# niclasborlin/dbat

Hardware: AMD Instinct MI355X
Metric: LM iterations/sec (higher is better)
Workload: dtype f64

## Files before the change

dbat_amd/_hip.py:

```python
from __future__ import annotations

import ctypes as C
import os
import sys

import numpy as np

_HERE = os.path.dirname(os.path.abspath(__file__))
LIB_PATH = os.path.join(_HERE, 'libdbat_hip.so')
if os.environ.get('DBAT_AMD_LIB') == 'prof':
    LIB_PATH = os.path.join(_HERE, 'libdbat_hip_prof.so')
elif os.environ.get('DBAT_AMD_LIB', '').endswith('.so'):
    LIB_PATH = os.environ['DBAT_AMD_LIB']
if LIB_PATH != os.path.join(_HERE, 'libdbat_hip.so'):
    sys.stderr.write('[dbat_amd] DBAT_AMD_LIB: loading %s instead of the product library\n' % LIB_PATH)

ABI_VERSION = 5
DAMP = {'none': 0, 'gm': 0, 'gna': 1, 'lm': 2, 'lmp': 3}

OK, EINVAL, EUNSUPPORTED, EDEVICE, ENOMEM = 0, -101, -102, -103, -104


class DbatHipUnavailable(RuntimeError):
    pass


class DbatHipError(RuntimeError):
    def __init__(self, code, msg):
        super().__init__('dbat_hip error %d: %s' % (code, msg))
        self.code = code


_dp = C.POINTER(C.c_double)
_ip = C.POINTER(C.c_int32)
_lp = C.POINTER(C.c_int64)
_bp = C.POINTER(C.c_uint8)


class Problem(C.Structure):
    _fields_ = [
        ('abi_version', C.c_int32), ('n_images', C.c_int32), ('n_points', C.c_int32),
        ('n_obs', C.c_int64), ('dist_model', C.c_int32), ('nK', C.c_int32), ('nP', C.c_int32),
        ('ip_cam', _ip), ('ip_pt', _ip), ('ip_val', _dp), ('ip_std', _dp),
        ('IO_val', _dp), ('px_size', _dp), ('EO_val', _dp), ('OP_val', _dp),
        ('est_IO', _bp), ('est_EO', _bp), ('est_OP', _bp),
        ('IO_block', _ip), ('EO_block', _ip),
        ('prior_IO_use', _bp), ('prior_IO_val', _dp), ('prior_IO_std', _dp),
        ('prior_EO_use', _bp), ('prior_EO_val', _dp), ('prior_EO_std', _dp),
        ('prior_OP_use', _bp), ('prior_OP_val', _dp), ('prior_OP_std', _dp),
        ('device', C.c_int32), ('shard_rank', C.c_int32), ('shard_count', C.c_int32),
    ]


class Options(C.Structure):
    _fields_ = [
        ('damping', C.c_int32), ('max_iter', C.c_int32), ('conv_tol', C.c_double),
        ('abs_term', C.c_int32), ('singular_test', C.c_int32), ('store_trace', C.c_int32),
        ('mu', C.c_double), ('alpha_min', C.c_double), ('lambda0', C.c_double),
        ('lambda_min', C.c_double), ('rho_bad', C.c_double), ('rho_good', C.c_double),
        ('delta0', C.c_double),
        ('term_fun', C.c_void_p), ('term_user', C.c_void_p), ('veto_fun', C.c_void_p), ('veto_user', C.c_void_p),
        ('trace_fun', C.c_void_p), ('trace_user', C.c_void_p),
    ]


TERM_FN = C.CFUNCTYPE(C.c_int32, C.c_void_p, _dp, _dp, C.c_int64)
VETO_FN = C.CFUNCTYPE(C.c_int32, C.c_void_p, _dp, C.c_int64)
TRACE_FN = C.CFUNCTYPE(None, C.c_void_p, C.c_int32, C.c_int32, C.c_double, C.c_double, C.c_int32, C.c_double)


def trace_text(damping, n, res, damp, step, rho):
    from fractions import Fraction
    if damping == DAMP['gna']:
        if damp != damp:
            return 'Gauss-Newton-Armijo: iteration %d, residual norm=%.2g' % (n, res)
        return 'Gauss-Newton-Armijo: iteration %d, residual norm=%.2g, last alpha=%s' % (n, res, Fraction(damp).limit_denominator(1 << 40))
    if damping == DAMP['lm']:
        if damp != damp:
            return 'Levenberg-Marquardt: iteration %d, residual norm=%.2g' % (n, res)
        return 'Levenberg-Marquardt: iteration %d, residual norm=%.2g, lambda=%.2g' % (n, res, damp)
    if damping == DAMP['lmp']:
        return 'Levenberg-Marquardt-Powell: iteration %d, residual norm=%.2g, delta=%.2g, step=%s, rho=%.1f' % (
            n, res, damp, ('GN', 'IP', 'CP')[step] if 0 <= step < 3 else '?', rho)
    return 'Gauss-Markov: iteration %d, residual norm=%.2g' % (n, res)


class Result(C.Structure):
    _fields_ = [
        ('code', C.c_int32), ('iters', C.c_int32), ('n_res', C.c_int32), ('n_damp', C.c_int32),
        ('n_trace', C.c_int32), ('sigma0', C.c_double), ('time_s', C.c_double),
        ('n_residual_evals', C.c_int32), ('n_linearizations', C.c_int32), ('n_solves', C.c_int32),
        ('n_trace_only', C.c_int32), ('stage_s', C.c_double * 5),
    ]


LOSS = {'huber': 0, 'cauchy': 1}
SCALE = {'apriori': 0, 'mad': 1}
ROBUST_MAX_OUTER = 64


class RobustOptions(C.Structure):
    _fields_ = [
        ('loss', C.c_int32), ('k', C.c_double), ('scale', C.c_int32), ('max_outer', C.c_int32),
        ('weight_tol', C.c_double),
    ]


class PairOptions(C.Structure):
    _fields_ = [('max_iter', C.c_int32), ('conv_tol', C.c_double), ('min_angle', C.c_double)]


class RobustResult(C.Structure):
    _fields_ = [
        ('outer', C.c_int32), ('converged', C.c_int32), ('inner_iters', C.c_int32 * ROBUST_MAX_OUTER),
        ('scale', C.c_double * ROBUST_MAX_OUTER), ('max_change', C.c_double), ('reweight_s', C.c_double),
    ]


ALLREDUCE_FN = C.CFUNCTYPE(C.c_int, C.c_void_p, C.c_void_p, C.c_int64, C.c_void_p)

class DepthStats(C.Structure):
    _fields_ = [('n_behind', C.c_int64), ('min_depth', C.c_double), ('argmin_column', C.c_int64)]


class VetoStats(C.Structure):
    _fields_ = [('tested', C.c_int64), ('rejected', C.c_int64), ('n_behind', C.c_int64), ('min_depth', C.c_double)]


_H = C.c_void_p
SYMBOLS = {
    'dbat_hip_last_error': (C.c_char_p, []),
    'dbat_hip_abi_version': (C.c_int, []),
    'dbat_hip_default_options': (C.c_int, [C.c_int32, C.POINTER(Options)]),
    'dbat_hip_plan': (C.c_int, [C.POINTER(Problem)] + [C.POINTER(C.c_int64)] * 7),
    'dbat_hip_plan_structural_rank_ok': (C.c_int, [C.POINTER(Problem), C.POINTER(C.c_int32)]),
    'dbat_hip_plan_point_owner': (C.c_int, [C.POINTER(Problem), _ip]),
    'dbat_hip_plan_serialize': (C.c_int, [C.POINTER(Problem), _dp]),
    'dbat_hip_plan_layout_stats': (C.c_int, [C.POINTER(Problem), C.POINTER(C.c_int64)]),
    'dbat_hip_plan_domain_map': (C.c_int, [C.POINTER(Problem), _ip, C.POINTER(C.c_int32)]),
    'dbat_hip_create': (C.c_int, [C.POINTER(Problem), C.POINTER(_H)]),
    'dbat_hip_destroy': (None, [_H]),
    'dbat_hip_num_params': (C.c_int64, [_H]),
    'dbat_hip_num_residuals': (C.c_int64, [_H]),
    'dbat_hip_serialize': (C.c_int, [_H, _dp]),
    'dbat_hip_deserialize': (C.c_int, [_H, _dp, _dp, _dp, _dp]),
    'dbat_hip_structural_rank_ok': (C.c_int, [_H, C.POINTER(C.c_int32)]),
    'dbat_hip_residual': (C.c_int, [_H, _dp, _dp, _dp]),
    'dbat_hip_jacobian_blocks': (C.c_int, [_H, _dp, _dp, _dp, _dp]),
    'dbat_hip_jacobian_sample': (C.c_int, [_H, _dp, C.c_int64, C.POINTER(C.c_int64), _dp, _dp, _dp, _dp]),
    'dbat_hip_linearize_solve': (C.c_int, [_H, _dp, C.c_double, C.c_int32, _dp, _dp]),
    'dbat_hip_jacobian_csc': (C.c_int, [_H, _dp, C.c_int32, C.POINTER(C.c_int64), C.POINTER(C.c_int64), C.POINTER(C.c_int64), _dp]),
    'dbat_hip_gradient': (C.c_int, [_H, _dp]),
    'dbat_hip_colnorms': (C.c_int, [_H, _dp]),
    'dbat_hip_jtimes_sqnorm': (C.c_int, [_H, _dp, _dp]),
    'dbat_hip_jtimes': (C.c_int, [_H, _dp, _dp]),
    'dbat_hip_solve': (C.c_int, [_H, C.POINTER(Options), _dp, C.POINTER(Result), _dp, _dp, _dp, _dp]),
    'dbat_hip_final_residuals': (C.c_int, [_H, _dp, _dp]),
    'dbat_hip_comm_unique_id': (C.c_int, [_bp]),
    'dbat_hip_comm_init': (C.c_int, [_H, _bp]),
    'dbat_hip_comm_allreduce_host': (C.c_int, [_H, _dp, C.c_int64, C.c_int32]),
    'dbat_hip_set_deterministic': (C.c_int, [_H, C.c_int32]),
    'dbat_hip_set_allreduce': (C.c_int, [_H, ALLREDUCE_FN, C.c_void_p]),
    'dbat_hip_owned_mask': (C.c_int, [_H, _bp]),
    'dbat_hip_forwintersect': (C.c_int, [_H, _dp, _bp, _dp]),
    'dbat_hip_resect': (C.c_int, [C.c_int32, C.c_int32, C.POINTER(C.c_int64), _dp, _dp, C.POINTER(C.c_int64), _ip, _dp, _dp]),
    'dbat_hip_rigidalign': (C.c_int, [C.c_int32, C.c_int64, _dp, _dp, _bp, C.c_int32, _dp, _dp, _dp]),
    'dbat_hip_multixform': (C.c_int, [C.c_int32, _dp, C.c_int64, C.c_int32, _dp, C.c_int64, _dp, _bp]),
    'dbat_hip_essmat5': (C.c_int, [C.c_int32, C.c_int32, C.POINTER(C.c_int64), _dp, _dp, _dp, _ip]),
    'dbat_hip_relorient': (C.c_int, [C.c_int32, C.c_int32, C.POINTER(C.c_int64), _dp, _dp, C.POINTER(C.c_int64), _ip, _dp,
                                     C.c_int32, _dp, _dp, _ip, _bp, _bp, _dp]),
    'dbat_hip_default_pair_options': (C.c_int, [C.POINTER(PairOptions)]),
    'dbat_hip_pairadjust': (C.c_int, [C.c_int32, C.c_int32, C.POINTER(C.c_int64), _dp, _dp, _bp, _dp, _dp, C.c_int32,
                                      C.POINTER(PairOptions), _dp, _dp, _bp, _dp, _ip, _dp, _dp]),
    'dbat_hip_bench_step': (C.c_int, [_H, C.c_double, C.c_int32, _dp]),
    'dbat_hip_structure_key': (C.c_int, [C.POINTER(Problem), C.POINTER(C.c_uint64)]),
    'dbat_hip_handle_key': (C.c_int, [_H, C.POINTER(C.c_uint64)]),
    'dbat_hip_set_values': (C.c_int, [_H, C.POINTER(Problem)]),
    'dbat_hip_set_x': (C.c_int, [_H, _dp]),
    'dbat_hip_info': (C.c_int, [_H, C.POINTER(C.c_int64)]),
    'dbat_hip_build_kernel_name': (C.c_int, [_H, C.c_char_p, C.c_int32]),
    'dbat_hip_chol_stats': (C.c_int, [_H, C.POINTER(C.c_int64)]),
    'dbat_hip_posterior_cov': (C.c_int, [_H, _dp, C.c_double, _dp, _dp, _dp, _dp]),
    'dbat_hip_redundancy': (C.c_int, [_H, _dp, _dp, _dp]),
    'dbat_hip_ray_angles': (C.c_int, [_H, _dp, _dp, _dp, _ip, _ip]),
    'dbat_hip_debug_ray_angles_host': (C.c_int, [C.POINTER(Problem), _dp, _dp]),
    'dbat_hip_point_depths': (C.c_int, [_H, _dp, C.c_double, _dp, _dp, C.POINTER(DepthStats)]),
    'dbat_hip_set_chirality': (C.c_int, [_H, C.c_int32, C.c_double]),
    'dbat_hip_chirality_stats': (C.c_int, [_H, C.POINTER(VetoStats)]),
    'dbat_hip_coverage': (C.c_int, [_H, _dp, _dp, _dp, _lp, _dp, _lp, _lp]),
    'dbat_hip_residual_stats': (C.c_int, [_H, _dp, _lp, _dp, _lp, _dp, _dp, _dp, _lp]),
    'dbat_hip_quality_hull_cap': (C.c_int32, []),
    'dbat_hip_debug_coverage_host': (C.c_int, [C.POINTER(Problem), _dp, _dp, _dp, _lp, _dp, _lp, _lp]),
    'dbat_hip_default_robust_options': (C.c_int, [C.c_int32, C.POINTER(RobustOptions)]),
    'dbat_hip_robust_weights': (C.c_int, [_H, _dp, C.POINTER(RobustOptions), _dp, _dp, _dp]),
    'dbat_hip_set_obs_weights': (C.c_int, [_H, _dp]),
    'dbat_hip_solve_robust': (C.c_int, [_H, C.POINTER(Options), C.POINTER(RobustOptions), _dp, C.POINTER(Result),
                                        _dp, _dp, _dp, _dp, C.POINTER(RobustResult), _dp]),
}
DEBUG_SYMBOLS = {
    'dbat_hip_debug_plan_digest': (C.c_int, [C.POINTER(Problem), C.POINTER(C.c_uint64), C.c_int32, C.c_char_p, C.c_int32]),
    'dbat_hip_debug_heavy_plan_selftest': (C.c_int, [C.POINTER(Problem), _dp]),
    'dbat_hip_debug_batch_stats': (C.c_int, [C.POINTER(Problem), C.POINTER(C.c_int64)]),
    'dbat_hip_debug_nd_stats': (C.c_int, [C.POINTER(Problem), C.c_int32, _dp]),
    'dbat_hip_debug_model_eval_host': (C.c_int, [C.c_int32, C.c_int32, C.c_int32, _dp, _dp, C.c_double,
                                                 _dp, _dp, _dp, _dp, _dp, _dp]),
    'dbat_hip_debug_ray_angles_ms': (C.c_int, [_H, _dp, C.POINTER(C.c_int64)]),
    'dbat_hip_debug_quality_ms': (C.c_int, [_H, _dp]),
    'dbat_hip_debug_point_depths_ms': (C.c_int, [_H, _dp]),
    'dbat_hip_debug_chirality_pass_ms': (C.c_int, [_H, _dp, C.c_int32, _dp]),
    'dbat_hip_debug_align_ms': (C.c_int, [_dp]),
    'dbat_hip_debug_align_timing': (C.c_int, [C.c_int32]),
    'dbat_hip_debug_relorient_ms': (C.c_int, [_dp]),
    'dbat_hip_debug_relorient_timing': (C.c_int, [C.c_int32]),
    'dbat_hip_debug_pairadjust_ms': (C.c_int, [_dp]),
    'dbat_hip_debug_pairadjust_timing': (C.c_int, [C.c_int32]),
}

_lib = None


def load():
    global _lib
    if _lib is not None:
        return _lib
    if not os.path.exists(LIB_PATH):
        raise DbatHipUnavailable(
            '%s not built: run `python -c "import __graft_entry__ as g; g.build()"` or '
            '`make -C dbat_amd/csrc` (needs hipcc).  There is no CPU fallback.' % LIB_PATH)
    try:
        try:
            import torch
        except Exception:
            pass
        lib = C.CDLL(LIB_PATH)
    except OSError as e:
        raise DbatHipUnavailable('cannot load %s: %s' % (LIB_PATH, e)) from e
    for name, (res, args) in {**SYMBOLS, **DEBUG_SYMBOLS}.items():
        try:
            fn = getattr(lib, name)
        except AttributeError as e:
            raise DbatHipUnavailable('%s does not export %s' % (LIB_PATH, name)) from e
        fn.restype = res
        fn.argtypes = args
    if lib.dbat_hip_abi_version() != ABI_VERSION:
        raise DbatHipUnavailable('ABI version mismatch')
    _lib = lib
    return lib


UNIQUE_ID_BYTES = 128


def comm_unique_id():
    buf = (C.c_uint8 * UNIQUE_ID_BYTES)()
    check(load().dbat_hip_comm_unique_id(buf))
    return bytes(buf)


def last_error():
    return load().dbat_hip_last_error().decode('utf-8', 'replace')


def check(rc):
    if rc != 0:
        raise DbatHipError(rc, last_error())


def dptr(a):
    return a.ctypes.data_as(_dp) if a is not None else None


def _flat(a, dtype):
    a = np.asarray(a)
    if a.dtype != dtype:
        a = a.astype(dtype)
    if a.ndim <= 1:
        return np.ascontiguousarray(a)
    if a.flags.f_contiguous:
        return a.reshape(-1, order='F')
    return a.flatten('F')


def _f64(a):
    return _flat(a, np.float64)


def _u8(a):
    a = np.asarray(a)
    if a.dtype != np.bool_:
        a = a.astype(bool)
    return _flat(a, np.bool_).view(np.uint8)


def _i32(a):
    return _flat(a, np.int32)


def problem_from_struct(s, device=0, shard_rank=0, shard_count=1):
    nc, npnt, no = s.EO.val.shape[1], s.OP.val.shape[1], s.IP.val.shape[1]
    dm = np.unique(s.IO.model.distModel)
    if dm.size != 1:
        raise ValueError('Mixed lens distortion models not implemented.')
    model = int(dm[0])
    if model == 1:
        if np.any(np.asarray(s.IO.val)[3:5] != 0) or np.any(np.asarray(s.bundle.est.IO)[3:5]):
            raise ValueError('lens distortion model 1 has no aspect/skew')
        model = 2
    if npnt >= 2 ** 31 or nc >= 2 ** 31:
        raise ValueError('too many points/images for int32 indices')
    keep = dict(
        ip_cam=_i32(s.IP.cam), ip_pt=_i32(s.IP.pt), ip_val=_f64(s.IP.val), ip_std=_f64(s.IP.std),
        IO_val=_f64(s.IO.val), px_size=_f64(s.IO.sensor.pxSize), EO_val=_f64(s.EO.val[:6]),
        OP_val=_f64(s.OP.val),
        est_IO=_u8(s.bundle.est.IO), est_EO=_u8(s.bundle.est.EO[:6]), est_OP=_u8(s.bundle.est.OP),
        IO_block=_i32(s.IO.struct.block), EO_block=_i32(s.EO.struct.block[:6]),
    )
    for nm in ('IO', 'EO', 'OP'):
        pr = getattr(s.prior, nm)
        rows = slice(0, 6) if nm == 'EO' else slice(None)
        use = np.asarray(pr.use)[rows]
        keep['prior_%s_use' % nm] = _u8(use)
        if use.any():
            keep['prior_%s_val' % nm] = _f64(np.nan_to_num(np.asarray(pr.val, float)[rows]))
            keep['prior_%s_std' % nm] = _f64(np.nan_to_num(np.asarray(pr.std, float)[rows], nan=1.0))
        else:
            keep['prior_%s_val' % nm] = _f64(np.asarray(pr.val, float)[rows])
            keep['prior_%s_std' % nm] = _f64(np.asarray(pr.std, float)[rows])
    p = Problem()
    p.abi_version = ABI_VERSION
    p.n_images, p.n_points, p.n_obs = nc, npnt, no
    p.dist_model, p.nK, p.nP = model, int(s.IO.model.nK), int(s.IO.model.nP)
    for k, v in keep.items():
        ptr_t = dict(Problem._fields_)[k]
        setattr(p, k, v.ctypes.data_as(ptr_t))
    p.device, p.shard_rank, p.shard_count = int(device), int(shard_rank), int(shard_count)
    return p, keep


class Handle:

    def __init__(self, s, device=0, shard_rank=0, shard_count=1, _problem=None):
        self.lib = load()
        self.prob, self._keep = _problem if _problem is not None else problem_from_struct(s, device, shard_rank, shard_count)
        h = _H()
        check(self.lib.dbat_hip_create(C.byref(self.prob), C.byref(h)))
        self.h = h
        self.n = int(self.lib.dbat_hip_num_params(h))
        self.m = int(self.lib.dbat_hip_num_residuals(h))
        self._cb = None

    def close(self):
        if getattr(self, 'h', None):
            self.lib.dbat_hip_destroy(self.h)
            self.h = None

    __del__ = close

    def key(self):
        k = (C.c_uint64 * 2)()
        check(self.lib.dbat_hip_handle_key(self.h, k))
        return (int(k[0]), int(k[1]))

    def set_values(self, s=None, _problem=None):
        prob, keep = _problem if _problem is not None else problem_from_struct(
            s, self.prob.device, self.prob.shard_rank, self.prob.shard_count)
        check(self.lib.dbat_hip_set_values(self.h, C.byref(prob)))
        self.prob, self._keep = prob, keep

    def serialize(self):
        x = np.empty(self.n)
        check(self.lib.dbat_hip_serialize(self.h, dptr(x)))
        return x

    def deserialize(self, x):
        nc, npnt = self.prob.n_images, self.prob.n_points
        R = 5 + self.prob.nK + self.prob.nP
        IO, EO, OP = np.empty(R * nc), np.empty(6 * nc), np.empty(3 * npnt)
        x = np.ascontiguousarray(x, float)
        check(self.lib.dbat_hip_deserialize(self.h, dptr(x), dptr(IO), dptr(EO), dptr(OP)))
        return (IO.reshape(R, nc, order='F'), EO.reshape(6, nc, order='F'),
                OP.reshape(3, npnt, order='F'))

    def structural_rank_ok(self):
        ok = C.c_int32(0)
        check(self.lib.dbat_hip_structural_rank_ok(self.h, C.byref(ok)))
        return bool(ok.value)

    def residual(self, x, want_r=True):
        x = np.ascontiguousarray(x, float)
        r = np.zeros(self.m) if want_r else None
        f = C.c_double(0)
        check(self.lib.dbat_hip_residual(self.h, dptr(x), dptr(r), C.byref(f)))
        return (r, f.value) if want_r else f.value

    def jacobian_blocks(self, x):
        no, R = self.prob.n_obs, 5 + self.prob.nK + self.prob.nP
        x = np.ascontiguousarray(x, float)
        JEO, JOP, JIO = np.zeros(12 * no), np.zeros(6 * no), np.zeros(2 * R * no)
        check(self.lib.dbat_hip_jacobian_blocks(self.h, dptr(x), dptr(JEO), dptr(JOP), dptr(JIO)))
        return (JEO.reshape(no, 6, 2).transpose(0, 2, 1), JOP.reshape(no, 3, 2).transpose(0, 2, 1),
                JIO.reshape(no, R, 2).transpose(0, 2, 1))

    def jacobian_sample(self, x, ip_cols):
        idx = np.ascontiguousarray(ip_cols, np.int64)
        n, R = idx.size, 5 + self.prob.nK + self.prob.nP
        x = np.ascontiguousarray(x, float)
        r, JEO, JOP, JIO = np.zeros(2 * n), np.zeros(12 * n), np.zeros(6 * n), np.zeros(2 * R * n)
        check(self.lib.dbat_hip_jacobian_sample(self.h, dptr(x), n, idx.ctypes.data_as(C.POINTER(C.c_int64)), dptr(r), dptr(JEO),
                                                dptr(JOP), dptr(JIO)))
        return (r.reshape(n, 2), JEO.reshape(n, 6, 2).transpose(0, 2, 1), JOP.reshape(n, 3, 2).transpose(0, 2, 1),
                JIO.reshape(n, R, 2).transpose(0, 2, 1))

    def jacobian_csc(self, x, weighted=True):
        import scipy.sparse as sp
        x = np.ascontiguousarray(x, float)
        nnz = C.c_int64(0)
        check(self.lib.dbat_hip_jacobian_csc(self.h, dptr(x), int(bool(weighted)), C.byref(nnz), None, None, None))
        colptr = np.zeros(self.n + 1, np.int64)
        rowidx = np.zeros(max(nnz.value, 1), np.int64)
        val = np.zeros(max(nnz.value, 1))
        i64 = C.POINTER(C.c_int64)
        check(self.lib.dbat_hip_jacobian_csc(self.h, dptr(x), int(bool(weighted)), C.byref(nnz), colptr.ctypes.data_as(i64),
                                             rowidx.ctypes.data_as(i64), dptr(val)))
        return sp.csc_matrix((val[:nnz.value], rowidx[:nnz.value], colptr), shape=(self.m, self.n))

    def linearize_solve(self, x, lam=0.0, scale=True):
        x = np.ascontiguousarray(x, float)
        p, st = np.empty(self.n), np.empty(8)
        check(self.lib.dbat_hip_linearize_solve(self.h, dptr(x), float(lam), int(bool(scale)),
                                                dptr(p), dptr(st)))
        return p, dict(f=st[0], JpJp=st[1], rJp=st[2], pp=st[3], trace=st[4], singular=bool(st[5]), rcond=st[6], chol_info=int(st[7]))

    def gradient(self):
        g = np.empty(self.n)
        check(self.lib.dbat_hip_gradient(self.h, dptr(g)))
        return g

    def colnorms(self):
        g = np.empty(self.n)
        check(self.lib.dbat_hip_colnorms(self.h, dptr(g)))
        return g

    def jtimes_sqnorm(self, v):
        v = np.ascontiguousarray(v, float)
        out = C.c_double(0)
        check(self.lib.dbat_hip_jtimes_sqnorm(self.h, dptr(v), C.byref(out)))
        return out.value

    def jtimes(self, v):
        v = np.ascontiguousarray(v, float)
        out = np.zeros(self.m)
        check(self.lib.dbat_hip_jtimes(self.h, dptr(v), dptr(out)))
        return out

    def solve(self, x0, opt, term_fun=None, veto_fun=None, trace_fun=None):
        x = np.ascontiguousarray(x0, float).copy()
        raised = []

        def guarded(fn, *views):
            if raised:
                return 1
            try:
                return int(bool(fn(*views)))
            except BaseException as e:
                raised.append(e)
                return 1
        keep = []
        if term_fun is not None:
            keep.append(TERM_FN(lambda _u, Jp, r, m: guarded(term_fun, np.ctypeslib.as_array(Jp, (m,)).copy(),
                                                             np.ctypeslib.as_array(r, (m,)).copy())))
            opt.term_fun = C.cast(keep[-1], C.c_void_p)
        if veto_fun is not None:
            keep.append(VETO_FN(lambda _u, xx, n: guarded(veto_fun, np.ctypeslib.as_array(xx, (n,)).copy())))
            opt.veto_fun = C.cast(keep[-1], C.c_void_p)
        if trace_fun is not None:
            def traced(_u, damping, n, res, damp, step, rho):
                if not raised:
                    try:
                        trace_fun(damping, n, res, damp, step, rho)
                    except BaseException as e:
                        raised.append(e)
            keep.append(TRACE_FN(traced))
            opt.trace_fun = C.cast(keep[-1], C.c_void_p)
        try:
            return self._solve(x, opt, raised)
        finally:
            if trace_fun is not None:
                opt.trace_fun = None
            if term_fun is not None:
                opt.term_fun = None
            if veto_fun is not None:
                opt.veto_fun = None

    def _solve(self, x, opt, raised):
        res = Result()
        mi = opt.max_iter
        rr = np.full(mi + 3, np.nan)
        damp = np.full(2 * mi + 4, np.nan)
        aux = np.full(2 * mi + 4, np.nan)
        trace = np.empty(self.n * (mi + 2)) if opt.store_trace else None
        check(self.lib.dbat_hip_solve(self.h, C.byref(opt), dptr(x), C.byref(res), dptr(rr),
                                      dptr(damp), dptr(aux), dptr(trace)))
        if raised:
            raise raised[0]
        T = (trace[:self.n * res.n_trace].reshape(self.n, res.n_trace, order='F')
             if trace is not None else None)
        return x, res, rr[:res.n_res], damp[:res.n_damp], aux, T

    def final_residuals(self):
        ru, rw = np.empty(self.m), np.empty(self.m)
        check(self.lib.dbat_hip_final_residuals(self.h, dptr(ru), dptr(rw)))
        return ru, rw

    def forwintersect(self, x, OP, skip=None):
        x = np.ascontiguousarray(x, float)
        out = np.ascontiguousarray(np.asarray(OP, float).flatten('F'))
        sk = None if skip is None else np.ascontiguousarray(np.asarray(skip, bool).astype(np.uint8))
        check(self.lib.dbat_hip_forwintersect(self.h, dptr(x), None if sk is None else sk.ctypes.data_as(_bp), dptr(out)))
        return out.reshape(3, -1, order='F')

    def set_deterministic(self, on=True):
        check(self.lib.dbat_hip_set_deterministic(self.h, int(bool(on))))

    def build_kernel_name(self):
        buf = C.create_string_buffer(64)
        check(self.lib.dbat_hip_build_kernel_name(self.h, buf, 64))
        return buf.value.decode()

    def comm_init(self, unique_id):
        buf = (C.c_uint8 * UNIQUE_ID_BYTES).from_buffer_copy(bytes(unique_id))
        check(self.lib.dbat_hip_comm_init(self.h, buf))

    def comm_allreduce_host(self, a, op='sum'):
        a = np.ascontiguousarray(a, np.float64).copy()
        check(self.lib.dbat_hip_comm_allreduce_host(self.h, dptr(a), a.size, {'sum': 0, 'max': 1, 'min': 2}[op]))
        return a

    def set_allreduce(self, pyfunc):
        def tramp(user, buf, count, stream):
            try:
                return int(pyfunc(int(buf or 0), int(count), int(stream or 0)) or 0)
            except Exception:
                import traceback
                traceback.print_exc()
                return 1
        self._cb = ALLREDUCE_FN(tramp)
        check(self.lib.dbat_hip_set_allreduce(self.h, self._cb, None))

    def owned_mask(self):
        m = np.zeros(self.n, np.uint8)
        check(self.lib.dbat_hip_owned_mask(self.h, m.ctypes.data_as(_bp)))
        return m.astype(bool)

    def index_maps(self):
        if getattr(self, '_index_maps', None) is None:
            big = 1e15
            IO, EO, OP = self.deserialize(big + np.arange(self.n, dtype=float))
            f = lambda a: np.where(a >= big / 2, np.rint(a - big), -1).astype(np.int64)
            maps = f(IO), f(EO), f(OP)
            for a in maps:
                a.setflags(write=False)
            self._index_maps = maps
        return self._index_maps

    def posterior_cov(self, x, sigma0, want_sinv=False):
        x = np.ascontiguousarray(x, float)
        NS = self.info()['NS']
        nc, npnt = int(self.prob.n_images), int(self.prob.n_points)
        nIOu = NS - 6 * nc
        CEO = np.zeros(36 * nc)
        CIO = np.zeros(max(nIOu * nIOu, 1))
        COP = np.zeros(9 * npnt)
        Sinv = np.zeros(NS * NS) if want_sinv else None
        check(self.lib.dbat_hip_posterior_cov(self.h, dptr(x), float(sigma0), dptr(CEO), dptr(CIO), dptr(COP),
                                              dptr(Sinv) if want_sinv else None))
        out = [CEO.reshape(nc, 6, 6).transpose(0, 2, 1), CIO[:nIOu * nIOu].reshape(nIOu, nIOu).T,
               COP.reshape(npnt, 3, 3).transpose(0, 2, 1)]
        if want_sinv:
            L = np.tril(Sinv.reshape(NS, NS).T)
            out.append(L + np.tril(L, -1).T)
        return tuple(out)

    def redundancy(self, x):
        x = np.ascontiguousarray(x, float)
        no = int(self.prob.n_obs)
        qvv = np.zeros(3 * max(no, 1))
        rp = np.zeros(max(self.m - 2 * no, 1))
        check(self.lib.dbat_hip_redundancy(self.h, dptr(x), dptr(qvv), dptr(rp)))
        return qvv[:3 * no].reshape(3, no, order='F'), rp[:self.m - 2 * no]

    def ray_angles(self, x):
        x = np.ascontiguousarray(x, float)
        nc, npnt = int(self.prob.n_images), int(self.prob.n_points)
        op, cam = np.zeros(max(npnt, 1)), np.zeros(max(nc, 1))
        opr, camr = np.zeros(max(npnt, 1), np.int32), np.zeros(max(nc, 1), np.int32)
        check(self.lib.dbat_hip_ray_angles(self.h, dptr(x), dptr(op), dptr(cam), opr.ctypes.data_as(_ip),
                                           camr.ctypes.data_as(_ip)))
        return op[:npnt], cam[:nc], opr[:npnt], camr[:nc]

    def ray_angles_ms(self):
        ms, info = np.zeros(3), (C.c_int64 * 2)()
        check(self.lib.dbat_hip_debug_ray_angles_ms(self.h, dptr(ms), info))
        return dict(points=float(ms[0]), cam_dirs=float(ms[1]), cam_pairs=float(ms[2]), mfma=int(info[0]),
                    workgroups=int(info[1]))

    def point_depths(self, x, thr=0.0, want_depth=True):
        x = np.ascontiguousarray(x, float)
        nc, no = int(self.prob.n_images), int(self.prob.n_obs)
        d = np.zeros(max(no, 1)) if want_depth else None
        im = np.zeros(max(nc, 1))
        st = DepthStats()
        check(self.lib.dbat_hip_point_depths(self.h, dptr(x), float(thr), dptr(d), dptr(im), C.byref(st)))
        return (d[:no] if want_depth else None), im[:nc], int(st.n_behind), float(st.min_depth), int(st.argmin_column)

    def point_depths_ms(self):
        ms = np.zeros(1)
        check(self.lib.dbat_hip_debug_point_depths_ms(self.h, dptr(ms)))
        return float(ms[0])

    def chirality_pass_ms(self, x, reps=20):
        x = np.ascontiguousarray(x, float)
        ms = np.zeros(2)
        check(self.lib.dbat_hip_debug_chirality_pass_ms(self.h, dptr(x), int(reps), dptr(ms)))
        return float(ms[0]), int(ms[1])

    def set_chirality(self, on=True, min_depth=0.0):
        check(self.lib.dbat_hip_set_chirality(self.h, int(bool(on)), float(min_depth)))

    def chirality_stats(self):
        st = VetoStats()
        check(self.lib.dbat_hip_chirality_stats(self.h, C.byref(st)))
        return int(st.tested), int(st.rejected), int(st.n_behind), float(st.min_depth)

    def coverage(self):
        return _coverage_call(lambda *a: self.lib.dbat_hip_coverage(self.h, *a), int(self.prob.n_images), int(self.prob.n_obs))

    def residual_stats(self, x):
        x = np.ascontiguousarray(x, float)
        nc, npnt = int(self.prob.n_images), int(self.prob.n_points)
        cam_n, op_n = np.zeros(max(nc, 1), np.int64), np.zeros(max(npnt, 1), np.int64)
        cam_ss, op_ss = np.zeros(max(nc, 1)), np.zeros(max(npnt, 1))
        tot, mx, mip = C.c_double(), C.c_double(), C.c_int64()
        check(self.lib.dbat_hip_residual_stats(self.h, dptr(x), cam_n.ctypes.data_as(_lp), dptr(cam_ss),
                                               op_n.ctypes.data_as(_lp), dptr(op_ss), C.cast(C.byref(tot), _dp),
                                               C.cast(C.byref(mx), _dp), C.cast(C.byref(mip), _lp)))
        return dict(cam_n=cam_n[:nc], cam_ss=cam_ss[:nc], op_n=op_n[:npnt], op_ss=op_ss[:npnt], total_ss=tot.value,
                    max_e=mx.value, max_ip=int(mip.value))

    def quality_ms(self):
        ms = np.zeros(2)
        check(self.lib.dbat_hip_debug_quality_ms(self.h, dptr(ms)))
        return dict(coverage=float(ms[0]), residual_stats=float(ms[1]))

    def robust_weights(self, x, ropt):
        x = np.ascontiguousarray(x, float)
        no = int(self.prob.n_obs)
        om, sn, sc = np.zeros(max(no, 1)), np.zeros(max(no, 1)), C.c_double()
        check(self.lib.dbat_hip_robust_weights(self.h, dptr(x), C.byref(ropt), dptr(om), dptr(sn), C.byref(sc)))
        return om[:no], sn[:no], sc.value

    def set_obs_weights(self, omega):
        if omega is None:
            check(self.lib.dbat_hip_set_obs_weights(self.h, None))
            return
        om = np.ascontiguousarray(omega, float).ravel()
        if om.size != int(self.prob.n_obs):
            raise ValueError('set_obs_weights: %d values for %d image points' % (om.size, int(self.prob.n_obs)))
        check(self.lib.dbat_hip_set_obs_weights(self.h, dptr(om)))

    def solve_robust(self, x0, opt, ropt):
        x = np.ascontiguousarray(x0, float).copy()
        res, rr = Result(), RobustResult()
        mi = opt.max_iter
        r = np.full(mi + 3, np.nan)
        damp = np.full(2 * mi + 4, np.nan)
        aux = np.full(2 * mi + 4, np.nan)
        trace = np.empty(self.n * (mi + 2)) if opt.store_trace else None
        no = int(self.prob.n_obs)
        om = np.ones(max(no, 1))
        check(self.lib.dbat_hip_solve_robust(self.h, C.byref(opt), C.byref(ropt), dptr(x), C.byref(res), dptr(r),
                                             dptr(damp), dptr(aux), dptr(trace), C.byref(rr), dptr(om)))
        T = (trace[:self.n * res.n_trace].reshape(self.n, res.n_trace, order='F')
             if trace is not None else None)
        return x, res, r[:res.n_res], damp[:res.n_damp], aux, T, rr, om[:no]

    def set_x(self, x):
        x = np.ascontiguousarray(x, float)
        check(self.lib.dbat_hip_set_x(self.h, dptr(x)))

    def bench_step(self, lam=0.0, scale=False):
        ms = np.zeros(16)
        check(self.lib.dbat_hip_bench_step(self.h, float(lam), int(bool(scale)), dptr(ms)))
        return ms

    def chol_stats(self):
        a = (C.c_int64 * 6)()
        check(self.lib.dbat_hip_chol_stats(self.h, a))
        keys = ('order_padded', 'tile_tasks', 'tile_products', 'tile_rows', 'nested_dissection', 'dataflow')
        return dict(zip(keys, [int(v) for v in a]))

    def info(self):
        a = (C.c_int64 * 24)()
        check(self.lib.dbat_hip_info(self.h, a))
        keys = ('NS', 'n_batches', 'max_k', 'n_obs_shard', 'n_pts_shard', 'BT', 'ncolmax', 'n_tiles',
                'domain_sharding', 'reduced_doubles_per_factorisation', 'vector_doubles_per_linearisation',
                'n_top_cams', 'factor_tile_rows', 'tasks_domain', 'tasks_top', 'tile_kernel_mfma',
                'heavy_tasks', 'heavy_mfma', 'heavy_row_groups', 'heavy_scratch_bytes', 'heavy_points', 'heavy_obs',
                'heavy_ksteps_per_task', 'heavy_algorithmic_flops')
        return dict(zip(keys, [int(v) for v in a]))


def structure_key(s, device=0, shard_rank=0, shard_count=1, _problem=None):
    prob, keep = _problem if _problem is not None else problem_from_struct(s, device, shard_rank, shard_count)
    k = (C.c_uint64 * 2)()
    check(load().dbat_hip_structure_key(C.byref(prob), k))
    return (int(k[0]), int(k[1]))


_cached = None
cache_stats = {'hits': 0, 'misses': 0}


def acquire(s, device=0):
    global _cached
    problem = problem_from_struct(s, device)
    h, _cached = _cached, None
    if h is not None and h.h:
        if h.key() == structure_key(None, _problem=problem):
            try:
                h.set_values(_problem=problem)
                cache_stats['hits'] += 1
                cache_stats['last'] = 'hit'
                return h
            except DbatHipError:
                pass
        h.close()
    cache_stats['misses'] += 1
    cache_stats['last'] = 'miss'
    return Handle(None, _problem=problem)


def release(h, keep=True):
    global _cached
    if not keep or h is None or not h.h:
        if h is not None:
            h.close()
        return
    if _cached is not None and _cached is not h:
        _cached.close()
    h.set_deterministic(False)
    h.set_chirality(False)
    _cached = h


def clear_cache():
    global _cached
    if _cached is not None:
        _cached.close()
    _cached = None


def default_options(damping='gna'):
    o = Options()
    check(load().dbat_hip_default_options(DAMP[damping.lower()], C.byref(o)))
    return o


def robust_options(loss, k=None, scale='apriori', max_outer=10, weight_tol=1e-3):
    o = RobustOptions()
    check(load().dbat_hip_default_robust_options(LOSS[loss], C.byref(o)))
    if k is not None:
        o.k = float(k)
    o.scale = SCALE[scale]
    o.max_outer = int(max_outer)
    o.weight_tol = float(weight_tol)
    return o


def plan(s, shard_rank=0, shard_count=1):
    lib = load()
    p, keep = problem_from_struct(s, 0, shard_rank, shard_count)
    v = [C.c_int64(0) for _ in range(7)]
    check(lib.dbat_hip_plan(C.byref(p), *[C.byref(a) for a in v]))
    keys = ('n', 'm', 'nIO', 'nEO', 'nOP', 'pt_lo', 'pt_hi')
    return dict(zip(keys, [a.value for a in v]))


def plan_structural_rank_ok(s):
    lib = load()
    p, keep = problem_from_struct(s)
    ok = C.c_int32(0)
    check(lib.dbat_hip_plan_structural_rank_ok(C.byref(p), C.byref(ok)))
    return bool(ok.value)


def plan_point_owner(s, shard_count):
    lib = load()
    p, keep = problem_from_struct(s, 0, 0, shard_count)
    owner = np.full(s.OP.val.shape[1], -1, np.int32)
    check(lib.dbat_hip_plan_point_owner(C.byref(p), owner.ctypes.data_as(_ip)))
    return owner


def resect_poses(pt_start, X, xn, tri_start, tri, device=0):
    lib = load()
    n = len(pt_start) - 1
    ps = np.ascontiguousarray(pt_start, np.int64)
    ts = np.ascontiguousarray(tri_start, np.int64)
    Xf = np.ascontiguousarray(np.asarray(X, float).flatten('F'))
    xf = np.ascontiguousarray(np.asarray(xn, float).flatten('F'))
    tf = np.ascontiguousarray(np.asarray(tri, np.int32).reshape(-1))
    P, rms = np.empty(12 * n), np.empty(n)
    i64p = C.POINTER(C.c_int64)
    check(lib.dbat_hip_resect(int(device), n, ps.ctypes.data_as(i64p), dptr(Xf), dptr(xf), ts.ctypes.data_as(i64p),
                              tf.ctypes.data_as(_ip), dptr(P), dptr(rms)))
    return P.reshape(n, 4, 3).transpose(0, 2, 1), rms


def essmat5_sets(set_start, Q1, Q2, device=0):
    lib = load()
    ss = np.ascontiguousarray(set_start, np.int64)
    n = len(ss) - 1
    Q1, Q2 = np.asarray(Q1, float), np.asarray(Q2, float)
    if Q1.ndim != 2 or Q1.shape[0] != 3 or Q1.shape != Q2.shape or n < 0 or (n >= 0 and Q1.shape[1] != ss[-1]):
        raise ValueError('essmat5: Q1 and Q2 must both be 3-by-n, n the end of the last set')
    q1, q2 = _f64(Q1), _f64(Q2)
    E, ns = np.zeros(90 * max(n, 1)), np.zeros(max(n, 1), np.int32)
    check(lib.dbat_hip_essmat5(int(device), n, ss.ctypes.data_as(C.POINTER(C.c_int64)), dptr(q1), dptr(q2), dptr(E),
                               ns.ctypes.data_as(_ip)))
    return E[:90 * n].reshape(n, 10, 9), ns[:n]


def relorient_pairs(pt_start, x1, x2, hyp_start, samples, thr2, front_dir, device=0):
    lib = load()
    ps, hs = np.ascontiguousarray(pt_start, np.int64), np.ascontiguousarray(hyp_start, np.int64)
    n = len(ps) - 1
    x1, x2 = np.asarray(x1, float), np.asarray(x2, float)
    smp = np.ascontiguousarray(np.asarray(samples, np.int32).reshape(-1, 5))
    t2 = np.ascontiguousarray(np.broadcast_to(np.asarray(thr2, float), (max(n, 0),)))
    if len(hs) != n + 1 or x1.ndim != 2 or x1.shape[0] != 2 or x1.shape != x2.shape or x1.shape[1] != ps[-1] or smp.shape[0] != hs[-1]:
        raise ValueError('relorient: x1 and x2 must both be 2-by-n and samples k-by-5, n and k the ends of the last ranges')
    total = x1.shape[1]
    a, b = _f64(x1), _f64(x2)
    E, P2, st = np.zeros(9 * max(n, 1)), np.zeros(12 * max(n, 1)), np.zeros(8 * max(n, 1), np.int32)
    inl, fr, X = np.zeros(max(total, 1), np.uint8), np.zeros(max(total, 1), np.uint8), np.zeros(3 * max(total, 1))
    i64p = C.POINTER(C.c_int64)
    check(lib.dbat_hip_relorient(int(device), n, ps.ctypes.data_as(i64p), dptr(a), dptr(b), hs.ctypes.data_as(i64p),
                                 smp.ctypes.data_as(_ip), dptr(t2), int(front_dir), dptr(E), dptr(P2), st.ctypes.data_as(_ip),
                                 inl.ctypes.data_as(_bp), fr.ctypes.data_as(_bp), dptr(X)))
    return dict(E=E[:9 * n].reshape(n, 9), P2=P2[:12 * n].reshape(n, 4, 3).transpose(0, 2, 1), stats=st[:8 * n].reshape(n, 8),
                inlier=inl[:total].astype(bool), in_front=fr[:total].astype(bool), X=X[:3 * total].reshape(3, total, order='F'))


def cams_from_e(e, x1, x2, front_dir, device=0):
    lib = load()
    x1, x2 = np.asarray(x1, float), np.asarray(x2, float)
    if x1.ndim != 2 or x1.shape[0] != 2 or x1.shape != x2.shape:
        raise ValueError('camsfrome: the points must be 2-by-n')
    n = x1.shape[1]
    ps = np.array([0, n], np.int64)
    a, b, E, t2 = _f64(x1), _f64(x2), np.ascontiguousarray(np.asarray(e, float).reshape(9)).copy(), np.ones(1)
    P2, st = np.zeros(12), np.zeros(8, np.int32)
    inl, fr, X = np.zeros(max(n, 1), np.uint8), np.zeros(max(n, 1), np.uint8), np.zeros(3 * max(n, 1))
    check(lib.dbat_hip_relorient(int(device), 1, ps.ctypes.data_as(C.POINTER(C.c_int64)), dptr(a), dptr(b), None, None, dptr(t2),
                                 int(front_dir), dptr(E), dptr(P2), st.ctypes.data_as(_ip), inl.ctypes.data_as(_bp),
                                 fr.ctypes.data_as(_bp), dptr(X)))
    return dict(P2=P2.reshape(4, 3).T.copy(), X=X[:3 * n].reshape(3, n, order='F'), in_front=fr[:n].astype(bool), sp=st[4:8].copy())


def relorient_timing(on=True):
    check(load().dbat_hip_debug_relorient_timing(int(bool(on))))


def relorient_ms():
    ms = np.zeros(3)
    check(load().dbat_hip_debug_relorient_ms(dptr(ms)))
    return dict(solve=float(ms[0]), score=float(ms[1]), cams=float(ms[2]))


PAIR_CODES = ('converged', 'max_iter', 'no_step', 'singular', 'too_few')


def pairadjust(pt_start, x1, x2, P2, X, use=None, w1=None, w2=None, front_dir=-1, max_iter=20, conv_tol=1e-6, min_angle=0.0,
               residuals=False, device=0):
    lib = load()
    ps = np.ascontiguousarray(pt_start, np.int64)
    n = len(ps) - 1
    x1, x2, X = np.asarray(x1, float), np.asarray(x2, float), np.asarray(X, float)
    P2 = np.asarray(P2, float).reshape(-1, 3, 4)
    if n < 0 or x1.ndim != 2 or x1.shape[0] != 2 or x1.shape != x2.shape or x1.shape[1] != ps[-1] or X.shape != (3, x1.shape[1]) \
            or P2.shape[0] != n:
        raise ValueError('pairadjust: x1 and x2 must be 2-by-total, X 3-by-total, total the end of the last range, and P2 one 3-by-4 per pair')
    total = x1.shape[1]
    a, b = _f64(x1), _f64(x2)
    wt = [None if w is None else _f64(np.broadcast_to(np.asarray(w, float), (2, total))) for w in (w1, w2)]
    u = None if use is None else np.ascontiguousarray(np.broadcast_to(np.asarray(use, bool), (total,))).view(np.uint8)
    P = np.ascontiguousarray(P2.transpose(0, 2, 1)).reshape(-1).copy()
    P = np.concatenate([P, np.zeros(12)]) if n == 0 else P
    Xf = X.flatten('F')
    Xf = np.zeros(3) if total == 0 else Xf
    used, ds, ist, Q = np.zeros(max(total, 1), np.uint8), np.zeros(4 * max(n, 1)), np.zeros(4 * max(n, 1), np.int32), np.zeros(36 * max(n, 1))
    res = np.zeros(4 * max(total, 1)) if residuals else None
    opt = PairOptions(int(max_iter), float(conv_tol), float(min_angle))
    check(lib.dbat_hip_pairadjust(int(device), n, ps.ctypes.data_as(C.POINTER(C.c_int64)), dptr(a), dptr(b),
                                  None if u is None else u.ctypes.data_as(_bp), dptr(wt[0]), dptr(wt[1]), int(front_dir), C.byref(opt),
                                  dptr(P), dptr(Xf), used.ctypes.data_as(_bp), dptr(ds), ist.ctypes.data_as(_ip), dptr(Q), dptr(res)))
    ds, ist = ds[:4 * n].reshape(n, 4), ist[:4 * n].reshape(n, 4)
    return dict(P2=P[:12 * n].reshape(n, 4, 3).transpose(0, 2, 1), X=Xf[:3 * total].reshape(3, total, order='F'), used=used[:total].astype(bool),
                f0=ds[:, 0].copy(), f=ds[:, 1].copy(), sigma0=ds[:, 2].copy(), lam=ds[:, 3].copy(), code=ist[:, 0].copy(),
                iters=ist[:, 1].copy(), trials=ist[:, 2].copy(), n_used=ist[:, 3].copy(), Q=Q[:36 * n].reshape(n, 6, 6).transpose(0, 2, 1),
                res=None if res is None else res[:4 * total].reshape(total, 2, 2).transpose(1, 2, 0))


def pairadjust_timing(on=True):
    check(load().dbat_hip_debug_pairadjust_timing(int(bool(on))))


def pairadjust_ms():
    ms = np.zeros(1)
    check(load().dbat_hip_debug_pairadjust_ms(dptr(ms)))
    return float(ms[0])


def rigidalign(X, Y, scale=False, use=None, resid=False, device=0):
    lib = load()
    X, Y = np.asarray(X, float), np.asarray(Y, float)
    if X.ndim != 2 or X.shape[0] != 3 or X.shape != Y.shape:
        raise ValueError('rigidalign: X and Y must both be 3-by-n')
    n = X.shape[1]
    Xf, Yf = _f64(X), _f64(Y)
    u = None
    if use is not None:
        u = np.ascontiguousarray(np.asarray(use, bool).ravel()).view(np.uint8)
        if u.shape[0] != n:
            raise ValueError('rigidalign: use must have one entry per column')
    T, st = np.zeros(16), np.zeros(4)
    r = np.empty(3 * n) if resid else None
    check(lib.dbat_hip_rigidalign(int(device), n, dptr(Xf), dptr(Yf), None if u is None else u.ctypes.data_as(_bp),
                                  int(bool(scale)), dptr(T), dptr(st), dptr(r)))
    return (T.reshape(4, 4, order='F'), dict(alpha=float(st[0]), rms=float(st[1]), used=int(st[2]), sv_ratio=float(st[3])),
            None if r is None else r.reshape(3, n, order='F'))


def multixform(EO, OP, T, device=0):
    lib = load()
    EO, OP, T = np.asarray(EO, float), np.asarray(OP, float), np.asarray(T, float)
    if T.shape != (4, 4):
        raise ValueError('multixform: T must be 4-by-4')
    EO = np.zeros((6, 0)) if EO.size == 0 else EO
    OP = np.zeros((3, 0)) if OP.size == 0 else OP
    if EO.ndim != 2 or OP.ndim != 2 or (OP.size and OP.shape[0] != 3):
        raise ValueError('multixform: EO must be 6-by-M (or more rows), OP 3-by-N')
    nc, npnt = (EO.shape[1] if EO.size else 0), (OP.shape[1] if OP.size else 0)
    rows = EO.shape[0] if nc else 6
    eo, op = np.array(EO, float, order='F'), np.array(OP, float, order='F')
    fail = np.zeros(max(nc, 1), np.uint8)
    check(lib.dbat_hip_multixform(int(device), dptr(_f64(T)), nc, int(rows), dptr(eo.reshape(-1, order='F')) if nc else None,
                                  npnt, dptr(op.reshape(-1, order='F')) if npnt else None, fail.ctypes.data_as(_bp)))
    return eo, op, fail[:nc].astype(bool)


def align_timing(on=True):
    check(load().dbat_hip_debug_align_timing(int(bool(on))))


def align_ms():
    ms = np.zeros(5)
    check(load().dbat_hip_debug_align_ms(dptr(ms)))
    return dict(centroid=float(ms[0]), cross=float(ms[1]), resid=float(ms[2]), points=float(ms[3]), cams=float(ms[4]))


def plan_layout_stats(s, shard_rank=0, shard_count=1):
    lib = load()
    p, keep = problem_from_struct(s, 0, shard_rank, shard_count)
    a = (C.c_int64 * 16)()
    check(lib.dbat_hip_plan_layout_stats(C.byref(p), a))
    v = [int(x) for x in a]
    return dict(n_tiles=v[0], n_batches=v[1], n_batches_tiled=v[2], n_groups=v[3], n_group_points=v[4], n_chunks=v[5],
                chunks_by_length={'1-8': v[6], '9-16': v[7], '17-32': v[8], '33-64': v[9]}, chunks_multi_round=v[10],
                k_max=v[11], rows_max=v[12], build_sig=bool(v[13]), backsub_sig=bool(v[14]), heavy_tasks=v[15])


def plan_digest(s, shard_rank=0, shard_count=1):
    lib = load()
    p, keep = problem_from_struct(s, 0, shard_rank, shard_count)
    out = (C.c_uint64 * 96)()
    names = C.create_string_buffer(4096)
    n = lib.dbat_hip_debug_plan_digest(C.byref(p), out, 96, names, 4096)
    if n < 0:
        check(n)
    return dict(zip(names.value.decode().split(','), [int(v) for v in out[:n]]))


def heavy_plan_selftest(s, shard_rank=0, shard_count=1):
    lib = load()
    p, keep = problem_from_struct(s, 0, shard_rank, shard_count)
    out = np.zeros(8)
    check(lib.dbat_hip_debug_heavy_plan_selftest(C.byref(p), dptr(out)))
    return dict(on=bool(out[0]), points=int(out[1]), row_groups=int(out[2]), tasks=int(out[3]), ksteps=int(out[4]),
                max_diff=float(out[5]), max_abs=float(out[6]), entries=int(out[7]))


def nd_stats(s, mode, shard_rank=0, shard_count=1):
    lib = load()
    p, keep = problem_from_struct(s, 0, shard_rank, shard_count)
    out = np.zeros(24)
    check(lib.dbat_hip_debug_nd_stats(C.byref(p), int(mode), dptr(out)))
    part = lambda v: dict(cameras=int(v[0]), blocks=int(v[1]), tile_columns=int(v[2]), tiles=int(v[3]), chain=int(v[4]),
                          products=int(v[5]), model_us=float(v[6]), mode=int(v[7]), valid=int(v[8]) == 0, run=int(v[9]),
                          model='estimate' if v[10] else 'list schedule')
    return part(out[:12]), part(out[12:])


def batch_stats(s, shard_rank=0, shard_count=1):
    lib = load()
    p, keep = problem_from_struct(s, 0, shard_rank, shard_count)
    a = (C.c_int64 * 16)()
    check(lib.dbat_hip_debug_batch_stats(C.byref(p), a))
    v = [int(x) for x in a]
    part = lambda q: dict(max_points=v[q], max_obs=v[q + 1], closed_by_cap=v[q + 2], max_tile_batches=v[q + 3])
    return dict(tiled=part(0), untiled=part(4), BT=v[8], PMAX=v[9], tile_bmax=v[10], n_batches_tiled=v[11],
                n_batches_untiled=v[12])


def plan_domain_map(s, shard_count):
    lib = load()
    p, keep = problem_from_struct(s, 0, 0, shard_count)
    owner = np.full(s.EO.val.shape[1], -1, np.int32)
    sub = C.c_int32(0)
    check(lib.dbat_hip_plan_domain_map(C.byref(p), owner.ctypes.data_as(_ip), C.byref(sub)))
    return owner, bool(sub.value)


def plan_serialize(s):
    lib = load()
    p, keep = problem_from_struct(s)
    x0 = np.empty(plan(s)['n'])
    check(lib.dbat_hip_plan_serialize(C.byref(p), dptr(x0)))
    return x0


def debug_model_eval_host(model, nK, nP, EO6, IO, px, Q, uv):
    lib = load()
    R = 5 + nK + nP
    r, A, B, Cc = np.zeros(2), np.zeros(12), np.zeros(6), np.zeros(2 * R)
    a = [np.ascontiguousarray(v, float) for v in (EO6, IO, Q, uv)]
    check(lib.dbat_hip_debug_model_eval_host(model, nK, nP, dptr(a[0]), dptr(a[1]), float(px),
                                             dptr(a[2]), dptr(a[3]), dptr(r), dptr(A), dptr(B), dptr(Cc)))
    return r, A.reshape(6, 2).T, B.reshape(3, 2).T, Cc.reshape(R, 2).T


def _coverage_call(fn, nc, no):
    lo, hi = np.zeros(2 * max(nc, 1)), np.zeros(2 * max(nc, 1))
    rad, area = np.zeros(max(nc, 1)), np.zeros(max(nc, 1))
    rip, hs, hip = np.zeros(max(nc, 1), np.int64), np.zeros(nc + 1, np.int64), np.zeros(max(no, 1), np.int64)
    lp = lambda a: a.ctypes.data_as(_lp)
    check(fn(dptr(lo), dptr(hi), dptr(rad), lp(rip), dptr(area), lp(hs), lp(hip)))
    return dict(lo=lo[:2 * nc].reshape(2, nc, order='F'), hi=hi[:2 * nc].reshape(2, nc, order='F'), rad_max=rad[:nc],
                rad_ip=rip[:nc], hull_area=area[:nc], hull=[hip[hs[c]:hs[c + 1]].copy() for c in range(nc)])


def quality_hull_cap():
    return int(load().dbat_hip_quality_hull_cap())


def debug_coverage_host(s):
    lib = load()
    p, keep = problem_from_struct(s)
    return _coverage_call(lambda *a: lib.dbat_hip_debug_coverage_host(C.byref(p), *a), int(p.n_images), int(p.n_obs))


def debug_ray_angles_host(s):
    lib = load()
    p, keep = problem_from_struct(s)
    op, cam = np.zeros(max(int(p.n_points), 1)), np.zeros(max(int(p.n_images), 1))
    check(lib.dbat_hip_debug_ray_angles_host(C.byref(p), dptr(op), dptr(cam)))
    return op[:int(p.n_points)], cam[:int(p.n_images)]
```

dbat_amd/csrc/chol_df.hpp:

```cpp
#pragma once
#include "env.hpp"
#include <cstdio>
#include <functional>
#include <queue>

#include "chol.hpp"
#include "nd.hpp"

namespace dbat {

constexpr int DF_LD = 65;
constexpr int DF_SPIN_CAP = 1 << 22;

struct DfTask { int i, k; };
struct DfJob { int i, k, jlo, jhi, part, np, mode, p; };

__device__ __forceinline__ double ld_coh(const double *p) {
    return __hip_atomic_load(p, __ATOMIC_RELAXED, __HIP_MEMORY_SCOPE_AGENT);
}
__device__ __forceinline__ void st_coh(double *p, double v) {
    __hip_atomic_store(p, v, __ATOMIC_RELAXED, __HIP_MEMORY_SCOPE_AGENT);
}

typedef double df_d2 __attribute__((ext_vector_type(2)));
__device__ __forceinline__ df_d2 ld_coh16(const double *p) {
    df_d2 v;
    asm volatile("global_load_dwordx4 %0, %1, off sc1" : "=v"(v) : "v"(p) : "memory");
    return v;
}
__device__ __forceinline__ df_d2 ld_l2_16(const double *p) {
    df_d2 v;
    asm volatile("global_load_dwordx4 %0, %1, off" : "=v"(v) : "v"(p) : "memory");
    return v;
}
__device__ __forceinline__ double ld_tile(const double *p, bool l2) {
    return l2 ? __hip_atomic_load(p, __ATOMIC_RELAXED, __HIP_MEMORY_SCOPE_WORKGROUP)
              : __hip_atomic_load(p, __ATOMIC_RELAXED, __HIP_MEMORY_SCOPE_AGENT);
}
__device__ __forceinline__ void df_wait16(df_d2 &a, df_d2 &b) {
    asm volatile("s_waitcnt vmcnt(0)" : "+v"(a), "+v"(b) : : "memory");
}
template <int LD>
__device__ __forceinline__ void df_load_tile16(const double *T, int64_t ld, double *Pm, int tx, int ty, bool l2) {
    const double *src = T + 2 * (tx & 31);
    df_d2 v[8];
    if (l2) {
#pragma unroll
        for (int q = 0; q < 8; ++q) v[q] = ld_l2_16(src + (int64_t)(2 * (ty + 4 * q) + (tx >> 5)) * ld);
    } else {
#pragma unroll
        for (int q = 0; q < 8; ++q) v[q] = ld_coh16(src + (int64_t)(2 * (ty + 4 * q) + (tx >> 5)) * ld);
    }
#pragma unroll
    for (int q = 0; q < 8; q += 2) df_wait16(v[q], v[q + 1]);
#pragma unroll
    for (int q = 0; q < 8; ++q) {
        double *dst = Pm + (2 * (ty + 4 * q) + (tx >> 5)) * LD + 2 * (tx & 31);
        dst[0] = v[q].x; dst[1] = v[q].y;
    }
}
__device__ __forceinline__ void df_tile16_issue(const double *T, int64_t ld, df_d2 (&v)[8], int tx, int ty, bool l2) {
    const double *src = T + 2 * (tx & 31);
    if (l2) {
#pragma unroll
        for (int q = 0; q < 8; ++q) v[q] = ld_l2_16(src + (int64_t)(2 * (ty + 4 * q) + (tx >> 5)) * ld);
    } else {
#pragma unroll
        for (int q = 0; q < 8; ++q) v[q] = ld_coh16(src + (int64_t)(2 * (ty + 4 * q) + (tx >> 5)) * ld);
    }
}
template <int LD>
__device__ __forceinline__ void df_tile16_commit(df_d2 (&v)[8], double *Pm, int tx, int ty) {
#pragma unroll
    for (int q = 0; q < 8; q += 2) df_wait16(v[q], v[q + 1]);
#pragma unroll
    for (int q = 0; q < 8; ++q) {
        double *dst = Pm + (2 * (ty + 4 * q) + (tx >> 5)) * LD + 2 * (tx & 31);
        dst[0] = v[q].x; dst[1] = v[q].y;
    }
}

__device__ __forceinline__ bool df_spin(const int *flag, int epoch, int *abort_flag) {
    int spins = 0;
    while (__hip_atomic_load(flag, __ATOMIC_RELAXED, __HIP_MEMORY_SCOPE_AGENT) != epoch) {
        __builtin_amdgcn_s_sleep(1);
        ++spins;
        if ((spins & 255) == 0) {
            if (spins > DF_SPIN_CAP) __hip_atomic_store(abort_flag, 1, __ATOMIC_RELAXED, __HIP_MEMORY_SCOPE_AGENT);
            if (__hip_atomic_load(abort_flag, __ATOMIC_RELAXED, __HIP_MEMORY_SCOPE_AGENT)) return false;
        }
    }
    return true;
}

constexpr int DF_TLD = 130;

template <int K, bool FIRST>
__device__ __forceinline__ void df_fmac_bcast(double &a, double m, double b) {
    if constexpr (FIRST)
        asm volatile("s_nop 1\n\tv_fmac_f64_dpp %0, %1, %2 row_newbcast:%3 row_mask:0xf bank_mask:0xf" : "+v"(a) : "v"(m), "v"(b), "n"(K));
    else
        asm volatile("v_fmac_f64_dpp %0, %1, %2 row_newbcast:%3 row_mask:0xf bank_mask:0xf" : "+v"(a) : "v"(m), "v"(b), "n"(K));
}
template <int K, bool FIRST = true>
struct DfUpdFrom {
    static __device__ __forceinline__ void run(double (&a)[16], double m, double nly) {
        if constexpr (K < 16) { df_fmac_bcast<K, FIRST>(a[K], m, nly); DfUpdFrom<K + 1, false>::run(a, m, nly); }
    }
};
__device__ __forceinline__ double df_swap16(double v) {
    const long long b = __double_as_longlong(v);
    const int lo = __builtin_amdgcn_ds_swizzle((int)(b & 0xffffffffll), 0x401F);
    const int hi = __builtin_amdgcn_ds_swizzle((int)(b >> 32), 0x401F);
    return __longlong_as_double(((long long)hi << 32) | (unsigned int)lo);
}
__device__ __forceinline__ double df_mirror16(double v, int src4 ) {
    const long long b = __double_as_longlong(v);
    const int lo = __builtin_amdgcn_ds_bpermute(src4, (int)(b & 0xffffffffll));
    const int hi = __builtin_amdgcn_ds_bpermute(src4, (int)(b >> 32));
    return __longlong_as_double(((long long)hi << 32) | (unsigned int)lo);
}
template <int J>
struct DfElimCol {
    static __device__ __forceinline__ void run(double (&a)[16], double &piv, unsigned &badmask, double m, int src4) {
        badmask |= !(piv > 0.0) ? 1u << J : 0u;
        const double araw = a[J];
        constexpr int J1 = J + 1 < 16 ? J + 1 : 0;
        const double y0 = __builtin_amdgcn_rsq(piv);
        const double t = y0 * y0;
        const double e = __builtin_fma(-piv, t, 1.0);
        const double y = __builtin_fma(y0, __builtin_fma(e, 0.375, 0.5) * e, y0);
        const double y2 = __builtin_fma(t, __builtin_fma(e, e, e), t);
        const double nly = -(araw * y2);
        double mn = 0.0;
        if constexpr (J < 15) {
            df_fmac_bcast<J1, true>(a[J1], m, nly);
            mn = df_mirror16(a[J1], src4);
            piv = readlane_f64(a[J1], J1);
            __builtin_amdgcn_sched_barrier(0);
        }
        a[J] = araw * y;
        DfUpdFrom<J + 2, false>::run(a, m, nly);
        if constexpr (J < 15) DfElimCol<J + 1>::run(a, piv, badmask, mn, src4);
    }
};

template <int NS>
__device__ __forceinline__ void df_trail(double *Tm, int p, int w, int lane) {
    constexpr int LD = DF_TLD;
    const int ntile = p == 0 ? 9 : (p == 1 ? 7 : 4);
    chol_d4 c4[NS];
    double av[NS][4], bv[NS][4];
    int cbs[NS], rbs[NS];
    bool valid[NS];
#pragma unroll
    for (int s3 = 0; s3 < NS; ++s3) {
        int n = w + 4 * s3;
        valid[s3] = n < ntile;
        n = valid[s3] ? n : ntile - 1;
        const int step = n < 4 ? 0 : (n < 7 ? 1 : 2);
        const int cb = p + 1 + step;
        n -= step == 0 ? 0 : (step == 1 ? 4 : 7);
        const int nT_ = 4 - cb;
        const int rowbase = n < nT_ ? 16 * (cb + n) : 64 + 16 * (n - nT_);
        const bool fresh = n == nT_ + p;
        cbs[s3] = cb; rbs[s3] = rowbase;
#pragma unroll
        for (int e = 0; e < 4; ++e) {
            const double v = Tm[(16 * cb + (lane >> 4) + 4 * e) * LD + (fresh ? 16 * cb : rowbase) + (lane & 15)];
            c4[s3][e] = fresh ? 0.0 : v;
        }
#pragma unroll
        for (int q = 0; q < 4; ++q) {
            const int m = 16 * p + 4 * q + (lane >> 4);
            av[s3][q] = -Tm[m * LD + 16 * cb + (lane & 15)];
            bv[s3][q] = Tm[m * LD + rowbase + (lane & 15)];
        }
    }
#pragma unroll
    for (int q = 0; q < 4; ++q)
#pragma unroll
        for (int s3 = 0; s3 < NS; ++s3) c4[s3] = __builtin_amdgcn_mfma_f64_16x16x4f64(av[s3][q], bv[s3][q], c4[s3], 0, 0, 0);
#pragma unroll
    for (int s3 = 0; s3 < NS; ++s3)
        if (valid[s3]) {
#pragma unroll
            for (int e = 0; e < 4; ++e) Tm[(16 * cbs[s3] + (lane >> 4) + 4 * e) * LD + rbs[s3] + (lane & 15)] = c4[s3][e];
        }
}

struct DfHook {
    int *pub_flag = nullptr;
    int epoch = 0;
    const int *look1 = nullptr, *look2 = nullptr;
    int *look_out = nullptr;
    const double *tsrc = nullptr;
    int64_t tld = 0;
    bool tb_loaded = false;
    double tb[16];
};
struct DfNoHook {};

#ifdef DBAT_POTF2_STAGES
#define DF_STG(n) do { if (t == 0) { asm volatile("s_waitcnt lgkmcnt(0)" ::: "memory"); const long long now_ = (long long)__builtin_readcyclecounter(); \
    atomicAdd((unsigned long long *)(tr + 16 + (n)), (unsigned long long)(now_ - stg_last_)); stg_last_ = now_; } } while (0)
#else
#define DF_STG(n) do { } while (0)
#endif
template <bool PUB = false, class HOOK = DfNoHook>
__device__ __forceinline__ void df_potf2(double *Tm, int nb, int j0, int *info, long long *tr, HOOK *H = nullptr) {
    constexpr int LD = DF_TLD;
    const int t = threadIdx.x, lane = t & 63;
    const int w = __builtin_amdgcn_readfirstlane(t >> 6);
#ifdef DBAT_POTF2_STAGES
    long long stg_last_ = (long long)__builtin_readcyclecounter();
#endif
    __syncthreads();
#pragma unroll 1
    for (int p = 0; p < 4; ++p) {
        {
            const int nlowT = 48 - 16 * p;
            int row, ident = -1;
            if (lane < 16) row = 16 * p + lane;
            else {
                const int s = 16 * w + (lane - 16);
                row = s < nlowT ? 16 * (p + 1) + s : 64 + (s - nlowT);
                if (lane < 32 && s - nlowT >= 16 * p) ident = s - nlowT - 16 * p;
            }
            const bool act = lane < 32;
            int lk1 = 0, lk2 = 0;
            if constexpr (PUB) {
                if (p == 3 && H->tsrc && H->look_out[2] == H->epoch) {
#pragma unroll
                    for (int kk = 0; kk < 16; ++kk) H->tb[kk] = ld_coh(H->tsrc + (int64_t)(4 * kk) * H->tld);
                    H->tb_loaded = true;
                }
                if (p >= 2 && t == 0) {
                    if (H->look1 && !H->tb_loaded) lk1 = __hip_atomic_load(H->look1, __ATOMIC_RELAXED, __HIP_MEMORY_SCOPE_AGENT);
                    if (H->look2 && p == 3) lk2 = __hip_atomic_load(H->look2, __ATOMIC_RELAXED, __HIP_MEMORY_SCOPE_AGENT);
                }
            }
            DF_STG(0);
            double a[16];
#pragma unroll
            for (int q = 0; q < 16; ++q) a[q] = (act && ident < 0) ? Tm[(16 * p + q) * LD + row] : (ident == q ? 1.0 : 0.0);
            DF_STG(1);
#ifndef DBAT_POTF2_STAGES
            if (tr && t == 0 && p == 1) tr[5] = wall_clock64();
#endif
            unsigned badmask = 0;
            double piv = readlane_f64(a[0], 0);
            const int src4 = 4 * (lane & ~16);
            DfElimCol<0>::run(a, piv, badmask, df_mirror16(a[0], src4), src4);
            DF_STG(2);
#ifndef DBAT_POTF2_STAGES
            if (tr && t == 0 && p == 1) tr[13] = wall_clock64();
#endif
            if (lane >= 16 ? act : w == 0) {
#pragma unroll
                for (int q = 0; q < 16; ++q) Tm[(16 * p + q) * LD + row] = a[q];
            }
            DF_STG(3);
            if (badmask != 0 && t == 0 && *info == 0) *info = j0 + 16 * p + __builtin_ctz(badmask) + 1;
            if constexpr (PUB) {
                if (p == 2 && t == 0) H->look_out[2] = lk1;
                if (p == 3 && t == 0) { H->look_out[0] = H->tb_loaded ? H->epoch : lk1; H->look_out[1] = lk2; }
            }
        }
        if constexpr (PUB) { if (p == 0 && H->pub_flag) asm volatile("s_waitcnt vmcnt(0)" ::: "memory"); }
        __syncthreads();
        if constexpr (PUB) {
            if (p == 0 && H->pub_flag && t == 0) __hip_atomic_store(H->pub_flag, H->epoch, __ATOMIC_RELAXED, __HIP_MEMORY_SCOPE_AGENT);
        }
        DF_STG(4);
#ifndef DBAT_POTF2_STAGES
        if (tr && t == 0) tr[6 + 2 * p] = wall_clock64();
#endif
        if (p == 3) break;
        if (p == 0) df_trail<3>(Tm, 0, w, lane);
        else if (p == 1) df_trail<2>(Tm, 1, w, lane);
        else df_trail<1>(Tm, 2, w, lane);
        DF_STG(5);
        __syncthreads();
        DF_STG(6);
#ifndef DBAT_POTF2_STAGES
        if (tr && t == 0) tr[7 + 2 * p] = wall_clock64();
#endif
    }
}

__device__ __forceinline__ bool df_spin_wave(const int *flag, int epoch, int *abort_flag) {
    int spins = 0;
    while (__hip_atomic_load(flag, __ATOMIC_RELAXED, __HIP_MEMORY_SCOPE_AGENT) != epoch) {
        __builtin_amdgcn_s_sleep(1);
        ++spins;
        if ((spins & 255) == 0) {
            if (spins > DF_SPIN_CAP) __hip_atomic_store(abort_flag, 1, __ATOMIC_RELAXED, __HIP_MEMORY_SCOPE_AGENT);
            if (__hip_atomic_load(abort_flag, __ATOMIC_RELAXED, __HIP_MEMORY_SCOPE_AGENT)) return false;
        }
    }
    return true;
}

constexpr unsigned long long DF_SENTINEL = 0xFFFFFFFFFFFFFFFFull;

struct DfView {
    double *base;
    const int64_t *toff;
    int64_t ld;
    const uint64_t *rowbits;
    int W;
    const int *iperm;
    const double *S;
    int64_t ldS;
    int n_nat;
    int no_l2;
};

__device__ __forceinline__ bool df_backward(double *smem, const DfView &V, int n, int nT, int j,
                                            const int *__restrict__ bk_ptr, const int *__restrict__ bk_idx,
                                            const int *flags, int epoch, int *abort_flag, const double *linv_all,
                                            double *q_out, double *q_nat, const double *qscale, double *dz_out) {
    constexpr int NB = 64, LD = 65;
    const int t = threadIdx.x, tx = t & 63, ty = t >> 6;
    const int nc = min(NB, n - NB * j);
    const int64_t col0 = (int64_t)NB * j;
    double *red = smem;
    double *part = smem + NB * LD;
    double *sv = part + 4 * NB;
    if (!df_spin_wave(flags + (int64_t)j * nT + j, epoch, abort_flag)) return false;
    if (!df_spin_wave(flags + (int64_t)nT * nT + j, epoch, abort_flag)) return false;
    double lv[16];
    const bool l2 = V.iperm != nullptr && !(V.no_l2 & 1);
#pragma unroll
    for (int q = 0; q < 16; ++q) lv[q] = ld_tile(linv_all + (size_t)j * NB * NB + tx * NB + ty + 4 * q, l2);
    const double yv = tx < nc ? ld_coh(V.base + V.toff[(int64_t)nT * nT + j] + (int64_t)tx * V.ld) : 0.0;
    double acc[16];
#pragma unroll
    for (int q = 0; q < 16; ++q) acc[q] = 0.0;
    for (int e = bk_ptr[j]; e < bk_ptr[j + 1]; ++e) {
        const int i = bk_idx[e];
        const int nr = min(NB, n - NB * i);
        if (!df_spin_wave(flags + (int64_t)i * nT + j, epoch, abort_flag)) return false;
        double v[16];
        const double *Lt = V.base + V.toff[(int64_t)i * nT + j] + tx;
#pragma unroll
        for (int q = 0; q < 16; ++q) v[q] = (tx < nr && ty + 4 * q < nc) ? ld_tile(Lt + (int64_t)(ty + 4 * q) * V.ld, l2) : 0.0;
        double qv = 0.0;
        int spins = 0;
        for (;;) {
            qv = tx < nr ? ld_coh(q_out + (int64_t)NB * i + tx) : 0.0;
            if (__all((unsigned long long)__double_as_longlong(qv) != DF_SENTINEL)) break;
            __builtin_amdgcn_s_sleep(1);
            if ((++spins & 255) == 0) {
                if (spins > DF_SPIN_CAP) __hip_atomic_store(abort_flag, 1, __ATOMIC_RELAXED, __HIP_MEMORY_SCOPE_AGENT);
                if (__hip_atomic_load(abort_flag, __ATOMIC_RELAXED, __HIP_MEMORY_SCOPE_AGENT)) return false;
            }
        }
#pragma unroll
        for (int q = 0; q < 16; ++q) acc[q] += v[q] * qv;
    }
#pragma unroll
    for (int q = 0; q < 16; ++q) red[(ty + 4 * q) * LD + tx] = acc[q];
    __syncthreads();
    {
        double s = 0.0;
#pragma unroll
        for (int r = 0; r < 16; ++r) s += red[tx * LD + 16 * ty + r];
        part[ty * NB + tx] = s;
    }
    __syncthreads();
    if (ty == 0) sv[tx] = yv - ((part[tx] + part[NB + tx]) + (part[2 * NB + tx] + part[3 * NB + tx]));
    __syncthreads();
    {
        double s = 0.0;
#pragma unroll
        for (int q = 0; q < 16; ++q) s += lv[q] * sv[ty + 4 * q];
        red[ty * NB + tx] = s;
    }
    __syncthreads();
    if (ty == 0 && tx < nc) {
        double qj = (red[tx] + red[NB + tx]) + (red[2 * NB + tx] + red[3 * NB + tx]);
        if (qj != qj) qj = __longlong_as_double(0x7ff8000000000000ll);
        st_coh(q_out + col0 + tx, qj);
        if (q_nat != q_out || dz_out) {
            const int zn = V.iperm ? V.iperm[col0 + tx] : (int)(col0 + tx);
            if (zn >= 0 && q_nat != q_out) q_nat[zn] = qj;
            if (zn >= 0 && dz_out) dz_out[zn] = qscale[zn] * qj;
        }
    }
    __syncthreads();
    return true;
}

struct DfChain {
    const int *cols;
    const int *par;
    const int *bits;
    int *claim;
    int *dflags;
    int *giveup;
    const int *pos;
    int ncols, nwg, ctr_slot, role_slot;
    int trace_potf2;
};

__device__ __forceinline__ void df_issue_acc_tile(const double *T, int64_t ld, double (&tp)[16], int tx, int ty) {
#pragma unroll
    for (int rt = 0; rt < 4; ++rt)
#pragma unroll
        for (int e = 0; e < 4; ++e) tp[4 * rt + e] = ld_coh(T + (int64_t)(16 * ty + (tx >> 4) + 4 * e) * ld + 16 * rt + (tx & 15));
}

__device__ __forceinline__ bool df_chain_role(double *smem, const DfView &V, int nT, const DfChain &C, int *flags, int *tflags,
                                              int *ctl, int epoch, double *linv_all, int *info, double *ldiag,
                                              int *s_word, long long *trace) {
    constexpr int NB = 64, XLD = DF_LD;
    double *Tm = smem, *Xm = smem + NB * DF_TLD;
    const int t = threadIdx.x, tx = t & 63, ty = t >> 6;
    int *abort_flag = ctl + 1, *counter = ctl + C.ctr_slot;
    int *s_task = s_word, *s_ok = s_word + 1, *look = s_word + 2;
    int k = -1;
    int *pub = nullptr;
    double tp[16];
#define DF_CLK(slot) do { if (trace && t == 0) trace[(int64_t)k * 16 + (slot)] = wall_clock64(); } while (0)
#define DF_VAL(slot, v) do { if (trace && t == 0) trace[(int64_t)k * 16 + (slot)] = (v); } while (0)
    bool fresh = true;
    for (;;) {
        if (k < 0) {
            for (;;) {
                if (t == 0) {
                    const int tk = atomicAdd(counter, 1);
                    int kk = tk < C.ncols ? C.cols[tk] : -1;
                    if (kk >= 0 && (C.bits[kk] & 1) && atomicAdd(C.giveup + kk - 1, 0) != epoch) kk = -2;
                    if (kk >= 0 && atomicExch(C.claim + kk, epoch) == epoch) kk = -2;
                    *s_task = kk;
                }
                __syncthreads();
                k = *s_task;
                __syncthreads();
                if (k != -2) break;
            }
            if (k < 0) return true;
            fresh = true;
        }
        if (fresh) {
            fresh = false;
            DF_CLK(0); DF_VAL(8, 1);
            const bool cont = (C.bits[k] & 1) != 0;
            if (t == 0) {
                bool ok = df_spin(C.dflags + k, epoch, abort_flag);
                if (ok && cont) ok = df_spin(flags + (int64_t)k * nT + (k - 1), epoch, abort_flag);
                *s_ok = ok;
            }
            __syncthreads();
            if (!*s_ok) { if (t == 0) *info = -1; return false; }
            df_issue_acc_tile(V.base + V.toff[(int64_t)k * nT + k], V.ld, tp, tx, ty);
            if (cont) df_load_tile16<XLD>(V.base + V.toff[(int64_t)k * nT + (k - 1)], V.ld, Xm, tx, ty, false);
            __syncthreads();
        }
        DF_CLK(1);
        {
            chol_d4 acc[4] = {{0, 0, 0, 0}, {0, 0, 0, 0}, {0, 0, 0, 0}, {0, 0, 0, 0}};
            if (C.bits[k] & 1) mfma_tile64<XLD>(Xm, Xm, ty, tx, acc);
#pragma unroll
            for (int rt = 0; rt < 4; ++rt)
#pragma unroll
                for (int e = 0; e < 4; ++e) {
                    const int c = 16 * ty + (tx >> 4) + 4 * e, r = 16 * rt + (tx & 15);
                    Tm[c * DF_TLD + r] = r >= c ? tp[4 * rt + e] - acc[rt][e] : 0.0;
                }
        }
        DF_CLK(2);
        const int p = C.par[k];
        const bool nxt = (C.bits[k] & 2) != 0;
        double *Tpk = V.base + V.toff[(int64_t)p * nT + k];
        DfHook H;
        H.pub_flag = pub; H.epoch = epoch;
        H.look1 = tflags + k; H.look2 = nxt ? C.dflags + k + 1 : nullptr; H.look_out = look;
        H.tsrc = Tpk + (int64_t)(tx >> 4) * V.ld + 16 * ty + (tx & 15); H.tld = V.ld;
        df_potf2<true>(Tm, NB, NB * k, info, trace && C.trace_potf2 ? trace + (int64_t)(nT + k) * 16 : nullptr, &H);
        DF_CLK(3);
        pub = nullptr;
        const double piv = ty == 0 ? Tm[tx * DF_TLD + tx] : 0.0;
        bool have_t = H.tb_loaded || look[0] == epoch;
        bool pre = nxt && look[1] == epoch;
        if (!have_t || (nxt && !pre)) {
            if (t == 0) {
                const bool ok = have_t || df_spin(tflags + k, epoch, abort_flag);
                int pr = pre ? 1 : 0;
                if (ok && nxt && !pre && __hip_atomic_load(C.dflags + k + 1, __ATOMIC_RELAXED, __HIP_MEMORY_SCOPE_AGENT) == epoch) pr = 1;
                *s_ok = ok ? 1 + pr : 0;
            }
            __syncthreads();
            const int st = *s_ok;
            if (!st) { if (t == 0) *info = -1; return false; }
            pre = st == 2;
        }
        if (pre && t == 0) __hip_atomic_store(C.claim + k + 1, epoch, __ATOMIC_RELAXED, __HIP_MEMORY_SCOPE_AGENT);
        DF_CLK(4); DF_VAL(9, pre ? 1 : 0); DF_VAL(10, H.tb_loaded ? 1 : 0);
        if (!H.tb_loaded) {
#pragma unroll
            for (int kk = 0; kk < 16; ++kk) H.tb[kk] = ld_coh(H.tsrc + (int64_t)(4 * kk) * V.ld);
        }
        double *Linv = linv_all + (size_t)k * NB * NB;
#pragma unroll
        for (int q = 0; q < 16; ++q) {
            const int c = ty + 4 * q;
            st_coh(Linv + c * NB + tx, (c >> 4) <= (tx >> 4) ? Tm[tx * DF_TLD + 64 + c] : 0.0);
        }
        if (pre) df_issue_acc_tile(V.base + V.toff[(int64_t)(k + 1) * nT + k + 1], V.ld, tp, tx, ty);
        DF_CLK(5);
        const int nrp = p == nT ? 1 : NB;
        {
            chol_d4 x[4] = {{0, 0, 0, 0}, {0, 0, 0, 0}, {0, 0, 0, 0}, {0, 0, 0, 0}};
            const double *pl = Tm + (tx & 15) * DF_TLD + 64 + (tx >> 4);
#pragma unroll
            for (int kk = 0; kk < 16; ++kk) {
                const double b = H.tb[kk];
#pragma unroll
                for (int cb = 0; cb < 4; ++cb)
                    if (kk < 4 * (cb + 1)) {
                        const double a = pl[16 * cb * DF_TLD + 4 * kk];
                        x[cb] = __builtin_amdgcn_mfma_f64_16x16x4f64(a, b, x[cb], 0, 0, 0);
                    }
            }
            asm volatile("s_waitcnt vmcnt(0)" ::: "memory");
            if (tx == 0) {
                if (atomicAdd(s_word + 5, 1) == 3) {
                    s_word[5] = 0;
                    __hip_atomic_store(flags + (int64_t)k * nT + k, epoch, __ATOMIC_RELAXED, __HIP_MEMORY_SCOPE_AGENT);
                }
            }
#pragma unroll
            for (int cb = 0; cb < 4; ++cb)
#pragma unroll
                for (int e = 0; e < 4; ++e) {
                    const int c = 16 * cb + (tx >> 4) + 4 * e, r = 16 * ty + (tx & 15);
                    if (r < nrp) st_coh(Tpk + (int64_t)c * V.ld + r, x[cb][e]);
                    Xm[c * XLD + r] = x[cb][e];
                }
        }
        if (ldiag && ty == 0) { const int zn = V.iperm[NB * k + tx]; if (zn >= 0) ldiag[zn] = piv; }
        if (t == 0 && nxt && !pre) {
            int got = 0;
            for (int s = 0; s < 6 && !got; ++s) {
                if (__hip_atomic_load(C.dflags + k + 1, __ATOMIC_RELAXED, __HIP_MEMORY_SCOPE_AGENT) == epoch)
                    got = atomicExch(C.claim + k + 1, epoch) != epoch ? 1 : -1;
                else __builtin_amdgcn_s_sleep(8);
            }
            *s_task = got > 0;
        }
        __syncthreads();
        DF_CLK(6);
        if (nxt && !pre && *s_task) {
            DF_VAL(9, 2);
            df_issue_acc_tile(V.base + V.toff[(int64_t)(k + 1) * nT + k + 1], V.ld, tp, tx, ty);
            asm volatile("s_waitcnt vmcnt(0)" ::: "memory");
            __syncthreads();
            if (t == 0) __hip_atomic_store(flags + (int64_t)p * nT + k, epoch, __ATOMIC_RELAXED, __HIP_MEMORY_SCOPE_AGENT);
            DF_CLK(7);
            k = k + 1;
            DF_CLK(0); DF_VAL(8, 0);
            continue;
        }
        if (pre) {
            pub = flags + (int64_t)p * nT + k;
            DF_CLK(7);
            k = k + 1;
            DF_CLK(0); DF_VAL(8, 0);
            continue;
        }
        asm volatile("s_waitcnt vmcnt(0)" ::: "memory");
        __syncthreads();
        if (t == 0) {
            __hip_atomic_store(flags + (int64_t)p * nT + k, epoch, __ATOMIC_RELAXED, __HIP_MEMORY_SCOPE_AGENT);
            int take = 0;
            if (nxt) {
                const int was = atomicExch(C.giveup + k, epoch);
                asm volatile("" ::"v"(was) : "memory");
                if (atomicAdd(counter, 0) > C.pos[k + 1] && atomicExch(C.claim + k + 1, epoch) != epoch) take = 1;
            }
            *s_task = take;
        }
        DF_CLK(7);
        __syncthreads();
        const int take = *s_task;
        __syncthreads();
        if (take) { k = k + 1; fresh = true; }
        else k = -1;
    }
#undef DF_CLK
#undef DF_VAL
}

template <bool CHAIN>
__global__ __launch_bounds__(256) void k_chol_df(DfView V, int n, int nT, const DfJob *__restrict__ tasks,
                                                 int ntasks, int *__restrict__ flags, int *__restrict__ ctl, int epoch,
                                                 double *__restrict__ linv_all, int *__restrict__ info,
                                                 long long *__restrict__ trace, const int *__restrict__ bk_ptr,
                                                 const int *__restrict__ bk_idx, double *__restrict__ q_out,
                                                 double *__restrict__ q_nat, double *__restrict__ ldiag,
                                                 const double *__restrict__ qscale, double *__restrict__ dz_out,
                                                 double *__restrict__ parts, int nparts,
                                                 const int *__restrict__ bk_list, int nbk, int ctr_slot, DfChain C) {
    constexpr int NB = 64, LD = DF_LD;
    __shared__ double smem[(CHAIN ? 3 : 2) * NB * LD];
    double *Pm = smem, *Qm = smem + NB * LD;
    __shared__ int s_word[8];
    int &s_task = s_word[0], &s_ok = s_word[1];
    const int t = threadIdx.x, tx = t & 63, ty = t >> 6;
    int *counter = ctl + ctr_slot, *abort_flag = ctl + 1;
    const bool l2 = V.iperm != nullptr && !(V.no_l2 & 1);
    if constexpr (CHAIN) {
        if (t == 0) { s_task = atomicAdd(ctl + C.role_slot, 1); s_word[5] = 0; }
        __syncthreads();
        const int arrival = s_task;
        __syncthreads();
        if (arrival < C.nwg &&
            !df_chain_role(smem, V, nT, C, flags, flags + (int64_t)(nT + 1) * nT + nparts, ctl, epoch, linv_all, info, ldiag, s_word,
                           trace ? trace + (int64_t)(ntasks + nT) * 16 : nullptr))
            return;
    }
    for (;;) {
        if (t == 0) s_task = atomicAdd(counter, 1);
        __syncthreads();
        const int task = s_task;
        if (task >= ntasks) {
            if (q_out == nullptr || task >= ntasks + nbk) return;
            if (trace && t == 0) trace[task * 16 + 0] = wall_clock64();
            if (!df_backward(smem, V, n, nT, bk_list[task - ntasks], bk_ptr, bk_idx, flags, epoch, abort_flag,
                             linv_all, q_out, q_nat, qscale, dz_out)) {
                if (t == 0) *info = -1;
                return;
            }
            if (trace && t == 0) trace[task * 16 + 4] = wall_clock64();
            continue;
        }
        const DfJob jb = tasks[task];
        const int i = jb.i, k = jb.k;
        const bool helper = jb.np < 0;
        const int jend = jb.jhi;
        int *pflags = flags + (int64_t)(nT + 1) * nT;
        int *tflags = pflags + nparts;
        const int nr = i == nT ? 1 : min(NB, n - NB * i);
        const int64_t col0 = (int64_t)NB * k;
        const int nc = min(NB, n - NB * k);
        double *Tik = V.base + V.toff[(int64_t)i * nT + k];
        if (trace && t == 0) trace[task * 16 + 0] = wall_clock64();
        chol_d4 acc[4];
#pragma unroll
        for (int rt = 0; rt < 4; ++rt)
#pragma unroll
            for (int e = 0; e < 4; ++e) {
                const int c = 16 * ty + (tx >> 4) + 4 * e, r = 16 * rt + (tx & 15);
                double v = 0.0;
                if (!helper && r < nr && c < nc) {
                    if (V.S) {
                        const int cn = V.iperm[NB * k + c];
                        if (i == nT) v = (r == 0 && cn >= 0) ? V.S[(int64_t)cn * V.ldS + V.n_nat] : 0.0;
                        else {
                            const int rn = V.iperm[NB * i + r];
                            if (cn >= 0 && rn >= 0) v = rn >= cn ? V.S[(int64_t)cn * V.ldS + rn] : V.S[(int64_t)rn * V.ldS + cn];
                            else v = (i == k && r == c && !(jb.mode & 8)) ? 1.0 : 0.0;
                        }
                    } else v = Tik[(int64_t)c * V.ld + r];
                }
                acc[rt][e] = -v;
            }
        bool alive = true;
        const uint64_t *bi = V.rowbits + (size_t)i * V.W, *bk = V.rowbits + (size_t)k * V.W;
        const int wend = (jend - 1) >> 6;
        auto word = [&](int w) {
            uint64_t m = bi[w] & bk[w];
            if (w == (jb.jlo >> 6)) m &= ~0ull << (jb.jlo & 63);
            if (w == (jend >> 6)) m &= (1ull << (jend & 63)) - 1;
            return m;
        };
        int jw = jb.jlo >> 6;
        uint64_t jm = jend > jb.jlo ? word(jw) : 0ull;
        auto next_j = [&]() -> int {
            for (;;) {
                if (jm) { const int j = 64 * jw + __builtin_ctzll(jm); jm &= jm - 1; return j; }
                if (jend <= jb.jlo || ++jw > wend) return -1;
                jm = word(jw);
            }
        };
        auto spin_both = [&](int j) {
            bool ok = df_spin(flags + (int64_t)k * nT + j, epoch, abort_flag);
            if (ok && i != k) ok = df_spin(flags + (int64_t)i * nT + j, epoch, abort_flag);
            return ok;
        };
        if (nc == NB && (nr == NB || i == k || (V.iperm && i == nT)) && !(V.ld & 1)) {
            df_d2 rp[8], rq[8];
#ifdef DBAT_HIP_PROFILING
            const bool abl_f = (V.no_l2 & 6) == 6;
            const bool abl_q = (V.no_l2 & 6) != 0, abl_p = (V.no_l2 & 4) != 0;
            if (abl_q) for (int q = 0; q < 8; ++q) { rq[q].x = 1e-3 * tx; rq[q].y = 1e-3 * ty; }
            if (abl_p) for (int q = 0; q < 8; ++q) { rp[q].x = 1e-3 * tx; rp[q].y = 1e-3 * ty; }
#else
            constexpr bool abl_q = false, abl_p = false, abl_f = false;
#endif
            int jc = next_j(), jn = -1;
            int f1 = 0, f2 = 0;
            auto look = [&](int j) {
                f1 = f2 = epoch;
                if (t == 0 && j >= 0 && !abl_f) {
                    f1 = __hip_atomic_load(flags + (int64_t)k * nT + j, __ATOMIC_RELAXED, __HIP_MEMORY_SCOPE_AGENT);
                    if (i != k) f2 = __hip_atomic_load(flags + (int64_t)i * nT + j, __ATOMIC_RELAXED, __HIP_MEMORY_SCOPE_AGENT);
                }
            };
            int64_t ok_n = 0, oi_n = 0;
            auto offsets = [&](int j, int64_t &ok_, int64_t &oi_) {
                ok_ = j >= 0 ? V.toff[(int64_t)k * nT + j] : 0;
                oi_ = j >= 0 && i != k ? V.toff[(int64_t)i * nT + j] : 0;
            };
            auto issue = [&](int64_t ok_, int64_t oi_) {
                if (!abl_p) df_tile16_issue(V.base + ok_, V.ld, rp, tx, ty, l2);
                if (i != k && !abl_q) df_tile16_issue(V.base + oi_, V.ld, rq, tx, ty, l2);
            };
            if (jc >= 0) {
                int64_t ok_c, oi_c;
                offsets(jc, ok_c, oi_c);
                jn = next_j();
                offsets(jn, ok_n, oi_n);
                if (t == 0) s_ok = spin_both(jc);
                __syncthreads();
                if (!s_ok) alive = false;
                else {
                    issue(ok_c, oi_c);
                    look(jn);
                }
            }
            while (alive && jc >= 0) {
                const int jnn = jn >= 0 ? next_j() : -1;
                int64_t ok_nn, oi_nn;
                offsets(jnn, ok_nn, oi_nn);
                if (t == 0 && jn >= 0 && (f1 != epoch || f2 != epoch)) look(jn);
                __syncthreads();
                df_tile16_commit<LD>(rp, Pm, tx, ty);
                if (i != k) df_tile16_commit<LD>(rq, Qm, tx, ty);
                if (t == 0) s_ok = jn >= 0 && f1 == epoch && f2 == epoch;
                __syncthreads();
                const bool early = s_ok;
                if (early) { issue(ok_n, oi_n); look(jnn); }
                mfma_tile64<LD>(Pm, i == k ? Pm : Qm, ty, tx, acc);
                if (jn >= 0 && !early) {
                    __syncthreads();
                    if (t == 0) s_ok = spin_both(jn);
                    __syncthreads();
                    if (!s_ok) { alive = false; break; }
                    issue(ok_n, oi_n);
                    look(jnn);
                }
                jc = jn; jn = jnn; ok_n = ok_nn; oi_n = oi_nn;
            }
        } else {
            for (int j = next_j(); j >= 0; j = next_j()) {
                if (t == 0) s_ok = spin_both(j);
                __syncthreads();
                if (!s_ok) { alive = false; break; }
                const double *Lk = V.base + V.toff[(int64_t)k * nT + j] + tx;
                const double *Li = V.base + V.toff[(int64_t)i * nT + j] + tx;
                const bool okc = tx < nc, okr = tx < nr && i != k;
                double vk[16], vi[16];
#pragma unroll
                for (int q = 0; q < 16; ++q) vk[q] = okc ? ld_tile(Lk + (int64_t)(ty + 4 * q) * V.ld, l2) : 0.0;
#pragma unroll
                for (int q = 0; q < 16; ++q) vi[q] = okr ? ld_tile(Li + (int64_t)(ty + 4 * q) * V.ld, l2) : 0.0;
#pragma unroll
                for (int q = 0; q < 16; ++q) { Pm[(ty + 4 * q) * LD + tx] = vk[q]; Qm[(ty + 4 * q) * LD + tx] = vi[q]; }
                __syncthreads();
                mfma_tile64<LD>(Pm, i == k ? Pm : Qm, ty, tx, acc);
            }
        }
        if (!alive) { if (t == 0) *info = -1; return; }
        __syncthreads();
        if (helper) {
            double *slot = parts + (size_t)jb.part * 4096;
#pragma unroll
            for (int rt = 0; rt < 4; ++rt)
#pragma unroll
                for (int e = 0; e < 4; ++e) {
                    const int c = 16 * ty + (tx >> 4) + 4 * e, r = 16 * rt + (tx & 15);
                    st_coh(slot + c * 64 + r, acc[rt][e]);
                }
            if (trace && t == 0) trace[task * 16 + 1] = wall_clock64();
            __builtin_amdgcn_s_waitcnt(0);
            __syncthreads();
            if (t == 0) __hip_atomic_store(pflags + jb.part, epoch, __ATOMIC_RELAXED, __HIP_MEMORY_SCOPE_AGENT);
            if (trace && t == 0) trace[task * 16 + 4] = wall_clock64();
            continue;
        }
        for (int h = 0; h < jb.np; ++h) {
            if (t == 0) s_ok = df_spin(pflags + jb.part + h, epoch, abort_flag);
            __syncthreads();
            if (!s_ok) { if (t == 0) *info = -1; return; }
            const double *slot = parts + (size_t)(jb.part + h) * 4096;
#pragma unroll
            for (int rt = 0; rt < 4; ++rt)
#pragma unroll
                for (int e = 0; e < 4; ++e) {
                    const int c = 16 * ty + (tx >> 4) + 4 * e, r = 16 * rt + (tx & 15);
                    acc[rt][e] += ld_coh(slot + c * 64 + r);
                }
            __syncthreads();
        }
        if (trace && t == 0) trace[task * 16 + 1] = wall_clock64();
        if (jb.mode & 4) {
#pragma unroll
            for (int rt = 0; rt < 4; ++rt)
#pragma unroll
                for (int e = 0; e < 4; ++e) {
                    const int c = 16 * ty + (tx >> 4) + 4 * e, r = 16 * rt + (tx & 15);
                    if (r < nr && c < nc) Tik[(int64_t)c * V.ld + r] = -acc[rt][e];
                }
            __syncthreads();
            continue;
        }
        if (jb.mode == 1 || jb.mode == 16) {
#pragma unroll
            for (int rt = 0; rt < 4; ++rt)
#pragma unroll
                for (int e = 0; e < 4; ++e) {
                    const int c = 16 * ty + (tx >> 4) + 4 * e, r = 16 * rt + (tx & 15);
                    if (r < nr && c < nc) st_coh(Tik + (int64_t)c * V.ld + r, -acc[rt][e]);
                }
            if (trace && t == 0) trace[task * 16 + 3] = wall_clock64();
            __builtin_amdgcn_s_waitcnt(0);
            __syncthreads();
            if (t == 0) __hip_atomic_store(jb.mode == 1 ? tflags + k : C.dflags + k, epoch, __ATOMIC_RELAXED, __HIP_MEMORY_SCOPE_AGENT);
            if (trace && t == 0) trace[task * 16 + 4] = wall_clock64();
            continue;
        }
        double *Linv = linv_all + (size_t)k * NB * NB;
        if (!CHAIN && i == k) {
#pragma unroll
            for (int rt = 0; rt < 4; ++rt)
#pragma unroll
                for (int e = 0; e < 4; ++e) {
                    const int c = 16 * ty + (tx >> 4) + 4 * e, r = 16 * rt + (tx & 15);
                    const double v = -acc[rt][e];
                    smem[c * DF_TLD + r] = (r < nc && c < nc) ? (r >= c ? v : 0.0) : (r == c ? 1.0 : 0.0);
                }
            if (trace && t == 0) trace[task * 16 + 2] = wall_clock64();
            if (trace && t == 0) trace[task * 16 + 14] = (long long)__builtin_readcyclecounter();
            df_potf2(smem, nc, (int)col0, info, trace ? trace + task * 16 : nullptr);
            if (trace && t == 0) trace[task * 16 + 15] = (long long)__builtin_readcyclecounter();
            if (ldiag && ty == 0 && tx < nc) {
                const int zn = V.iperm ? V.iperm[col0 + tx] : (int)(col0 + tx);
                if (zn >= 0) ldiag[zn] = smem[tx * DF_TLD + tx];
            }
            if (jb.mode == 2) {
                __syncthreads();
                const int p = jb.p;
                const int nrp = p == nT ? 1 : min(NB, n - NB * p);
                double *Tpk = V.base + V.toff[(int64_t)p * nT + k];
                if (t == 0) s_ok = df_spin(tflags + k, epoch, abort_flag);
                __syncthreads();
                if (!s_ok) { if (t == 0) *info = -1; return; }
                df_load_tile16<DF_TLD>(Tpk, V.ld, smem, tx, ty, false);
                __syncthreads();
                chol_d4 x[4] = {{0, 0, 0, 0}, {0, 0, 0, 0}, {0, 0, 0, 0}, {0, 0, 0, 0}};
                const double *pq = smem + (tx >> 4) * DF_TLD + 16 * ty + (tx & 15);
                const double *pl = smem + (tx & 15) * DF_TLD + 64 + (tx >> 4);
#pragma unroll
                for (int kk = 0; kk < 16; ++kk) {
                    const double b = pq[4 * kk * DF_TLD];
#pragma unroll
                    for (int cb = 0; cb < 4; ++cb)
                        if (kk < 4 * (cb + 1)) {
                            const double a = pl[16 * cb * DF_TLD + 4 * kk];
                            x[cb] = __builtin_amdgcn_mfma_f64_16x16x4f64(a, b, x[cb], 0, 0, 0);
                        }
                }
#pragma unroll
                for (int cb = 0; cb < 4; ++cb)
#pragma unroll
                    for (int e = 0; e < 4; ++e) {
                        const int c = 16 * cb + (tx >> 4) + 4 * e, r = 16 * ty + (tx & 15);
                        if (r < nrp && c < nc) st_coh(Tpk + (int64_t)c * V.ld + r, x[cb][e]);
                    }
                __builtin_amdgcn_s_waitcnt(0);
                __syncthreads();
                if (t == 0) __hip_atomic_store(flags + (int64_t)p * nT + k, epoch, __ATOMIC_RELAXED, __HIP_MEMORY_SCOPE_AGENT);
            }
#pragma unroll 4
            for (int c = ty; c < NB; c += 4) {
                if (!V.iperm && tx < nc && c < nc && tx >= c) st_coh(Tik + (int64_t)c * V.ld + tx, smem[c * DF_TLD + tx]);
                st_coh(Linv + c * NB + tx, (tx < nc && c < nc && (c >> 4) <= (tx >> 4)) ? smem[tx * DF_TLD + 64 + c] : 0.0);
            }
        } else {
#pragma unroll
            for (int rt = 0; rt < 4; ++rt)
#pragma unroll
                for (int e = 0; e < 4; ++e) {
                    const int c = 16 * ty + (tx >> 4) + 4 * e, r = 16 * rt + (tx & 15);
                    Qm[c * LD + r] = -acc[rt][e];
                }
            if (t == 0) s_ok = df_spin(flags + (int64_t)k * nT + k, epoch, abort_flag);
            __syncthreads();
            if (!s_ok) { if (t == 0) *info = -1; return; }
            if (trace && t == 0) trace[task * 16 + 2] = wall_clock64();
            df_load_tile16<LD>(Linv, NB, Pm, tx, ty, l2);
            __syncthreads();
            {
                chol_d4 x[4] = {{0, 0, 0, 0}, {0, 0, 0, 0}, {0, 0, 0, 0}, {0, 0, 0, 0}};
                mfma_tile64<LD>(Pm, Qm, ty, tx, x);
#pragma unroll
                for (int rt = 0; rt < 4; ++rt)
#pragma unroll
                    for (int e = 0; e < 4; ++e) {
                        const int c = 16 * ty + (tx >> 4) + 4 * e, r = 16 * rt + (tx & 15);
                        if (r < nr && c < nc) st_coh(Tik + (int64_t)c * V.ld + r, x[rt][e]);
                    }
            }
        }
        if (trace && t == 0) trace[task * 16 + 3] = wall_clock64();
        __builtin_amdgcn_s_waitcnt(0);
        __syncthreads();
        if (t == 0) {
            __hip_atomic_store(flags + (int64_t)i * nT + k, epoch, __ATOMIC_RELAXED, __HIP_MEMORY_SCOPE_AGENT);
        }
        if (trace && t == 0) trace[task * 16 + 4] = wall_clock64();
    }
}

__global__ void k_df_reset(int *__restrict__ info, int *__restrict__ ctl, unsigned long long *__restrict__ qflag, int nq) {
    const int i = blockIdx.x * blockDim.x + threadIdx.x;
    if (i == 0) { *info = 0; for (int q = 0; q < 8; ++q) ctl[q] = 0; }
    if (i < nq) qflag[i] = DF_SENTINEL;
}

template <int LD>
__device__ __forceinline__ void si_load(const double *T, double *Pm, int tx, int ty, double sign = 1.0) {
#pragma unroll
    for (int q = 0; q < 16; ++q) { const int c = ty + 4 * q; Pm[c * LD + tx] = sign * T[c * 64 + tx]; }
}
template <int LD>
__device__ __forceinline__ void si_load_T(const double *T, double *Pm, int tx, int ty, double sign = 1.0) {
#pragma unroll
    for (int q = 0; q < 16; ++q) { const int c = ty + 4 * q; Pm[tx * LD + c] = sign * T[c * 64 + tx]; }
}
struct SiTask { int i, k; };
__global__ __launch_bounds__(256) void k_selinv_m(double *__restrict__ tiles, const int64_t *__restrict__ toff, int nT,
                                                  const double *__restrict__ linv_all, const SiTask *__restrict__ tasks) {
    constexpr int LD = DF_LD;
    __shared__ double smem[2 * 64 * LD];
    double *Pm = smem, *Qm = smem + 64 * LD;
    const int tx = threadIdx.x & 63, ty = threadIdx.x >> 6;
    const SiTask tk = tasks[blockIdx.x];
    double *T = tiles + toff[(int64_t)tk.i * nT + tk.k];
    si_load_T<LD>(linv_all + (size_t)tk.k * 4096, Pm, tx, ty);
    si_load<LD>(T, Qm, tx, ty);
    __syncthreads();
    chol_d4 acc[4] = {{0, 0, 0, 0}, {0, 0, 0, 0}, {0, 0, 0, 0}, {0, 0, 0, 0}};
    mfma_tile64<LD>(Pm, Qm, ty, tx, acc);
#pragma unroll
    for (int rt = 0; rt < 4; ++rt)
#pragma unroll
        for (int e = 0; e < 4; ++e) T[(16 * ty + (tx >> 4) + 4 * e) * 64 + 16 * rt + (tx & 15)] = acc[rt][e];
}
__global__ __launch_bounds__(256) void k_selinv_off(double *__restrict__ Z, const double *__restrict__ M, const int64_t *__restrict__ toff,
                                                    int nT, const int *__restrict__ bk_ptr, const int *__restrict__ bk_idx,
                                                    const SiTask *__restrict__ tasks) {
    constexpr int LD = DF_LD;
    __shared__ double smem[2 * 64 * LD];
    double *Pm = smem, *Qm = smem + 64 * LD;
    const int tx = threadIdx.x & 63, ty = threadIdx.x >> 6;
    const SiTask tk = tasks[blockIdx.x];
    const int i = tk.i, k = tk.k;
    chol_d4 acc[4] = {{0, 0, 0, 0}, {0, 0, 0, 0}, {0, 0, 0, 0}, {0, 0, 0, 0}};
    for (int e = bk_ptr[k]; e < bk_ptr[k + 1]; ++e) {
        const int j = bk_idx[e];
        __syncthreads();
        si_load_T<LD>(M + toff[(int64_t)j * nT + k], Pm, tx, ty);
        if (i >= j) si_load<LD>(Z + toff[(int64_t)i * nT + j], Qm, tx, ty);
        else si_load_T<LD>(Z + toff[(int64_t)j * nT + i], Qm, tx, ty);
        __syncthreads();
        mfma_tile64<LD>(Pm, Qm, ty, tx, acc);
    }
    double *T = Z + toff[(int64_t)i * nT + k];
#pragma unroll
    for (int rt = 0; rt < 4; ++rt)
#pragma unroll
        for (int e = 0; e < 4; ++e) T[(16 * ty + (tx >> 4) + 4 * e) * 64 + 16 * rt + (tx & 15)] = -acc[rt][e];
}
__global__ __launch_bounds__(256) void k_selinv_diag(double *__restrict__ Z, const double *__restrict__ M, const int64_t *__restrict__ toff,
                                                     int nT, const int *__restrict__ bk_ptr, const int *__restrict__ bk_idx,
                                                     const double *__restrict__ linv_all, const int *__restrict__ cols) {
    constexpr int LD = DF_LD;
    __shared__ double smem[2 * 64 * LD];
    double *Pm = smem, *Qm = smem + 64 * LD;
    const int tx = threadIdx.x & 63, ty = threadIdx.x >> 6;
    const int k = cols[blockIdx.x];
    chol_d4 acc[4] = {{0, 0, 0, 0}, {0, 0, 0, 0}, {0, 0, 0, 0}, {0, 0, 0, 0}};
    si_load_T<LD>(linv_all + (size_t)k * 4096, Pm, tx, ty);
    __syncthreads();
    mfma_tile64<LD>(Pm, Pm, ty, tx, acc);
    for (int e = bk_ptr[k]; e < bk_ptr[k + 1]; ++e) {
        const int j = bk_idx[e];
        __syncthreads();
        si_load_T<LD>(Z + toff[(int64_t)j * nT + k], Pm, tx, ty);
        si_load_T<LD>(M + toff[(int64_t)j * nT + k], Qm, tx, ty, -1.0);
        __syncthreads();
        mfma_tile64<LD>(Pm, Qm, ty, tx, acc);
    }
    double *T = Z + toff[(int64_t)k * nT + k];
#pragma unroll
    for (int rt = 0; rt < 4; ++rt)
#pragma unroll
        for (int e = 0; e < 4; ++e) T[(16 * ty + (tx >> 4) + 4 * e) * 64 + 16 * rt + (tx & 15)] = acc[rt][e];
}

struct DataflowChol {
    int n = 0, n_nat = 0, nT = 0, W = 0, ntasks = 0, ntiles = 0, epoch = 0, grid = 512;
    bool permuted = false;
    bool reset_done = false;
    bool reset_args(int *&ctl, unsigned long long *&q, int &nq) const {
        if (!permuted || !d_ctl || !d_qperm) return false;
        ctl = d_ctl; q = reinterpret_cast<unsigned long long *>(d_qperm); nq = nT * CHOL_NB;
        return true;
    }
    long long n_products = 0;
    int *d_flags = nullptr, *d_ctl = nullptr, *d_bk_ptr = nullptr, *d_bk_idx = nullptr, *d_iperm = nullptr;
    int64_t *d_toff = nullptr;
    uint64_t *d_rowbits = nullptr;
    DfJob *d_tasks = nullptr, *d_tasksB = nullptr;
    int ntasksB = 0, nbk = 0;
    int *d_bk_list = nullptr;
    uint64_t *d_rowbits_top = nullptr;
    bool two_phase = false;
    int64_t top_tile0 = 0, n_top_tiles = 0;
    std::vector<double> sim_critical_us, sim_schedule_us;
    std::vector<DfJob> h_tasksB;
    DfTask *d_tile_ij = nullptr;
    int nparts = 0;
    bool env_l2 = false;
    int env_df_ablate = 0;
    bool use_chain = false;
    int nchain = 0, nchainB = 0, chain_wg = 0, chain_wgB = 0;
    int *d_chain_cols = nullptr, *d_chain_colsB = nullptr, *d_chain_par = nullptr, *d_chain_bits = nullptr, *d_chain_bitsB = nullptr, *d_chain_pos = nullptr;
    double *d_parts = nullptr;
    double *d_tiles = nullptr, *d_qperm = nullptr;
    double *d_ztiles = nullptr;
    SiTask *d_si_m = nullptr, *d_si_off = nullptr;
    int *d_si_diag = nullptr, *d_perm = nullptr;
    int n_si_m = 0;
    std::vector<int> si_off_ptr, si_diag_ptr;
    std::vector<uint64_t> h_rowbits;
    long long *d_trace = nullptr;
    std::vector<DfJob> h_tasks;
    std::vector<int> perm;
    size_t linv_doubles() const { return (size_t)std::max(nT, 1) * CHOL_NB * CHOL_NB; }

    void release() {
        void *ps[] = {d_flags, d_ctl, d_bk_ptr, d_bk_idx, d_iperm, d_toff, d_rowbits, d_tasks, d_tile_ij, d_tiles, d_qperm, d_parts,
                      d_tasksB, d_bk_list, d_rowbits_top, d_chain_cols, d_chain_colsB, d_chain_par, d_chain_bits, d_chain_bitsB, d_chain_pos,
                      d_ztiles, d_si_m, d_si_off, d_si_diag, d_perm};
        for (void *p : ps) if (p) (void)hipFree(p);
        d_flags = d_ctl = d_bk_ptr = d_bk_idx = d_iperm = nullptr; d_toff = nullptr; d_rowbits = nullptr;
        d_tasks = nullptr; d_tile_ij = nullptr; d_tiles = d_qperm = d_parts = nullptr;
        d_tasksB = nullptr; d_bk_list = nullptr; d_rowbits_top = nullptr;
        d_chain_cols = d_chain_colsB = d_chain_par = d_chain_bits = d_chain_bitsB = d_chain_pos = nullptr;
        d_ztiles = nullptr; d_si_m = d_si_off = nullptr; d_si_diag = d_perm = nullptr; n_si_m = 0;
        si_off_ptr.clear(); si_diag_ptr.clear();
    }
    void dump_trace(hipStream_t stream, const char *path) const {
        if (!d_trace) return;
        std::vector<long long> h((size_t)(ntasks + 3 * nT) * 16);
        (void)hipStreamSynchronize(stream);
        (void)hipMemcpy(h.data(), d_trace, h.size() * sizeof(long long), hipMemcpyDeviceToHost);
        FILE *f = fopen(path, "w");
        if (!f) return;
        for (int t = 0; t < ntasks + nT; ++t) {
            const int i = t < ntasks ? (h_tasks[t].np < 0 ? -(h_tasks[t].i + 2) : h_tasks[t].i) : -1, k = t < ntasks ? h_tasks[t].k : nT - 1 - (t - ntasks);
            fprintf(f, "%d,%d,%d", t, i, k);
            for (int q = 0; q < 16; ++q) fprintf(f, ",%lld", h[(size_t)t * 16 + q]);
            fprintf(f, ",%d,%d,%d\n", t < ntasks ? h_tasks[t].jlo : 0, t < ntasks ? (h_tasks[t].np < 0 ? h_tasks[t].jhi : h_tasks[t].k) : 0,
                    t < ntasks ? h_tasks[t].mode : 0);
        }
        for (int k = 0; k < nT && use_chain; ++k) {
            fprintf(f, "%d,-3,%d", ntasks + nT + k, k);
            for (int q = 0; q < 16; ++q) fprintf(f, ",%lld", h[(size_t)(ntasks + nT + k) * 16 + q]);
            fprintf(f, ",0,0,0\n");
        }
        for (int k = 0; k < nT && use_chain; ++k) {
            fprintf(f, "%d,-4,%d", ntasks + 2 * nT + k, k);
            for (int q = 0; q < 16; ++q) fprintf(f, ",%lld", h[(size_t)(ntasks + 2 * nT + k) * 16 + q]);
            fprintf(f, ",0,0,0\n");
        }
        fclose(f);
    }
    template <class T>
    static bool up(T *&dst, const std::vector<T> &v) {
        if (hipMalloc((void **)&dst, std::max<size_t>(v.size(), 1) * sizeof(T)) != hipSuccess) return false;
        if (!v.empty()) (void)hipMemcpy(dst, v.data(), v.size() * sizeof(T), hipMemcpyHostToDevice);
        return true;
    }
    struct JobList { std::vector<DfJob> jobs; std::vector<int> dptr, dep, own, sumjob, presum, bits, par; };
    void build_jobs(int phase, const std::vector<uint64_t> &rowbits, const std::vector<int> &col_owner, int rank, JobList &L, int merge_depth = 0) {
        auto has = [&](int i, int k) { return (rowbits[(size_t)i * W + (k >> 6)] >> (k & 63)) & 1ull; };
        const int split_min = std::max(env_int("DBAT_HIP_DF_SPLIT", 96), 2);
        const int chunk = std::max(env_int("DBAT_HIP_DF_CHUNK", 32), 1);
        const bool merge = permuted;
        auto top = [&](int k) { return phase != 0 && col_owner[k] < 0; };
        auto mine = [&](int k) { return phase == 0 || col_owner[k] == rank; };
        int dom_lo = nT, dom_hi = 0;
        if (phase == 1) for (int k = 0; k < nT; ++k) if (col_owner[k] == rank) { dom_lo = std::min(dom_lo, k); dom_hi = k + 1; }
        if (dom_hi <= dom_lo) dom_lo = dom_hi = 0;
        L.jobs.clear(); L.dptr.assign(1, 0); L.dep.clear();
        L.own.assign((size_t)(nT + 1) * nT, -1); L.sumjob.assign(nT, -1);
        L.presum.assign(nT, -1); L.bits.assign(nT, 0); L.par.assign(nT, -1);
        const bool chain = use_chain && merge;
        auto inphase = [&](int c) { return c < nT && (phase == 0 || (phase == 1 ? col_owner[c] == rank : col_owner[c] < 0)); };
        std::vector<int> js;
        const int merge_min = 4;
        int merge_k = 0;
        int run0 = 0;
        std::vector<int> run_of(nT, 0), merge_cut;
        for (int k = 0; k < nT; ++k) {
            if (chain && merge_depth > 0) {
                if (!(k > 0 && (L.bits[k - 1] & 2))) { run0 = k; merge_cut.clear(); }
                run_of[k] = run0;
                int c = run0 - 1;
                while (c >= 0 && L.par[c] != k) --c;
                if (c >= 0) { merge_cut.assign({run_of[c], c + 1, run0}); merge_k = k; }
                else if (k - merge_k >= merge_depth) merge_cut.clear();
            }
            auto emit = [&](int i, int mode, int par, int jhi_owner) {
                auto push_products = [&](int q0, int q1) {
                    for (int q = q0; q < q1; ++q) { L.dep.push_back(L.own[(size_t)k * nT + js[q]]); L.dep.push_back(i != k ? L.own[(size_t)i * nT + js[q]] : -1); }
                    L.dptr.push_back((int)L.dep.size());
                };
                n_products += (long long)js.size();
                const int nj = (int)js.size();
                const int nch = nj > split_min ? (nj + chunk - 1) / chunk : 1;
                if (nch == 1 && !merge_cut.empty()) {
                    int qc[4], npc = 0, q0 = 0;
                    for (int c : merge_cut) {
                        const int q = (int)(std::lower_bound(js.begin(), js.end(), c) - js.begin());
                        if (q > q0) { qc[npc++] = q; q0 = q; }
                    }
                    if (npc > 0 && nj - q0 >= merge_min) {
                        q0 = 0;
                        for (int c = 0; c < npc; ++c) {
                            L.jobs.push_back(DfJob{i, k, js[q0], qc[c] < nj ? js[qc[c]] : jhi_owner, nparts + c, -1, 0, -1});
                            push_products(q0, qc[c]);
                            q0 = qc[c];
                        }
                        const int me = (int)L.jobs.size();
                        L.jobs.push_back(DfJob{i, k, q0 < nj ? js[q0] : jhi_owner, jhi_owner, nparts, npc, mode, i == k ? par : -1});
                        push_products(q0, nj);
                        nparts += npc;
                        return me;
                    }
                }
                for (int c = 0; c + 1 < nch; ++c) {
                    L.jobs.push_back(DfJob{i, k, js[chunk * c], js[chunk * (c + 1)], nparts + c, -1, 0, -1});
                    push_products(chunk * c, chunk * (c + 1));
                }
                const int me = (int)L.jobs.size();
                L.jobs.push_back(DfJob{i, k, nch > 1 ? js[chunk * (nch - 1)] : (nj ? js[0] : jhi_owner), jhi_owner, nparts, nch - 1, mode, i == k ? par : -1});
                push_products(chunk * (nch - 1), nj);
                nparts += nch - 1;
                return me;
            };
            if (phase == 1 && top(k)) {
                for (int i = k; i <= nT; ++i) {
                    if (!has(i, k)) continue;
                    js.clear();
                    for (int j = dom_lo; j < std::min(dom_hi, k); ++j) if (has(i, j) && has(k, j)) js.push_back(j);
                    emit(i, rank == 0 ? 4 : 12, -1, std::min(dom_hi, k));
                }
                continue;
            }
            if (phase == 1 ? !mine(k) : (phase == 2 && !top(k))) continue;
            auto products = [&](int i) {
                js.clear();
                for (int j = 0; j < k; ++j) if (has(i, j) && has(k, j) && (phase != 2 || top(j))) js.push_back(j);
            };
            int par = -1;
            if (merge) for (int i = k + 1; i <= nT && par < 0; ++i) if (has(i, k)) par = i;
            if (par >= 0) { products(par); L.sumjob[k] = emit(par, 1, -1, k); }
            products(k);
            L.par[k] = par;
            if (chain) {
                const bool cont = k > 0 && (L.bits[k - 1] & 2) != 0;
                if (cont) js.pop_back();
                L.presum[k] = emit(k, 16, -1, cont ? k - 1 : k);
                js.clear();
                L.bits[k] = (cont ? 1 : 0) | ((par == k + 1 && k + 1 < nT && inphase(k + 1)) ? 2 : 0);
            }
            L.own[(size_t)k * nT + k] = emit(k, par >= 0 ? 2 : 0, par, k);
            if (par >= 0) L.own[(size_t)par * nT + k] = L.own[(size_t)k * nT + k];
            for (int i = k + 1; i <= nT; ++i)
                if (has(i, k) && i != par) { products(i); L.own[(size_t)i * nT + k] = emit(i, 0, -1, k); }
        }
    }
    void order_jobs(JobList &L, const char *what) {
        std::vector<DfJob> &jobs = L.jobs;
        const std::vector<int> &dptr = L.dptr, &dep = L.dep, &own = L.own, &sumjob = L.sumjob;
        const int nt = (int)jobs.size();
        if (nt == 0) return;
        auto is_helper = [&](int t) { return jobs[t].np < 0; };
        auto is_share = [&](int t) { return (jobs[t].mode & 4) != 0; };
        auto is_diag = [&](int t) { return jobs[t].np >= 0 && jobs[t].i == jobs[t].k && !is_share(t) && jobs[t].mode != 16; };
        auto nprod_of = [&](int t) { return (dptr[t + 1] - dptr[t]) / 2; };
        auto for_deps = [&](int t, const std::function<void(int)> &f) {
            for (int q = dptr[t]; q < dptr[t + 1]; ++q) if (dep[q] >= 0) f(dep[q]);
            if (!is_helper(t)) {
                for (int h = 1; h <= jobs[t].np; ++h) f(t - h);
                if (jobs[t].mode == 0 && jobs[t].i != jobs[t].k) f(own[(size_t)jobs[t].k * nT + jobs[t].k]);
                if (jobs[t].mode == 2) f(sumjob[jobs[t].k]);
                if (is_diag(t) && L.presum[jobs[t].k] >= 0) {
                    f(L.presum[jobs[t].k]);
                    if (L.bits[jobs[t].k] & 1) f(own[(size_t)(jobs[t].k - 1) * nT + jobs[t].k - 1]);
                }
            }
        };
        const double c_prod = 2.5, c_diag = 13.5, c_off = 4.5, c_hop = 2.0, c_add = 1.5, c_help = 2.0;
        auto tail_of = [&](int t) { return is_helper(t) || is_share(t) || jobs[t].mode == 1 || jobs[t].mode == 16 ? c_help : (is_diag(t) ? c_diag + (jobs[t].mode == 2 ? 2.5 : 0.0) : c_off); };
        std::vector<double> est(nt, 0.0), fin(nt, 0.0);
        for (int t = 0; t < nt; ++t) {
            double e = 0.0;
            for_deps(t, [&](int d) { e = std::max(e, fin[d]); });
            est[t] = e;
            fin[t] = e + c_hop + (nprod_of(t) ? c_prod : 0.0) + tail_of(t);
        }
        std::vector<double> blev(nt, 0.0);
        for (int t = nt - 1; t >= 0; --t) {
            blev[t] += c_hop + c_prod + tail_of(t);
            for_deps(t, [&](int d) { blev[d] = std::max(blev[d], blev[t]); });
        }
        const int workers = std::max(1, std::min(grid, 256));
        auto simulate = [&](const std::vector<int> &ord) {
            std::vector<double> done(nt, 0.0);
            std::priority_queue<double, std::vector<double>, std::greater<double>> freeat;
            for (int w = 0; w < workers; ++w) freeat.push(0.0);
            double last = 0.0;
            for (int t : ord) {
                double tc = freeat.top(); freeat.pop();
                for (int q = dptr[t]; q + 1 < dptr[t + 1]; q += 2) {
                    double av = done[dep[q]];
                    if (dep[q + 1] >= 0) av = std::max(av, done[dep[q + 1]]);
                    tc = std::max(tc, av + c_hop) + c_prod;
                }
                if (!is_helper(t)) {
                    for (int h = jobs[t].np; h >= 1; --h) tc = std::max(tc, done[t - h] + c_hop) + c_add;
                    if (jobs[t].mode == 0 && jobs[t].i != jobs[t].k) tc = std::max(tc, done[own[(size_t)jobs[t].k * nT + jobs[t].k]] + c_hop);
                    if (jobs[t].mode == 2) tc = std::max(tc, done[sumjob[jobs[t].k]] + c_hop - c_diag);
                    if (is_diag(t) && L.presum[jobs[t].k] >= 0) {
                        tc = std::max(tc, done[L.presum[jobs[t].k]] + c_hop);
                        if (L.bits[jobs[t].k] & 1) tc = std::max(tc, done[own[(size_t)(jobs[t].k - 1) * nT + jobs[t].k - 1]]);
                    }
                }
                tc += tail_of(t);
                done[t] = tc; last = std::max(last, tc);
                freeat.push(tc);
            }
            return last;
        };
        std::vector<int> indeg0(nt, 0), sptr(nt + 1, 0), succ;
        for (int t = 0; t < nt; ++t) for_deps(t, [&](int d) { ++indeg0[t]; ++sptr[d + 1]; });
        for (int t = 0; t < nt; ++t) sptr[t + 1] += sptr[t];
        succ.resize(sptr[nt]);
        {
            std::vector<int> fill(sptr.begin(), sptr.end() - 1);
            for (int t = 0; t < nt; ++t) for_deps(t, [&](int d) { succ[fill[d]++] = t; });
        }
        auto kahn = [&](const std::vector<double> &key) {
            std::vector<int> ord(nt), indeg(indeg0);
            typedef std::pair<double, int> KI;
            std::priority_queue<KI, std::vector<KI>, std::greater<KI>> pq;
            for (int t = 0; t < nt; ++t) if (!indeg[t]) pq.push(KI(key[t], t));
            size_t n_out = 0;
            while (!pq.empty()) {
                const int t = pq.top().second; pq.pop();
                ord[n_out++] = t;
                for (int q = sptr[t]; q < sptr[t + 1]; ++q) if (--indeg[succ[q]] == 0) pq.push(KI(key[succ[q]], succ[q]));
            }
            return ord;
        };
        const double betas[] = {0.0, 0.25, 0.5, 1.0, 2.0, 4.0, 1e6};
        const int ncand = (int)(sizeof(betas) / sizeof(betas[0])) + 1;
        std::vector<int> best_ord;
        double tbest = 1e300;
        int best = -1;
        std::vector<double> key(nt), tcs(ncand);
        const int forced = env_int("DBAT_HIP_DF_ORDER", -1);
        for (int c = 0; c < ncand; ++c) {
            if (quiet && forced < 0 && c != 0 && c != 3) { tcs[c] = 1e300; continue; }
            if (c + 1 < ncand) for (int t = 0; t < nt; ++t) key[t] = est[t] - betas[c] * blev[t];
            else for (int t = 0; t < nt; ++t) key[t] = est[t] - c_prod * nprod_of(t);
            std::vector<int> ord = kahn(key);
            tcs[c] = simulate(ord);
            if (forced == c || (forced < 0 && tcs[c] < tbest)) { tbest = tcs[c]; best = c; best_ord.swap(ord); }
        }
        double cp = 0.0;
        for (int t = 0; t < nt; ++t) cp = std::max(cp, fin[t]);
        sim_critical_us.push_back(cp); sim_schedule_us.push_back(tbest);
        if (stats_on()) {
            fprintf(stderr, "[chol %s] %d tasks, critical path %.0f us; simulated with %d workgroups, key = earliest start - beta x bottom level:",
                    what, nt, cp, workers);
            for (int c = 0; c + 1 < ncand; ++c) fprintf(stderr, " beta %g: %.0f us,", betas[c], tcs[c]);
            fprintf(stderr, " earliest start - own work: %.0f us -> candidate %d\n", tcs[ncand - 1], best);
        }
        std::vector<DfJob> sorted(nt);
        for (int t = 0; t < nt; ++t) sorted[t] = jobs[best_ord[t]];
        jobs.swap(sorted);
    }
    struct Sched { std::vector<int> colsA, colsB, bitsA, bitsB, par, pos, bkl, bptr, bidx; std::vector<uint64_t> rowbits_top; };
    bool quiet = false;
    bool stats_on() const { return !quiet && env_on("DBAT_HIP_PLAN_STATS"); }
    void schedule_host(const std::vector<uint64_t> &rowbits, const std::vector<int> &col_owner, int rank, Sched &H) {
        auto has = [&](int i, int k) { return (rowbits[(size_t)i * W + (k >> 6)] >> (k & 63)) & 1ull; };
        if (const char *g = env_get("DBAT_HIP_DF_GRID")) grid = std::min(std::max(atoi(g), 1), 4096);
        nparts = 0; n_products = 0;
        two_phase = !col_owner.empty();
        h_rowbits = rowbits;
        use_chain = permuted && env_int("DBAT_HIP_DF_CHAIN", 1) != 0;
        if (use_chain && !two_phase && !env_get("DBAT_HIP_DF_CHAIN")) {
            long long nprod = 0;
            int longest = 0, cur = 0;
            for (int k = 0; k < nT; ++k) {
                int par = -1;
                for (int i = k; i <= nT; ++i) {
                    if (!has(i, k)) continue;
                    if (i > k && par < 0) par = i;
                    for (int w = 0; w < W; ++w) {
                        uint64_t m = rowbits[(size_t)i * W + w] & rowbits[(size_t)k * W + w];
                        if (w == (k >> 6)) m &= (1ull << (k & 63)) - 1;
                        else if (w > (k >> 6)) m = 0;
                        nprod += __builtin_popcountll(m);
                    }
                }
                cur = (k > 0 && cur > 0) ? cur : 1;
                longest = std::max(longest, cur);
                cur = par == k + 1 ? cur + 1 : 0;
            }
            const double t_products = (double)nprod * 2.6 / std::min(grid, 256), t_chain = longest * 17.0;
            use_chain = t_products < 0.6 * t_chain;
            if (stats_on())
                fprintf(stderr, "[chol] %lld tile products (%.0f us over the workgroups), longest chain %d links (%.0f us): chain role %s\n",
                        nprod, t_products, longest, t_chain, use_chain ? "on" : "off");
        }
        auto split_chain = [&](JobList &L, std::vector<DfJob> &tasks, std::vector<int> &cols) {
            tasks.clear(); cols.clear();
            for (const DfJob &j : L.jobs) {
                if (use_chain && j.np >= 0 && j.i == j.k && (j.mode == 0 || j.mode == 2)) cols.push_back(j.k);
                else tasks.push_back(j);
            }
        };
        auto chain_width = [&](const std::vector<int> &cols, const std::vector<int> &bits) {
            int runs = 0;
            for (int k : cols) runs += !(bits[k] & 1);
            return std::max(1, std::min(runs, env_int("DBAT_HIP_DF_CHAIN_WG", 32)));
        };
        std::vector<int> &colsA = H.colsA, &colsB = H.colsB;
        sim_critical_us.clear(); sim_schedule_us.clear();
        JobList L;
        std::vector<int> &bkl = H.bkl;
        bkl.clear(); h_tasksB.clear(); ntasksB = 0; nchain = nchainB = 0; chain_wg = chain_wgB = 0;
        if (!two_phase) {
            build_jobs(0, rowbits, col_owner, rank, L);
            order_jobs(L, "all");
            const int force_merge = env_int("DBAT_HIP_DF_MERGE", -1);
            if (use_chain && force_merge != 0) {
                const int np0 = nparts;
                const long long prod0 = n_products;
                JobList M;
                nparts = 0; n_products = 0;
                build_jobs(0, rowbits, col_owner, rank, M, 2);
                order_jobs(M, "all, sums cut at the merge columns");
                const bool better = nparts <= 4096 && (force_merge == 1 || sim_schedule_us[1] < 0.99 * sim_schedule_us[0]);
                if (better) std::swap(L, M); else { nparts = np0; n_products = prod0; }
                sim_critical_us.erase(sim_critical_us.begin() + (better ? 0 : 1)); sim_schedule_us.erase(sim_schedule_us.begin() + (better ? 0 : 1));
                if (stats_on()) fprintf(stderr, "[chol] sums cut at the merge columns: %s (%d partial sums)\n", better ? "yes" : "no", nparts);
            }
            split_chain(L, h_tasks, colsA); ntasks = (int)h_tasks.size();
            for (int j = nT - 1; j >= 0; --j) bkl.push_back(j);
        } else {
            build_jobs(1, rowbits, col_owner, rank, L);
            order_jobs(L, "domain");
            split_chain(L, h_tasks, colsA); ntasks = (int)h_tasks.size();
            JobList B;
            build_jobs(2, rowbits, col_owner, rank, B);
            order_jobs(B, "top");
            split_chain(B, h_tasksB, colsB); ntasksB = (int)h_tasksB.size();
            if (use_chain) {
                for (int k = 0; k < nT; ++k) if (B.par[k] >= 0) L.par[k] = B.par[k];
                nchainB = (int)colsB.size(); chain_wgB = chain_width(colsB, B.bits);
                H.bitsB = B.bits;
            }
            for (int j = nT - 1; j >= 0; --j) if (col_owner[j] < 0) bkl.push_back(j);
            for (int j = nT - 1; j >= 0; --j) if (col_owner[j] == rank) bkl.push_back(j);
            H.rowbits_top = rowbits;
            for (int i = 0; i <= nT; ++i)
                for (int k = 0; k < nT; ++k)
                    if (col_owner[k] >= 0) H.rowbits_top[(size_t)i * W + (k >> 6)] &= ~(1ull << (k & 63));
        }
        nbk = (int)bkl.size();
        if (use_chain) {
            nchain = (int)colsA.size(); chain_wg = chain_width(colsA, L.bits);
            H.pos.assign(nT, 0);
            for (size_t q = 0; q < colsA.size(); ++q) H.pos[colsA[q]] = (int)q;
            for (size_t q = 0; q < colsB.size(); ++q) H.pos[colsB[q]] = (int)q;
            H.bitsA = L.bits; H.par = L.par;
            if (stats_on()) {
                int runs = 0, longest = 0, cur = 0;
                for (int k = 0; k < nT; ++k) { if (L.bits[k] & 1) ++cur; else { cur = 1; } longest = std::max(longest, cur); }
                for (int k : colsA) runs += !(L.bits[k] & 1);
                fprintf(stderr, "[chol] chain role: %d diagonal tiles in %d chains (longest %d), %d workgroups%s\n", nchain, runs, longest, chain_wg,
                        two_phase ? " (domain)" : "");
            }
        }
        H.bptr.assign(nT + 1, 0); H.bidx.clear();
        for (int j = 0; j < nT; ++j) {
            for (int i = nT - 1; i > j; --i)
                if (has(i, j)) H.bidx.push_back(i);
            H.bptr[j + 1] = (int)H.bidx.size();
        }
    }
    bool finish_setup(const std::vector<uint64_t> &rowbits, const std::vector<int64_t> &toff,
                      const std::vector<int> &col_owner = std::vector<int>(), int rank = 0) {
        Sched H;
        schedule_host(rowbits, col_owner, rank, H);
        if (two_phase) {
            if (!up(d_tasksB, h_tasksB) || !up(d_rowbits_top, H.rowbits_top)) return false;
            if (use_chain && (!up(d_chain_colsB, H.colsB) || !up(d_chain_bitsB, H.bitsB))) return false;
        }
        if (use_chain && (!up(d_chain_cols, H.colsA) || !up(d_chain_bits, H.bitsA) || !up(d_chain_par, H.par) || !up(d_chain_pos, H.pos))) return false;
        if (env_on("DBAT_HIP_DF_TRACE") && !two_phase && hipMalloc(&d_trace, (size_t)(ntasks + 3 * nT) * 16 * sizeof(long long)) != hipSuccess) d_trace = nullptr;
        if (!up(d_tasks, h_tasks) || !up(d_bk_ptr, H.bptr) || !up(d_bk_idx, H.bidx) || !up(d_rowbits, rowbits) || !up(d_toff, toff) || !up(d_bk_list, H.bkl))
            return false;
        if (hipMalloc(&d_flags, ((size_t)(nT + 1) * nT + (size_t)nparts + 4 * (size_t)nT) * sizeof(int)) != hipSuccess) return false;
        if (nparts > 0 && hipMalloc(&d_parts, (size_t)nparts * 4096 * sizeof(double)) != hipSuccess) return false;
        if (hipMalloc(&d_ctl, 8 * sizeof(int)) != hipSuccess) return false;
        (void)hipMemset(d_flags, 0, ((size_t)(nT + 1) * nT + (size_t)nparts + 4 * (size_t)nT) * sizeof(int));
        (void)hipMemset(d_ctl, 0, 8 * sizeof(int));
        env_l2 = env_int("DBAT_HIP_DF_L2", 0) != 0;
        env_df_ablate = 2 * (env_int("DBAT_HIP_DF_ABLATE", 0) & 3);
        epoch = 0;
        return true;
    }
    bool setup_inplace(const CholEnvelope &env, int64_t lda) {
        release();
        permuted = false; perm.clear();
        n = n_nat = env.n; nT = (n + CHOL_NB - 1) / CHOL_NB; W = (nT + 64) / 64;
        std::vector<uint64_t> rb((size_t)(nT + 1) * W, 0);
        std::vector<int64_t> toff((size_t)(nT + 1) * nT, -1);
        for (int i = 0; i <= nT; ++i) {
            const int kf = i < nT ? env.panel_first[i] / CHOL_NB : 0;
            for (int k = kf; k <= std::min(i, nT - 1); ++k) {
                rb[(size_t)i * W + (k >> 6)] |= 1ull << (k & 63);
                toff[(size_t)i * nT + k] = (int64_t)CHOL_NB * k * lda + (i == nT ? (int64_t)n : (int64_t)CHOL_NB * i);
            }
        }
        return finish_setup(rb, toff);
    }
    struct Symbolic {
        std::vector<int> iperm, col_owner;
        std::vector<uint64_t> rb;
        std::vector<int64_t> toff;
        std::vector<DfTask> tile_ij;
    };
    struct PatternStats { int etree_depth = 0, longest_run = 0; long long products = 0; };
    PatternStats pattern_stats(const std::vector<uint64_t> &rb) const {
        PatternStats st;
        std::vector<int> depth(nT, 1);
        int cur = 0;
        for (int k = 0; k < nT; ++k) {
            int par = -1;
            for (int i = k + 1; i < nT; ++i) {
                if (!((rb[(size_t)i * W + (k >> 6)] >> (k & 63)) & 1ull)) continue;
                if (par < 0) par = i;
                for (int w = 0; w <= (k >> 6); ++w) {
                    uint64_t m = rb[(size_t)i * W + w] & rb[(size_t)k * W + w];
                    if (w == (k >> 6)) m &= (1ull << (k & 63)) - 1;
                    st.products += __builtin_popcountll(m);
                }
            }
            for (int w = 0; w <= (k >> 6); ++w) {
                uint64_t m = rb[(size_t)k * W + w];
                if (w == (k >> 6)) m &= (1ull << (k & 63)) - 1;
                st.products += __builtin_popcountll(m);
            }
            st.etree_depth = std::max(st.etree_depth, depth[k]);
            if (par >= 0) depth[par] = std::max(depth[par], depth[k] + 1);
            cur = cur > 0 ? cur : 1;
            st.longest_run = std::max(st.longest_run, cur);
            cur = par == k + 1 ? cur + 1 : 0;
        }
        return st;
    }
    bool setup_permuted(int nc, int nio, const uint64_t *adj, int adj_words, const NdTree &nd, int rank) {
        release();
        Symbolic Y;
        symbolic_permuted(nc, nio, adj, adj_words, nd, Y);
        const std::vector<int> &block_end = nd.block_end;
        if (!up(d_tile_ij, Y.tile_ij) || !up(d_iperm, Y.iperm)) return false;
        if (hipMalloc(&d_tiles, (size_t)ntiles * 4096 * sizeof(double)) != hipSuccess) return false;
        (void)hipMemset(d_tiles, 0, (size_t)ntiles * 4096 * sizeof(double));
        if (hipMalloc(&d_qperm, (size_t)nT * CHOL_NB * sizeof(double)) != hipSuccess) return false;
        if (env_on("DBAT_HIP_PLAN_STATS"))
            fprintf(stderr, "[chol] order %d (%d with block padding, %zu blocks), %d tile rows, %d tiles (%.1f MB), dense lower triangle would be %d tiles\n",
                    n_nat, n, block_end.size(), nT, ntiles, ntiles * 32768.0 / 1e6, nT * (nT + 1) / 2 + nT);
        if (env_on("DBAT_HIP_PLAN_STATS")) {
            fprintf(stderr, "[chol] cameras per block, last (root separator) first:");
            for (size_t b = block_end.size(); b-- > 0 && block_end.size() - b <= 24;)
                fprintf(stderr, " %d", block_end[b] - (b ? block_end[b - 1] : 0));
            fprintf(stderr, "\n");
        }
        if (env_on("DBAT_HIP_PLAN_STATS") && !Y.col_owner.empty()) {
            int ntop = 0, nmine = 0;
            for (int k = 0; k < nT; ++k) { ntop += Y.col_owner[k] < 0; nmine += Y.col_owner[k] == rank; }
            fprintf(stderr, "[chol] rank %d of %d: %d tile columns in its domain, %d top columns, %lld top tiles (%.1f MB summed over the ranks per factorisation)\n",
                    rank, nd.nparts, nmine, ntop, (long long)n_top_tiles, n_top_tiles * 32768.0 / 1e6);
        }
        return finish_setup(Y.rb, Y.toff, Y.col_owner, rank);
    }
    void symbolic_permuted(int nc, int nio, const uint64_t *adj, int adj_words, const NdTree &nd, Symbolic &Y) {
        permuted = true;
        n_nat = 6 * nc + nio;
        const std::vector<int> &order = nd.order, &block_end = nd.block_end;
        std::vector<int> rowpos(nc);
        int off = 0;
        {
            const bool pad_all = env_on("DBAT_HIP_ND_PAD_ALL");
            size_t b = 0; int q0 = 0;
            for (int q = 0; q < nc; ++q) {
                if (q == q0) {
                    const int sep_rows = 6 * (block_end[b] - q0), used = off % CHOL_NB;
                    const bool saves = used > 0 && (used + sep_rows + CHOL_NB - 1) / CHOL_NB < 1 + (sep_rows + CHOL_NB - 1) / CHOL_NB;
                    const int join_small = env_int("DBAT_HIP_ND_JOIN_SMALL", 2 * CHOL_NB);
                    const bool joins = !pad_all && (saves || (used > 0 && sep_rows <= join_small)) && b > 0 && b < nd.block_sep.size() && nd.block_sep[b] &&
                                       nd.block_owner[b] == nd.block_owner[b - 1];
                    if (!joins) off = (off + CHOL_NB - 1) / CHOL_NB * CHOL_NB;
                }
                rowpos[order[q]] = off; off += 6;
                while (b < block_end.size() && block_end[b] <= q + 1) { q0 = q + 1; ++b; }
            }
        }
        const int io0 = nio > 0 ? (off + CHOL_NB - 1) / CHOL_NB * CHOL_NB : off;
        n = (io0 + nio + CHOL_NB - 1) / CHOL_NB * CHOL_NB;
        nT = n / CHOL_NB; W = (nT + 64) / 64;
        perm.assign(n_nat, 0);
        std::vector<int> &iperm = Y.iperm;
        iperm.assign((size_t)n, -1);
        for (int c = 0; c < nc; ++c)
            for (int a = 0; a < 6; ++a) perm[6 * c + a] = rowpos[c] + a;
        for (int u = 0; u < nio; ++u) perm[6 * nc + u] = io0 + u;
        for (int z = 0; z < n_nat; ++z) iperm[perm[z]] = z;
        auto pos6 = [&](int c) { return rowpos[c]; };
        std::vector<uint64_t> &rb = Y.rb;
        rb.assign((size_t)(nT + 1) * W, 0);
        auto setbit = [&](int i, int k) { rb[(size_t)i * W + (k >> 6)] |= 1ull << (k & 63); };
        for (int a = 0; a < nc; ++a) {
            const int ta0 = pos6(a) / CHOL_NB, ta1 = (pos6(a) + 5) / CHOL_NB;
            for (int w = 0; w < adj_words; ++w) {
                uint64_t m = adj[(size_t)a * adj_words + w];
                while (m) {
                    const int b = 64 * w + __builtin_ctzll(m);
                    m &= m - 1;
                    if (b >= nc) break;
                    const int tb0 = pos6(b) / CHOL_NB, tb1 = (pos6(b) + 5) / CHOL_NB;
                    for (int ti = ta0; ti <= ta1; ++ti)
                        for (int tj = tb0; tj <= tb1; ++tj) setbit(std::max(ti, tj), std::min(ti, tj));
                }
            }
            for (int ti = ta0; ti <= ta1; ++ti) for (int tj = ta0; tj <= ti; ++tj) setbit(ti, tj);
        }
        for (int i = 0; i < nT; ++i) setbit(i, i);
        for (int i = io0 / CHOL_NB; i < nT && nio > 0; ++i) for (int k = 0; k <= i; ++k) setbit(i, k);
        for (int k = 0; k < nT; ++k) setbit(nT, k);
        {
            std::vector<int> rows;
            for (int k = 0; k < nT; ++k) {
                rows.clear();
                for (int i = k + 1; i <= nT; ++i) if ((rb[(size_t)i * W + (k >> 6)] >> (k & 63)) & 1ull) rows.push_back(i);
                for (size_t a = 0; a < rows.size(); ++a)
                    for (size_t b = 0; b <= a; ++b)
                        if (rows[b] < nT) setbit(rows[a], rows[b]);
            }
        }
        std::vector<int> &col_owner = Y.col_owner;
        col_owner.clear();
        if (nd.nparts > 1) {
            col_owner.assign(nT, -1);
            size_t b = 0;
            for (int q = 0; q < nc; ++q) {
                while (b < block_end.size() && block_end[b] <= q) ++b;
                const int ow = b < nd.block_owner.size() ? nd.block_owner[b] : -1;
                for (int t = rowpos[order[q]] / CHOL_NB; t <= (rowpos[order[q]] + 5) / CHOL_NB; ++t) col_owner[t] = ow;
            }
        }
        std::vector<int64_t> &toff = Y.toff;
        std::vector<DfTask> &tile_ij = Y.tile_ij;
        toff.assign((size_t)(nT + 1) * nT, -1); tile_ij.clear();
        for (int pass = 0; pass < 2; ++pass) {
            if (pass == 1) top_tile0 = (int64_t)tile_ij.size();
            for (int k = 0; k < nT; ++k) {
                if ((!col_owner.empty() && col_owner[k] < 0) != (pass == 1)) continue;
                for (int i = k; i <= nT; ++i)
                    if ((rb[(size_t)i * W + (k >> 6)] >> (k & 63)) & 1ull) {
                        toff[(size_t)i * nT + k] = (int64_t)tile_ij.size() * 4096;
                        tile_ij.push_back(DfTask{i, k});
                    }
            }
        }
        ntiles = (int)tile_ij.size();
        n_top_tiles = ntiles - top_tile0;
    }
    bool selinv_supported() const { return permuted && !two_phase; }
    bool selected_inverse(hipStream_t stream, const double *linv_work) {
        if (!d_ztiles) {
            auto has = [&](int i, int k) { return (h_rowbits[(size_t)i * W + (k >> 6)] >> (k & 63)) & 1ull; };
            std::vector<SiTask> mt, off;
            std::vector<int> level(nT, 0), diag;
            int nlev = 0;
            for (int k = nT - 1; k >= 0; --k) {
                int lv = 0;
                for (int i = k + 1; i < nT; ++i) if (has(i, k)) { lv = std::max(lv, level[i] + 1); mt.push_back(SiTask{i, k}); }
                level[k] = lv; nlev = std::max(nlev, lv + 1);
            }
            si_off_ptr.assign(nlev + 1, 0); si_diag_ptr.assign(nlev + 1, 0);
            for (int lv = 0; lv < nlev; ++lv) {
                for (int k = nT - 1; k >= 0; --k) {
                    if (level[k] != lv) continue;
                    diag.push_back(k);
                    for (int i = k + 1; i < nT; ++i) if (has(i, k)) off.push_back(SiTask{i, k});
                }
                si_off_ptr[lv + 1] = (int)off.size(); si_diag_ptr[lv + 1] = (int)diag.size();
            }
            n_si_m = (int)mt.size();
            if (!up(d_si_m, mt) || !up(d_si_off, off) || !up(d_si_diag, diag) || !up(d_perm, perm)) return false;
            if (hipMalloc(&d_ztiles, (size_t)ntiles * 4096 * sizeof(double)) != hipSuccess) { d_ztiles = nullptr; return false; }
        }
        if (n_si_m > 0)
            hipLaunchKernelGGL(k_selinv_m, dim3(n_si_m), dim3(256), 0, stream, d_tiles, d_toff, nT, linv_work, d_si_m);
        for (size_t lv = 0; lv + 1 < si_off_ptr.size(); ++lv) {
            const int no = si_off_ptr[lv + 1] - si_off_ptr[lv], nd = si_diag_ptr[lv + 1] - si_diag_ptr[lv];
            if (no > 0)
                hipLaunchKernelGGL(k_selinv_off, dim3(no), dim3(256), 0, stream, d_ztiles, (const double *)d_tiles, d_toff, nT, d_bk_ptr,
                                   d_bk_idx, d_si_off + si_off_ptr[lv]);
            if (nd > 0)
                hipLaunchKernelGGL(k_selinv_diag, dim3(nd), dim3(256), 0, stream, d_ztiles, (const double *)d_tiles, d_toff, nT, d_bk_ptr,
                                   d_bk_idx, linv_work, d_si_diag + si_diag_ptr[lv]);
        }
        return true;
    }
    int selinv_levels() const { return (int)si_off_ptr.size() - 1; }
    void solve(hipStream_t stream, double *A, int64_t lda, double *q_out, double *linv_work, int *info_dev,
               double *ldiag = nullptr, const double *qscale = nullptr, double *dz_out = nullptr) {
        if (d_trace) (void)hipMemsetAsync(d_trace, 0, (size_t)(ntasks + 3 * nT) * 16 * sizeof(long long), stream);
        ++epoch;
        DfView V;
        V.toff = d_toff; V.rowbits = d_rowbits; V.W = W; V.no_l2 = (env_l2 ? 0 : 1) | env_df_ablate;
        double *qflag;
        V.S = nullptr; V.ldS = lda; V.n_nat = n_nat;
        if (permuted) {
            if (!reset_done)
                hipLaunchKernelGGL(k_df_reset, dim3((nT * CHOL_NB + 255) / 256), dim3(256), 0, stream, info_dev, d_ctl,
                                   reinterpret_cast<unsigned long long *>(d_qperm), nT * CHOL_NB);
            reset_done = false;
            V.base = d_tiles; V.ld = 64; V.iperm = d_iperm; qflag = d_qperm; V.S = A;
        } else {
            (void)hipMemsetAsync(info_dev, 0, sizeof(int), stream);
            (void)hipMemsetAsync(d_ctl, 0, 8 * sizeof(int), stream);
            V.base = A; V.ld = lda; V.iperm = nullptr; qflag = q_out;
            (void)hipMemsetAsync(q_out, 0xFF, (size_t)n * sizeof(double), stream);
        }
        if (permuted && use_chain)
            hipLaunchKernelGGL(k_chol_df<true>, dim3(chain_grid(ntasks + nT, chain_wg)), dim3(256), 0, stream, V, n, nT, d_tasks, ntasks,
                               d_flags, d_ctl, epoch, linv_work, info_dev, d_trace, d_bk_ptr, d_bk_idx, qflag, q_out, ldiag,
                               qscale, dz_out, d_parts, nparts, d_bk_list, nbk, 0, chain_arg(0));
        else
            hipLaunchKernelGGL(k_chol_df<false>, dim3(std::min(grid, ntasks + nT)), dim3(256), 0, stream, V, n, nT, d_tasks, ntasks,
                               d_flags, d_ctl, epoch, linv_work, info_dev, d_trace, d_bk_ptr, d_bk_idx, qflag, q_out, ldiag,
                               qscale, dz_out, d_parts, nparts, d_bk_list, nbk, 0, DfChain{});
    }
    DfChain chain_arg(int which) const {
        DfChain C;
        int *dfl = d_flags + (size_t)(nT + 1) * nT + nparts + nT;
        C.cols = which ? d_chain_colsB : d_chain_cols; C.ncols = which ? nchainB : nchain;
        C.par = d_chain_par; C.bits = which ? d_chain_bitsB : d_chain_bits;
        C.dflags = dfl; C.claim = dfl + nT; C.giveup = dfl + 2 * nT; C.pos = d_chain_pos;
        C.nwg = which ? chain_wgB : chain_wg;
        C.ctr_slot = which ? 5 : 3; C.role_slot = which ? 6 : 4;
        C.trace_potf2 = env_int("DBAT_HIP_DF_TRACE_POTF2", 0);
        return C;
    }
    int chain_grid(int work, int wg) const { return std::max(std::min(grid, work + wg), wg + 1); }
    double *top_tiles() const { return d_tiles + top_tile0 * 4096; }
    int64_t top_tiles_count() const { return n_top_tiles * 4096; }
    void solve_domain(hipStream_t stream, double *A, int64_t lda, double *linv_work, int *info_dev, double *ldiag) {
        ++epoch;
        DfView V;
        V.toff = d_toff; V.rowbits = d_rowbits; V.W = W; V.no_l2 = (env_l2 ? 0 : 1) | env_df_ablate;
        V.ldS = lda; V.n_nat = n_nat; V.base = d_tiles; V.ld = 64; V.iperm = d_iperm; V.S = A;
        hipLaunchKernelGGL(k_df_reset, dim3((nT * CHOL_NB + 255) / 256), dim3(256), 0, stream, info_dev, d_ctl,
                           reinterpret_cast<unsigned long long *>(d_qperm), nT * CHOL_NB);
        if (ntasks > 0 && use_chain)
            hipLaunchKernelGGL(k_chol_df<true>, dim3(chain_grid(ntasks, chain_wg)), dim3(256), 0, stream, V, n, nT, d_tasks, ntasks,
                               d_flags, d_ctl, epoch, linv_work, info_dev, (long long *)nullptr, d_bk_ptr, d_bk_idx, (double *)nullptr,
                               (double *)nullptr, ldiag, (const double *)nullptr, (double *)nullptr, d_parts, nparts, d_bk_list, 0, 0, chain_arg(0));
        else if (ntasks > 0)
            hipLaunchKernelGGL(k_chol_df<false>, dim3(std::min(grid, ntasks)), dim3(256), 0, stream, V, n, nT, d_tasks, ntasks,
                               d_flags, d_ctl, epoch, linv_work, info_dev, (long long *)nullptr, d_bk_ptr, d_bk_idx, (double *)nullptr,
                               (double *)nullptr, ldiag, (const double *)nullptr, (double *)nullptr, d_parts, nparts, d_bk_list, 0, 0, DfChain{});
    }
    void solve_top(hipStream_t stream, int64_t lda, double *q_out, double *linv_work, int *info_dev, double *ldiag,
                   const double *qscale, double *dz_out) {
        DfView V;
        V.toff = d_toff; V.rowbits = d_rowbits_top; V.W = W; V.no_l2 = 1;
        V.ldS = lda; V.n_nat = n_nat; V.base = d_tiles; V.ld = 64; V.iperm = d_iperm; V.S = nullptr;
        if (use_chain)
            hipLaunchKernelGGL(k_chol_df<true>, dim3(chain_grid(ntasksB + nbk, chain_wgB)), dim3(256), 0, stream, V, n, nT, d_tasksB, ntasksB,
                               d_flags, d_ctl, epoch, linv_work, info_dev, (long long *)nullptr, d_bk_ptr, d_bk_idx, d_qperm, q_out, ldiag,
                               qscale, dz_out, d_parts, nparts, d_bk_list, nbk, 2, chain_arg(1));
        else
            hipLaunchKernelGGL(k_chol_df<false>, dim3(std::min(grid, ntasksB + nbk)), dim3(256), 0, stream, V, n, nT, d_tasksB, ntasksB,
                               d_flags, d_ctl, epoch, linv_work, info_dev, (long long *)nullptr, d_bk_ptr, d_bk_idx, d_qperm, q_out, ldiag,
                               qscale, dz_out, d_parts, nparts, d_bk_list, nbk, 2, DfChain{});
    }
};

inline void df_score_order(int nc, int nio, const uint64_t *adj, int adj_words, const NdTree &T, NdScore &sc) {
    DataflowChol D;
    D.quiet = true;
    DataflowChol::Symbolic Y;
    D.symbolic_permuted(nc, nio, adj, adj_words, T, Y);
    const DataflowChol::PatternStats st = D.pattern_stats(Y.rb);
    sc.cams = nc; sc.blocks = (int)T.block_end.size(); sc.tile_cols = D.nT; sc.tiles = D.ntiles;
    sc.chain = st.etree_depth; sc.run = st.longest_run; sc.products = st.products;
    if (st.products > 1000000) {
        sc.model = 1;
        sc.model_us = std::max(st.etree_depth * 17.0, (double)st.products * 2.6 / std::min(D.grid, 256));
    } else {
        DataflowChol::Sched H;
        D.schedule_host(Y.rb, std::vector<int>(), 0, H);
        sc.model = 0;
        sc.model_us = D.sim_schedule_us.empty() ? 0.0 : D.sim_schedule_us[0];
    }
}

}
```

dbat_amd/csrc/debug_host.hpp:

```cpp
#pragma once

extern "C" {
#define DBAT_PLAN_FIELDS(X)                                                                                           \
    X(x2z) X(io_src) X(io_fixed) X(z_est) X(z_prw) X(z_prv) X(z_mine) X(z0) X(prior_z) X(porder) X(pt_rank) X(o_cam)    \
    X(o_pt) X(o_uv) X(o_w) X(o_seg) X(o_row) X(batch_start) X(o_lc) X(o_pidx) X(tile_batch) X(tile_cam_start)           \
    X(tile_order) X(tile_cams) X(cm_pt) X(cm_uv) X(cm_w) X(cm_chunk_cam) X(cm_chunk_start) X(giant_start)               \
    X(tile_io_start) X(tile_iocols) X(tile_cam_io) X(tile_io_simple) X(sg_chunk) X(sg_tile_chunk0) X(sg_lc) X(sg_gcam)  \
    X(sg_uv) X(sg_w) X(cam_w) X(cam_ncol) X(cam_col) X(cam_iorow) X(cam_eo_est) X(px) X(cam_first) X(cam_adj)
int dbat_hip_debug_plan_digest(const dbat_hip_problem *prob, uint64_t *out, int32_t n_out, char *names, int32_t names_len) {
    API_TRY
    if (!prob || !out) { g_err = "null argument"; return DBAT_HIP_EINVAL; }
    Plan P;
    if (!build_plan(*prob, P, true)) { g_err = P.err; return DBAT_HIP_EINVAL; }
    auto fnv = [](const void *p, size_t n) {
        uint64_t h = 1469598103934665603ull;
        const unsigned char *b = (const unsigned char *)p;
        for (size_t i = 0; i < n; ++i) h = (h ^ b[i]) * 1099511628211ull;
        return h ^ (uint64_t)n;
    };
    std::vector<uint64_t> hs;
    std::string nm;
#define X(F) hs.push_back(fnv(P.F.data(), P.F.size() * sizeof(P.F[0]))); nm += #F ",";
    DBAT_PLAN_FIELDS(X)
#undef X
    hs.push_back(fnv(P.nd.order.data(), P.nd.order.size() * sizeof(int))); nm += "nd.order,";
    hs.push_back(fnv(P.nd.block_end.data(), P.nd.block_end.size() * sizeof(int))); nm += "nd.block_end,";
    hs.push_back(fnv(P.nd.cam_owner.data(), P.nd.cam_owner.size() * sizeof(int))); nm += "nd.cam_owner,";
    const int64_t sc[] = {P.n, P.m, P.NS, P.NZ, P.nIOu, P.pt_lo, P.pt_hi, P.CMAX, P.nb_tiled, P.n_cm_chunks_tiled, P.sg_kmax, P.sg_rows_max,
                          P.sg_ngroups, P.sg_npoints, P.sg_ok, P.sg_backsub_ok, P.BT, P.ncolmax, P.with_io, P.uniform_w, P.all_std8, P.max_k,
                          P.shared_eo, P.rank_ok, P.order_dims, P.mg_subtree, P.n_tiles_io_simple, P.n_prior[0], P.n_prior[1], P.n_prior[2]};
    hs.push_back(fnv(sc, sizeof(sc))); nm += "scalars";
    if ((int)hs.size() > n_out) { g_err = "digest buffer too small"; return DBAT_HIP_EINVAL; }
    for (size_t i = 0; i < hs.size(); ++i) out[i] = hs[i];
    for (int i = (int)hs.size(); i < n_out; ++i) out[i] = 0;
    if (names && names_len > 0) snprintf(names, (size_t)names_len, "%s", nm.c_str());
    return (int)hs.size();
    API_CATCH
}

int dbat_hip_debug_heavy_plan_selftest(const dbat_hip_problem *prob, double *out) {
    API_TRY
    if (!prob || !out) { g_err = "null argument"; return DBAT_HIP_EINVAL; }
    Plan P;
    if (!build_plan(*prob, P, true)) { g_err = P.err; return DBAT_HIP_EINVAL; }
    for (int i = 0; i < 8; ++i) out[i] = 0.0;
    if (!P.hv_ok) return DBAT_HIP_OK;
    const int64_t NS = P.NS;
    if (NS > 4000) { g_err = "selftest: reduced system too large for the dense host check"; return DBAT_HIP_EINVAL; }
    auto val = [](int64_t pt, int64_t row, int c) {
        uint64_t h = (uint64_t)pt * 0x9E3779B97F4A7C15ull ^ (uint64_t)(row + 1) * 0xC2B2AE3D27D4EB4Full ^ (uint64_t)(c + 1) * 0x165667B19E3779F9ull;
        h ^= h >> 29; h *= 0xBF58476D1CE4E5B9ull; h ^= h >> 32;
        return (double)(int64_t)(h % 2001) / 1000.0 - 1.0;
    };
    std::vector<double> Zs((size_t)P.hv_z_doubles, 0.0);
    std::vector<double> ref((size_t)(NS + 1) * (NS + 1), 0.0), got((size_t)(NS + 1) * (NS + 1), 0.0);
    const int64_t ho0 = P.hv_obs0, ho1 = (int64_t)P.o_cam.size();
    std::vector<int64_t> prow; std::vector<double> pval;
    int64_t o = ho0;
    while (o < ho1) {
        const int32_t pt = P.o_pt[o];
        const int32_t hp = pt - P.hv_pt0;
        prow.clear(); pval.clear();
        std::vector<int32_t> slot_row((size_t)(P.hv_pt_io0[hp + 1] - P.hv_pt_io0[hp]), -1);
        int64_t oe = o;
        for (; oe < ho1 && P.o_pt[oe] == pt; ++oe) {
            const int32_t c = P.o_cam[oe];
            const int32_t dst = P.hv_obs_dst[oe - ho0];
            const int ld = P.hv_obs_ld[oe - ho0];
            for (int a = 0; a < 6; ++a) {
                const int64_t row = P.cam_col[(size_t)c * MAXCOL + a];
                prow.push_back(row);
                for (int k = 0; k < 3; ++k) { const double v = val(pt, row, k); pval.push_back(v); Zs[(size_t)dst + (size_t)k * ld + a] = v; }
            }
            for (int q = 6; q < P.cam_ncol[c]; ++q) {
                const int sl = P.hv_obs_ioloc[(size_t)(oe - ho0) * Plan::HV_NIOC + (q - 6)];
                if (sl >= (int)slot_row.size()) { g_err = "selftest: IO slot out of range"; return DBAT_HIP_EINVAL; }
                const int32_t row = P.cam_col[(size_t)c * MAXCOL + q];
                if (slot_row[sl] >= 0 && slot_row[sl] != row) { g_err = "selftest: two IO columns in one slot"; return DBAT_HIP_EINVAL; }
                slot_row[sl] = row;
            }
        }
        for (size_t sl = 0; sl < slot_row.size(); ++sl) {
            if (slot_row[sl] < 0) { g_err = "selftest: IO slot without a column"; return DBAT_HIP_EINVAL; }
            const int gs = P.hv_pt_io0[hp] + (int)sl;
            if (P.hv_io_pt[gs] != hp) { g_err = "selftest: IO slot of another point"; return DBAT_HIP_EINVAL; }
            prow.push_back(slot_row[sl]);
            for (int k = 0; k < 3; ++k) { const double v = val(pt, slot_row[sl], k); pval.push_back(v); Zs[(size_t)P.hv_io_dst[gs] + (size_t)k * P.hv_io_ld[gs]] = v; }
        }
        prow.push_back(NS);
        for (int k = 0; k < 3; ++k) { const double v = val(pt, NS, k); pval.push_back(v); Zs[(size_t)P.hv_pt_y[2 * hp] + (size_t)k * P.hv_pt_y[2 * hp + 1]] = v; }
        for (size_t a = 0; a < prow.size(); ++a)
            for (size_t b = 0; b < prow.size(); ++b) {
                const int64_t ri = prow[a], rj = prow[b];
                if (ri < rj || (ri == NS && rj == NS)) continue;
                ref[(size_t)rj * (NS + 1) + ri] -= pval[3 * a] * pval[3 * b] + pval[3 * a + 1] * pval[3 * b + 1] + pval[3 * a + 2] * pval[3 * b + 2];
            }
        o = oe;
    }
    int64_t nks_all = 0;
    for (int t = 0; t < P.hv_ntasks; ++t) {
        const int gi = P.hv_task[4 * t], gj = P.hv_task[4 * t + 1], ks0 = P.hv_task[4 * t + 2], nks = P.hv_task[4 * t + 3];
        const int nbi = P.hv_grp_nb[gi], nbj = P.hv_grp_nb[gj];
        nks_all += nks;
        std::vector<double> acc((size_t)48 * 48, 0.0);
        for (int ks = 0; ks < nks; ++ks)
            for (int kk = 0; kk < 4; ++kk) {
                const int32_t *op = P.hv_ops.data() + ((size_t)(ks0 + ks) * 4 + kk) * 2;
                if ((op[0] < 0) != (op[1] < 0)) { g_err = "selftest: half an operand"; return DBAT_HIP_EINVAL; }
                if (op[0] < 0) continue;
                for (int i = 0; i < 16 * nbi; ++i)
                    for (int j = 0; j < 16 * nbj; ++j) acc[(size_t)i * 48 + j] += Zs[(size_t)op[0] + i] * Zs[(size_t)op[1] + j];
            }
        for (int i = 0; i < 16 * nbi; ++i)
            for (int j = 0; j < 16 * nbj; ++j) {
                if (gi == gj && i < j) continue;
                const int32_t ri = P.hv_grp_row[(size_t)gi * 48 + i], cj = P.hv_grp_row[(size_t)gj * 48 + j];
                if (ri < 0 || cj < 0 || cj == NS) continue;
                if (ri < cj) { g_err = "selftest: rows of the groups are not ascending"; return DBAT_HIP_EINVAL; }
                got[(size_t)cj * (NS + 1) + ri] -= acc[(size_t)i * 48 + j];
            }
    }
    double dmax = 0, vmax = 0; int64_t ncmp = 0;
    for (size_t i = 0; i < ref.size(); ++i) {
        dmax = std::max(dmax, std::fabs(ref[i] - got[i])); vmax = std::max(vmax, std::fabs(ref[i]));
        ncmp += ref[i] != 0.0;
    }
    out[0] = 1; out[1] = P.hv_npts; out[2] = P.hv_ngroups; out[3] = P.hv_ntasks; out[4] = (double)nks_all;
    out[5] = dmax; out[6] = vmax; out[7] = (double)ncmp;
    return DBAT_HIP_OK;
    API_CATCH
}

int dbat_hip_debug_batch_stats(const dbat_hip_problem *prob, int64_t *out) {
    API_TRY
    if (!prob || !out) { g_err = "null argument"; return DBAT_HIP_EINVAL; }
    Plan P;
    if (!build_plan(*prob, P, true)) { g_err = P.err; return DBAT_HIP_EINVAL; }
    for (int i = 0; i < 16; ++i) out[i] = 0;
    const int64_t nb = (int64_t)P.batch_start.size() - 1;
    for (int64_t b = 0; b < nb; ++b) {
        const int64_t o0 = P.batch_start[b], o1 = P.batch_start[b + 1];
        if (o1 <= o0) continue;
        int64_t *st = out + (b < P.nb_tiled ? 0 : 4);
        st[0] = std::max<int64_t>(st[0], (int64_t)P.o_pidx[o1 - 1] + 1);
        st[1] = std::max<int64_t>(st[1], o1 - o0);
    }
    out[2] = P.nb_pcap[0]; out[6] = P.nb_pcap[1];
    for (size_t t = 0; P.nb_tiled > 0 && t + 1 < P.tile_batch.size(); ++t)
        out[3] = std::max<int64_t>(out[3], P.tile_batch[t + 1] - P.tile_batch[t]);
    out[8] = P.BT; out[9] = Plan::PMAX; out[10] = P.tile_bmax; out[11] = P.nb_tiled; out[12] = nb - P.nb_tiled;
    return DBAT_HIP_OK;
    API_CATCH
}

int dbat_hip_debug_nd_stats(const dbat_hip_problem *prob, int32_t mode, double *out) {
    API_TRY
    if (!prob || !out || mode < 0 || mode > 2) { g_err = "null argument or mode not 0, 1, 2"; return DBAT_HIP_EINVAL; }
    Plan P;
    if (!build_plan(*prob, P, false)) { g_err = P.err; return DBAT_HIP_EINVAL; }
    const bool nd_off = env_on("DBAT_HIP_ND_OFF");
    const int nparts = P.mg_subtree ? P.nranks : 1;
    auto put = [&](const NdTree &T, NdScore sc, int m, double *o) {
        if (sc.mode != m) df_score_order(P.nc, P.nIOu, P.cam_adj.data(), P.cam_adj_words, T, sc);
        const double v[12] = {(double)sc.cams, (double)sc.blocks, (double)sc.tile_cols, (double)sc.tiles, (double)sc.chain, (double)sc.products,
                              sc.model_us, (double)m, (double)nd_check(P.nc, P.cam_adj.data(), P.cam_adj_words, T), (double)sc.run, (double)sc.model, 0.0};
        std::copy(v, v + 12, o);
    };
    NdTree T;
    nd_build(P.nc, P.cam_adj.data(), P.cam_adj_words, P.nd_xyz.data(), P.nd_weight.data(), nparts, P.nd_leaf, nd_off, mode, T);
    put(T, NdScore(), mode, out);
    NdScore sc[3];
    const int chosen = nd_select(P.nc, P.nIOu, P.cam_adj.data(), P.cam_adj_words, P.nd_xyz.data(), P.nd_weight.data(), nparts, P.nd_leaf, nd_off,
                                 -1, true, T, sc);
    put(T, sc[chosen], chosen, out + 12);
    return DBAT_HIP_OK;
    API_CATCH
}

int dbat_hip_debug_model_eval_host(int32_t model, int32_t nK, int32_t nP, const double *EO6, const double *IO,
                                   double px_size, const double *Q3, const double *uv, double *r2,
                                   double *A12, double *B6, double *C ) {
    if (model < 2 || model > 5 || nK < 0 || nK > MAXK || nP < 0 || nP > MAXP) { g_err = "bad model"; return DBAT_HIP_EINVAL; }
    CamRec c{};
    c.c[0] = EO6[0]; c.c[1] = EO6[1]; c.c[2] = EO6[2];
    cam_rotation(EO6 + 3, c.Mt, c.sk, c.ck);
    c.f = IO[0]; c.pp[0] = IO[1]; c.pp[1] = IO[2]; c.b[0] = IO[3]; c.b[1] = IO[4];
    for (int k = 0; k < nK; ++k) c.K[k] = IO[5 + k];
    for (int k = 0; k < nP; ++k) c.P[k] = IO[5 + nK + k];
    c.sz = px_size;
    double r[2], A[2][6], B[2][3], Cf[2][MAXIO];
    switch (model) {
        case 2: obs_eval<2, true, true>(c, nK, nP, Q3, uv[0], uv[1], r, A, B, Cf); break;
        case 3: obs_eval<3, true, true>(c, nK, nP, Q3, uv[0], uv[1], r, A, B, Cf); break;
        case 4: obs_eval<4, true, true>(c, nK, nP, Q3, uv[0], uv[1], r, A, B, Cf); break;
        default: obs_eval<5, true, true>(c, nK, nP, Q3, uv[0], uv[1], r, A, B, Cf); break;
    }
    r2[0] = r[0]; r2[1] = r[1];
    for (int k = 0; k < 6; ++k) { A12[2 * k] = A[0][k]; A12[2 * k + 1] = A[1][k]; }
    for (int k = 0; k < 3; ++k) { B6[2 * k] = B[0][k]; B6[2 * k + 1] = B[1][k]; }
    for (int k = 0; k < 5 + nK + nP; ++k) { C[2 * k] = Cf[0][k]; C[2 * k + 1] = Cf[1][k]; }
    return DBAT_HIP_OK;
}
}
```

dbat_amd/csrc/env.hpp:

```cpp
#pragma once
#include <cstdlib>
#include <cstring>
#include <string>

extern char **environ;

namespace dbat {

#ifdef DBAT_HIP_PROFILING
constexpr bool kProfilingBuild = true;
#else
constexpr bool kProfilingBuild = false;
#endif

struct EnvSwitch { const char *name; bool measurement; const char *what; const char *values = nullptr; };
static const EnvSwitch kEnvSwitches[] = {
    {"DBAT_HIP_SIG", false, "0: signature kernels off, 2: on wherever a chunk's rows fit (default: by group length)", "0|1|2"},
    {"DBAT_HIP_SIG_IOS_OFF", false, "self-calibration: IO rows by LDS atomics in every tile"},
    {"DBAT_HIP_CMAX", false, "cameras per tile (0: column-list kernel only)"},
    {"DBAT_HIP_BT", false, "observations per batch (128 | 256)", "128|256"},
    {"DBAT_HIP_TILE_BMIN", false, "fewest batches a tile may be capped at (default 2)"},
    {"DBAT_HIP_HEAVY", false, "0: heavy / giant points by the column-list kernels (pair terms by global atomics) instead of the matrix-core path", "0|1"},
    {"DBAT_HIP_HEAVY_KS", false, "heavy / giant points: k-steps per task of k_heavy_syrk at most (default: by the amount of work, 12 ... 96)"},
    {"DBAT_HIP_GIANT_THREADS", false, "threads of the giant-point kernels (64 | 128 | 256)", "64|128|256"},
    {"DBAT_HIP_MG_REPLICATED", false, "several ranks: envelope summed, replicated factorisation"},
    {"DBAT_HIP_ND_OFF", false, "no nested dissection"},
    {"DBAT_HIP_ND_LEAF", false, "leaf size of the dissection"},
    {"DBAT_HIP_ND_SEP", false, "separators inside a domain: 0 = lower boundary at the median, 1 = minimum vertex cover at the median, 2 = minimum cover with slid cuts (default: the one the model of the factorisation prefers)", "0|1|2"},
    {"DBAT_HIP_ND_PAD_ALL", false, "every block of the dissection on a tile boundary"},
    {"DBAT_HIP_ND_JOIN_SMALL", false, "separators up to that many rows join their child's last tile"},
    {"DBAT_HIP_DF_SPLIT", false, "factorisation: helper tasks for sums longer than this many products (default 96)"},
    {"DBAT_HIP_DF_CHUNK", false, "factorisation: products per helper task (default 32)"},
    {"DBAT_HIP_DF_CHAIN", false, "factorisation: 0 = diagonal tiles as ordinary tasks (no chain role), 1 = chain role whatever the pattern", "0|1"},
    {"DBAT_HIP_DF_MERGE", false, "factorisation: sums of the columns where two parts of the dissection meet cut into early and late pieces: 0 = never, 1 = wherever the chain role is on (default: where the simulated schedule is shorter)", "0|1"},
    {"DBAT_HIP_DF_CHAIN_WG", false, "factorisation: workgroups of the chain role at most (default 32)"},
    {"DBAT_HIP_DF_L2", false, "factorisation: 1 = finished tiles of the compact layout are read through the L2", "0|1"},
    {"DBAT_HIP_COV_DENSE", false, "posterior covariance: the dense inverse of the reduced system (rocsolver_dpotri) instead of the selected inversion"},
    {"DBAT_HIP_SPRANK_OFF", false, "structural rank from the counting conditions only"},
    {"DBAT_HIP_PLAN_THREADS", false, "threads of the host plan (default: hardware concurrency, at most 32)"},
    {"DBAT_HIP_PLAN_GRAIN", false, "elements per thread below which a pass of the host plan is not split (tests: 1)"},
    {"DBAT_HIP_PLAN_STATS", false, "1: print layout statistics, 2: also the wall time of every section of the plan"},
    {"DBAT_HIP_PIVOT_STATS", false, "print the pivot extremes and the rcond estimate of every solve"},
    {"DBAT_HIP_ABLATE", true, "k_build_sig / tile kernels: switch phases off (results are wrong), phase clocks"},
    {"DBAT_HIP_DF_TRACE", true, "per-task clocks of the factorisation, written to this file"},
    {"DBAT_HIP_DF_TRACE_POTF2", true, "with DF_TRACE: clocks inside the chain role's factorisations as well"},
    {"DBAT_HIP_DF_ABLATE", true, "factorisation: operand tiles of the products not fetched (1: L(i,j), 2: both, 3: and no flag looks) -- timing only, wrong results", "0|1|2|3"},
    {"DBAT_HIP_DF_ORDER", true, "one of the candidate task orders instead of the simulated best"},
    {"DBAT_HIP_DF_GRID", true, "workgroups of the factorisation"},
    {"DBAT_HIP_GRID_OBS", true, "launch size of the observation-parallel kernels"},
};

inline const char *env_get(const char *name) {
    for (const EnvSwitch &e : kEnvSwitches)
        if (!strcmp(e.name, name)) return (e.measurement && !kProfilingBuild) ? nullptr : getenv(name);
    return nullptr;
}
inline int env_int(const char *name, int dflt) { const char *e = env_get(name); return e ? atoi(e) : dflt; }
inline bool env_on(const char *name) { return env_get(name) != nullptr; }

inline bool env_validate(std::string &err) {
    for (char **p = environ; p && *p; ++p) {
        if (strncmp(*p, "DBAT_HIP_", 9) != 0) continue;
        const char *eq = strchr(*p, '=');
        const std::string name(*p, eq ? (size_t)(eq - *p) : strlen(*p));
        const EnvSwitch *hit = nullptr;
        for (const EnvSwitch &e : kEnvSwitches) if (name == e.name) hit = &e;
        if (!hit) { err = "unknown environment variable " + name + " (the switches of libdbat_hip.so: csrc/env.hpp, DESIGN.md 9)"; return false; }
        if (hit->measurement && !kProfilingBuild) {
            err = name + " is a measurement switch (" + hit->what + "): this library was built without -DDBAT_HIP_PROFILING (make -C dbat_amd/csrc prof)";
            return false;
        }
        if (hit->values && eq) {
            const std::string val(eq + 1), list = std::string("|") + hit->values + "|";
            if (val.empty() || val.find('|') != std::string::npos || list.find("|" + val + "|") == std::string::npos) {
                err = name + "=" + val + ": not one of " + hit->values + " (" + hit->what + ")";
                return false;
            }
        }
    }
    return true;
}

}
```

include/dbat_hip.h:

```cpp
#ifndef DBAT_HIP_H
#define DBAT_HIP_H

#include <stdint.h>

#ifdef __cplusplus
extern "C" {
#endif

#define DBAT_HIP_ABI_VERSION 5

#define DBAT_HIP_OK            0
#define DBAT_HIP_EINVAL       -101
#define DBAT_HIP_EUNSUPPORTED -102
#define DBAT_HIP_EDEVICE      -103
#define DBAT_HIP_ENOMEM       -104

#define DBAT_HIP_DAMP_GM   0
#define DBAT_HIP_DAMP_GNA  1
#define DBAT_HIP_DAMP_LM   2
#define DBAT_HIP_DAMP_LMP  3

typedef struct dbat_hip_handle dbat_hip_handle;

typedef struct dbat_hip_problem {
    int32_t abi_version;
    int32_t n_images;
    int32_t n_points;
    int64_t n_obs;
    int32_t dist_model;
    int32_t nK, nP;

    const int32_t *ip_cam;
    const int32_t *ip_pt;
    const double  *ip_val;
    const double  *ip_std;

    const double  *IO_val;
    const double  *px_size;
    const double  *EO_val;
    const double  *OP_val;

    const uint8_t *est_IO;
    const uint8_t *est_EO;
    const uint8_t *est_OP;
    const int32_t *IO_block;
    const int32_t *EO_block;

    const uint8_t *prior_IO_use; const double *prior_IO_val; const double *prior_IO_std;
    const uint8_t *prior_EO_use; const double *prior_EO_val; const double *prior_EO_std;
    const uint8_t *prior_OP_use; const double *prior_OP_val; const double *prior_OP_std;

    int32_t device;
    int32_t shard_rank;
    int32_t shard_count;
} dbat_hip_problem;

typedef int32_t (*dbat_hip_term_fn)(void *user, const double *Jp, const double *r, int64_t n_residuals);
typedef int32_t (*dbat_hip_veto_fn)(void *user, const double *x, int64_t n_params);
typedef void (*dbat_hip_trace_fn)(void *user, int32_t damping, int32_t iter, double res_norm, double damp, int32_t step_type, double rho);

typedef struct dbat_hip_options {
    int32_t damping;
    int32_t max_iter;
    double  conv_tol;
    int32_t abs_term;
    int32_t singular_test;
    int32_t store_trace;
    double  mu;
    double  alpha_min;
    double  lambda0;
    double  lambda_min;
    double  rho_bad;
    double  rho_good;
    double  delta0;
    dbat_hip_term_fn term_fun;
    void   *term_user;
    dbat_hip_veto_fn veto_fun;
    void   *veto_user;
    dbat_hip_trace_fn trace_fun;
    void   *trace_user;
} dbat_hip_options;

typedef struct dbat_hip_result {
    int32_t code;
    int32_t iters;
    int32_t n_res;
    int32_t n_damp;
    int32_t n_trace;
    double  sigma0;
    double  time_s;
    int32_t n_residual_evals;
    int32_t n_linearizations;
    int32_t n_solves;
    int32_t n_trace_only;
    double  stage_s[5];
} dbat_hip_result;

const char *dbat_hip_last_error(void);
int  dbat_hip_abi_version(void);

int  dbat_hip_default_options(int32_t damping, dbat_hip_options *opt);


int  dbat_hip_plan(const dbat_hip_problem *prob, int64_t *n_params, int64_t *n_residuals,
                   int64_t *n_io, int64_t *n_eo, int64_t *n_op,
                   int64_t *shard_pt_lo, int64_t *shard_pt_hi);

int  dbat_hip_plan_structural_rank_ok(const dbat_hip_problem *prob, int32_t *ok);

int  dbat_hip_plan_point_owner(const dbat_hip_problem *prob, int32_t *owner );

int  dbat_hip_plan_serialize(const dbat_hip_problem *prob, double *x0);

int  dbat_hip_create(const dbat_hip_problem *prob, dbat_hip_handle **out);
void dbat_hip_destroy(dbat_hip_handle *h);

int  dbat_hip_structure_key(const dbat_hip_problem *prob, uint64_t *key );
int  dbat_hip_handle_key(const dbat_hip_handle *h, uint64_t *key );
int  dbat_hip_set_values(dbat_hip_handle *h, const dbat_hip_problem *prob);

int64_t dbat_hip_num_params(const dbat_hip_handle *h);
int64_t dbat_hip_num_residuals(const dbat_hip_handle *h);

int  dbat_hip_serialize(const dbat_hip_handle *h, double *x );
int  dbat_hip_deserialize(const dbat_hip_handle *h, const double *x,
                          double *IO , double *EO , double *OP );
int  dbat_hip_structural_rank_ok(const dbat_hip_handle *h, int32_t *ok);


int  dbat_hip_residual(dbat_hip_handle *h, const double *x, double *r_unweighted, double *f);

int  dbat_hip_jacobian_blocks(dbat_hip_handle *h, const double *x,
                              double *JEO, double *JOP, double *JIO);


int  dbat_hip_linearize_solve(dbat_hip_handle *h, const double *x, double lambda,
                              int32_t scale_columns, double *p, double *stats);

int  dbat_hip_gradient(dbat_hip_handle *h, double *g);
int  dbat_hip_colnorms(dbat_hip_handle *h, double *Jn);
int  dbat_hip_jtimes_sqnorm(dbat_hip_handle *h, const double *v, double *sqnorm);
int  dbat_hip_jtimes(dbat_hip_handle *h, const double *v, double *Jv);

int  dbat_hip_jacobian_sample(dbat_hip_handle *h, const double *x, int64_t n, const int64_t *ip_col, double *res,
                              double *JEO, double *JOP, double *JIO);

int  dbat_hip_jacobian_csc(dbat_hip_handle *h, const double *x, int32_t weighted, int64_t *nnz,
                           int64_t *colptr, int64_t *rowidx, double *val);


int  dbat_hip_solve(dbat_hip_handle *h, const dbat_hip_options *opt, double *x,
                    dbat_hip_result *result, double *res, double *damp, double *aux,
                    double *trace);

int  dbat_hip_final_residuals(dbat_hip_handle *h, double *r_unweighted, double *r_weighted);


#define DBAT_HIP_UNIQUE_ID_BYTES 128
int  dbat_hip_comm_unique_id(uint8_t *id );
int  dbat_hip_comm_init(dbat_hip_handle *h, const uint8_t *id );
int  dbat_hip_comm_allreduce_host(dbat_hip_handle *h, double *buf, int64_t count, int32_t op);

int  dbat_hip_set_deterministic(dbat_hip_handle *h, int32_t on);

typedef int (*dbat_hip_allreduce_fn)(void *user, void *buf_dev, int64_t count, void *stream);
int  dbat_hip_set_allreduce(dbat_hip_handle *h, dbat_hip_allreduce_fn fn, void *user);

int  dbat_hip_plan_domain_map(const dbat_hip_problem *prob, int32_t *cam_owner, int32_t *subtree);

int  dbat_hip_owned_mask(const dbat_hip_handle *h, uint8_t *mask);


int  dbat_hip_forwintersect(dbat_hip_handle *h, const double *x, const uint8_t *skip, double *OP);

int  dbat_hip_resect(int32_t device, int32_t n_images, const int64_t *pt_start, const double *X, const double *xn,
                     const int64_t *tri_start, const int32_t *tri, double *P, double *rms);


int  dbat_hip_rigidalign(int32_t device, int64_t n, const double *X, const double *Y, const uint8_t *use, int32_t scale,
                         double *T, double *stats, double *resid);

int  dbat_hip_multixform(int32_t device, const double *T, int64_t n_images, int32_t eo_rows, double *EO, int64_t n_points,
                         double *OP, uint8_t *fail);


int  dbat_hip_essmat5(int32_t device, int32_t n_sets, const int64_t *set_start, const double *Q1, const double *Q2,
                      double *E, int32_t *n_sol);

int  dbat_hip_relorient(int32_t device, int32_t n_pairs, const int64_t *pt_start, const double *x1, const double *x2,
                        const int64_t *hyp_start, const int32_t *samples, const double *thr2, int32_t front_dir,
                        double *E, double *P2, int32_t *stats, uint8_t *inlier, uint8_t *in_front, double *X);


typedef struct dbat_hip_pair_options {
    int32_t max_iter;
    double  conv_tol;
    double  min_angle;
} dbat_hip_pair_options;

int  dbat_hip_default_pair_options(dbat_hip_pair_options *opt);

int  dbat_hip_pairadjust(int32_t device, int32_t n_pairs, const int64_t *pt_start, const double *x1, const double *x2,
                         const uint8_t *use, const double *w1, const double *w2, int32_t front_dir,
                         const dbat_hip_pair_options *opt, double *P2, double *X, uint8_t *used, double *dstat,
                         int32_t *istat, double *Q, double *res);


int  dbat_hip_bench_step(dbat_hip_handle *h, double lambda, int32_t scale_columns, double *ms);
int  dbat_hip_set_x(dbat_hip_handle *h, const double *x);
int  dbat_hip_info(const dbat_hip_handle *h, int64_t *info );

int  dbat_hip_plan_layout_stats(const dbat_hip_problem *prob, int64_t *st );

int  dbat_hip_build_kernel_name(const dbat_hip_handle *h, char *buf, int32_t buf_len);

int  dbat_hip_chol_stats(const dbat_hip_handle *h, int64_t *st );

int  dbat_hip_posterior_cov(dbat_hip_handle *h, const double *x, double sigma0, double *CEO, double *CIO,
                            double *COP, double *Sinv);

int  dbat_hip_redundancy(dbat_hip_handle *h, const double *x, double *qvv_ip, double *r_prior);

int  dbat_hip_ray_angles(dbat_hip_handle *h, const double *x, double *op_angle, double *cam_angle,
                         int32_t *op_rays, int32_t *cam_rays);
int  dbat_hip_debug_ray_angles_host(const dbat_hip_problem *prob, double *op_angle, double *cam_angle);

typedef struct dbat_hip_depth_stats {
    int64_t n_behind;
    double  min_depth;
    int64_t argmin_column;
} dbat_hip_depth_stats;
int  dbat_hip_point_depths(dbat_hip_handle *h, const double *x, double thr, double *depth_out, double *img_min_out,
                           dbat_hip_depth_stats *stats_out);

int  dbat_hip_set_chirality(dbat_hip_handle *h, int32_t on, double min_depth);
typedef struct dbat_hip_veto_stats {
    int64_t tested, rejected, n_behind;
    double  min_depth;
} dbat_hip_veto_stats;
int  dbat_hip_chirality_stats(const dbat_hip_handle *h, dbat_hip_veto_stats *out);

int  dbat_hip_coverage(dbat_hip_handle *h, double *lo, double *hi, double *rad_max, int64_t *rad_ip, double *hull_area,
                       int64_t *hull_start, int64_t *hull_ip);
int  dbat_hip_residual_stats(dbat_hip_handle *h, const double *x, int64_t *cam_n, double *cam_ss, int64_t *op_n,
                             double *op_ss, double *total_ss, double *max_e, int64_t *max_ip);
int32_t dbat_hip_quality_hull_cap(void);
int  dbat_hip_debug_coverage_host(const dbat_hip_problem *prob, double *lo, double *hi, double *rad_max, int64_t *rad_ip,
                                  double *hull_area, int64_t *hull_start, int64_t *hull_ip);

#define DBAT_HIP_LOSS_HUBER    0
#define DBAT_HIP_LOSS_CAUCHY   1
#define DBAT_HIP_SCALE_APRIORI 0
#define DBAT_HIP_SCALE_MAD     1
#define DBAT_HIP_ROBUST_MAX_OUTER 64

typedef struct dbat_hip_robust_options {
    int32_t loss;
    double  k;
    int32_t scale;
    int32_t max_outer;
    double  weight_tol;
} dbat_hip_robust_options;

typedef struct dbat_hip_robust_result {
    int32_t outer;
    int32_t converged;
    int32_t inner_iters[DBAT_HIP_ROBUST_MAX_OUTER];
    double  scale[DBAT_HIP_ROBUST_MAX_OUTER];
    double  max_change;
    double  reweight_s;
} dbat_hip_robust_result;

int  dbat_hip_default_robust_options(int32_t loss, dbat_hip_robust_options *ropt);

int  dbat_hip_robust_weights(dbat_hip_handle *h, const double *x, const dbat_hip_robust_options *ropt,
                             double *omega, double *s_norm, double *scale);

int  dbat_hip_set_obs_weights(dbat_hip_handle *h, const double *omega);

int  dbat_hip_solve_robust(dbat_hip_handle *h, const dbat_hip_options *opt, const dbat_hip_robust_options *ropt,
                           double *x, dbat_hip_result *result, double *res, double *damp, double *aux, double *trace,
                           dbat_hip_robust_result *rr, double *omega_out);

#ifdef __cplusplus
}
#endif
#endif
```

Baseline: 647.0.

## Order each dataflow Cholesky sum's products by modeled tile availability

Adds plan-time product lists so each update task in the dataflow Cholesky walks its products in the order the schedule simulator expects their source tiles to be ready, instead of ascending column order. The host simulator iteratively re-sorts products by modeled availability, compares column-order, cut-sum and listed candidates, and picks the shortest simulated schedule. Listed tasks carry a flag bit and index into a new device list array. The aim is less time that workgroups spend spinning on tiles not yet finished, at the cost of more host planning time and an extra indirect load per product.

```diff
diff --git a/dbat_amd/_hip.py b/dbat_amd/_hip.py
--- a/dbat_amd/_hip.py
+++ b/dbat_amd/_hip.py
@@ -191,6 +191,8 @@
     'dbat_hip_residual_stats': (C.c_int, [_H, _dp, _lp, _dp, _lp, _dp, _dp, _dp, _lp]),
     'dbat_hip_quality_hull_cap': (C.c_int32, []),
     'dbat_hip_debug_coverage_host': (C.c_int, [C.POINTER(Problem), _dp, _dp, _dp, _lp, _dp, _lp, _lp]),
+    'dbat_hip_debug_df_schedule': (C.c_int, [C.POINTER(Problem), _lp, _dp, _ip, C.c_int64, _ip, C.c_int64,
+                                             C.POINTER(C.c_uint64), C.c_int64]),
     'dbat_hip_default_robust_options': (C.c_int, [C.c_int32, C.POINTER(RobustOptions)]),
     'dbat_hip_robust_weights': (C.c_int, [_H, _dp, C.POINTER(RobustOptions), _dp, _dp, _dp]),
     'dbat_hip_set_obs_weights': (C.c_int, [_H, _dp]),
@@ -1012,6 +1014,24 @@
     return part(out[:12]), part(out[12:])
 
 
+def df_schedule(s):
+    lib = load()
+    p, keep = problem_from_struct(s)
+    hdr = np.zeros(16, np.int64)
+    cand = np.zeros(4)
+    null_i, null_u = C.cast(None, _ip), C.cast(None, C.POINTER(C.c_uint64))
+    check(lib.dbat_hip_debug_df_schedule(C.byref(p), hdr.ctypes.data_as(_lp), dptr(cand), null_i, 0, null_i, 0, null_u, 0))
+    nT, W, nt, nl = (int(v) for v in hdr[:4])
+    jobs = np.zeros((max(nt, 1), 8), np.int32)
+    plist = np.zeros(max(nl, 1), np.int32)
+    rb = np.zeros(((nT + 1), W), np.uint64)
+    check(lib.dbat_hip_debug_df_schedule(C.byref(p), hdr.ctypes.data_as(_lp), dptr(cand), jobs.ctypes.data_as(_ip), jobs.size,
+                                         plist.ctypes.data_as(_ip), plist.size, rb.ctypes.data_as(C.POINTER(C.c_uint64)), rb.size))
+    return dict(nT=nT, W=W, jobs=jobs[:nt], plist=plist[:nl], listed_bit=int(hdr[10]), rowbits=rb, cand_us=[float(v) for v in cand],
+                taken=int(hdr[4]), nparts=int(hdr[5]), products=int(hdr[6]), chain_role=bool(hdr[7]), chain_tiles=int(hdr[8]),
+                n_listed=int(hdr[9]))
+
+
 def batch_stats(s, shard_rank=0, shard_count=1):
     lib = load()
     p, keep = problem_from_struct(s, 0, shard_rank, shard_count)
diff --git a/dbat_amd/csrc/chol_df.hpp b/dbat_amd/csrc/chol_df.hpp
--- a/dbat_amd/csrc/chol_df.hpp
+++ b/dbat_amd/csrc/chol_df.hpp
@@ -13,6 +13,7 @@
 constexpr int DF_SPIN_CAP = 1 << 22;
 
 struct DfTask { int i, k; };
+constexpr int DF_LISTED = 32;
 struct DfJob { int i, k, jlo, jhi, part, np, mode, p; };
 
 __device__ __forceinline__ double ld_coh(const double *p) {
@@ -403,6 +404,7 @@
     const int *pos;
     int ncols, nwg, ctr_slot, role_slot;
     int trace_potf2;
+    const int *plist;
 };
 
 __device__ __forceinline__ void df_issue_acc_tile(const double *T, int64_t ld, double (&tp)[16], int tx, int ty) {
@@ -640,6 +642,8 @@
         const DfJob jb = tasks[task];
         const int i = jb.i, k = jb.k;
         const bool helper = jb.np < 0;
+        const bool listed = CHAIN && (jb.mode & DF_LISTED) != 0;
+        const int mode = CHAIN ? jb.mode & ~DF_LISTED : jb.mode;
         const int jend = jb.jhi;
         int *pflags = flags + (int64_t)(nT + 1) * nT;
         int *tflags = pflags + nparts;
@@ -677,9 +681,11 @@
             if (w == (jend >> 6)) m &= (1ull << (jend & 63)) - 1;
             return m;
         };
-        int jw = jb.jlo >> 6;
-        uint64_t jm = jend > jb.jlo ? word(jw) : 0ull;
+        int jw = listed ? 0 : jb.jlo >> 6;
+        uint64_t jm = !listed && jend > jb.jlo ? word(jw) : 0ull;
+        int lp = jb.jlo;
         auto next_j = [&]() -> int {
+            if (listed) return lp < jend ? C.plist[lp++] : -1;
             for (;;) {
                 if (jm) { const int j = 64 * jw + __builtin_ctzll(jm); jm &= jm - 1; return j; }
                 if (jend <= jb.jlo || ++jw > wend) return -1;
@@ -818,7 +824,7 @@
             __syncthreads();
             continue;
         }
-        if (jb.mode == 1 || jb.mode == 16) {
+        if (mode == 1 || mode == 16) {
 #pragma unroll
             for (int rt = 0; rt < 4; ++rt)
 #pragma unroll
@@ -829,7 +835,7 @@
             if (trace && t == 0) trace[task * 16 + 3] = wall_clock64();
             __builtin_amdgcn_s_waitcnt(0);
             __syncthreads();
-            if (t == 0) __hip_atomic_store(jb.mode == 1 ? tflags + k : C.dflags + k, epoch, __ATOMIC_RELAXED, __HIP_MEMORY_SCOPE_AGENT);
+            if (t == 0) __hip_atomic_store(mode == 1 ? tflags + k : C.dflags + k, epoch, __ATOMIC_RELAXED, __HIP_MEMORY_SCOPE_AGENT);
             if (trace && t == 0) trace[task * 16 + 4] = wall_clock64();
             continue;
         }
@@ -851,7 +857,7 @@
                 const int zn = V.iperm ? V.iperm[col0 + tx] : (int)(col0 + tx);
                 if (zn >= 0) ldiag[zn] = smem[tx * DF_TLD + tx];
             }
-            if (jb.mode == 2) {
+            if (mode == 2) {
                 __syncthreads();
                 const int p = jb.p;
                 const int nrp = p == nT ? 1 : min(NB, n - NB * p);
@@ -1034,6 +1040,10 @@
     int64_t top_tile0 = 0, n_top_tiles = 0;
     std::vector<double> sim_critical_us, sim_schedule_us;
     std::vector<DfJob> h_tasksB;
+    std::vector<int> h_plist;
+    int *d_plist = nullptr;
+    double cand_us[4] = {-1.0, -1.0, -1.0, -1.0};
+    int cand_taken = 0;
     DfTask *d_tile_ij = nullptr;
     int nparts = 0;
     bool env_l2 = false;
@@ -1057,11 +1067,11 @@
     void release() {
         void *ps[] = {d_flags, d_ctl, d_bk_ptr, d_bk_idx, d_iperm, d_toff, d_rowbits, d_tasks, d_tile_ij, d_tiles, d_qperm, d_parts,
                       d_tasksB, d_bk_list, d_rowbits_top, d_chain_cols, d_chain_colsB, d_chain_par, d_chain_bits, d_chain_bitsB, d_chain_pos,
-                      d_ztiles, d_si_m, d_si_off, d_si_diag, d_perm};
+                      d_ztiles, d_si_m, d_si_off, d_si_diag, d_perm, d_plist};
         for (void *p : ps) if (p) (void)hipFree(p);
         d_flags = d_ctl = d_bk_ptr = d_bk_idx = d_iperm = nullptr; d_toff = nullptr; d_rowbits = nullptr;
         d_tasks = nullptr; d_tile_ij = nullptr; d_tiles = d_qperm = d_parts = nullptr;
-        d_tasksB = nullptr; d_bk_list = nullptr; d_rowbits_top = nullptr;
+        d_tasksB = nullptr; d_bk_list = nullptr; d_rowbits_top = nullptr; d_plist = nullptr;
         d_chain_cols = d_chain_colsB = d_chain_par = d_chain_bits = d_chain_bitsB = d_chain_pos = nullptr;
         d_ztiles = nullptr; d_si_m = d_si_off = nullptr; d_si_diag = d_perm = nullptr; n_si_m = 0;
         si_off_ptr.clear(); si_diag_ptr.clear();
@@ -1098,7 +1108,12 @@
         if (!v.empty()) (void)hipMemcpy(dst, v.data(), v.size() * sizeof(T), hipMemcpyHostToDevice);
         return true;
     }
-    struct JobList { std::vector<DfJob> jobs; std::vector<int> dptr, dep, own, sumjob, presum, bits, par; };
+    struct JobList {
+        std::vector<DfJob> jobs; std::vector<int> dptr, dep, own, sumjob, presum, bits, par;
+        std::vector<int> pj, ord, ord_list, walk; std::vector<char> listed;
+        double t_col = 0.0, t_list = -1.0, cp = 0.0;
+        int np = 0; long long nprod = 0;
+    };
     void build_jobs(int phase, const std::vector<uint64_t> &rowbits, const std::vector<int> &col_owner, int rank, JobList &L, int merge_depth = 0) {
         auto has = [&](int i, int k) { return (rowbits[(size_t)i * W + (k >> 6)] >> (k & 63)) & 1ull; };
         const int split_min = std::max(env_int("DBAT_HIP_DF_SPLIT", 96), 2);
@@ -1109,7 +1124,7 @@
         int dom_lo = nT, dom_hi = 0;
         if (phase == 1) for (int k = 0; k < nT; ++k) if (col_owner[k] == rank) { dom_lo = std::min(dom_lo, k); dom_hi = k + 1; }
         if (dom_hi <= dom_lo) dom_lo = dom_hi = 0;
-        L.jobs.clear(); L.dptr.assign(1, 0); L.dep.clear();
+        L.jobs.clear(); L.dptr.assign(1, 0); L.dep.clear(); L.pj.clear();
         L.own.assign((size_t)(nT + 1) * nT, -1); L.sumjob.assign(nT, -1);
         L.presum.assign(nT, -1); L.bits.assign(nT, 0); L.par.assign(nT, -1);
         const bool chain = use_chain && merge;
@@ -1130,7 +1145,7 @@
             }
             auto emit = [&](int i, int mode, int par, int jhi_owner) {
                 auto push_products = [&](int q0, int q1) {
-                    for (int q = q0; q < q1; ++q) { L.dep.push_back(L.own[(size_t)k * nT + js[q]]); L.dep.push_back(i != k ? L.own[(size_t)i * nT + js[q]] : -1); }
+                    for (int q = q0; q < q1; ++q) { L.dep.push_back(L.own[(size_t)k * nT + js[q]]); L.dep.push_back(i != k ? L.own[(size_t)i * nT + js[q]] : -1); L.pj.push_back(js[q]); }
                     L.dptr.push_back((int)L.dep.size());
                 };
                 n_products += (long long)js.size();
@@ -1198,7 +1213,7 @@
                 if (has(i, k) && i != par) { products(i); L.own[(size_t)i * nT + k] = emit(i, 0, -1, k); }
         }
     }
-    void order_jobs(JobList &L, const char *what) {
+    void order_jobs(JobList &L, const char *what, int sums = 0) {
         std::vector<DfJob> &jobs = L.jobs;
         const std::vector<int> &dptr = L.dptr, &dep = L.dep, &own = L.own, &sumjob = L.sumjob;
         const int nt = (int)jobs.size();
@@ -1234,14 +1249,17 @@
             for_deps(t, [&](int d) { blev[d] = std::max(blev[d], blev[t]); });
         }
         const int workers = std::max(1, std::min(grid, 256));
+        std::vector<double> done;
+        const std::vector<int> *walk = nullptr;
         auto simulate = [&](const std::vector<int> &ord) {
-            std::vector<double> done(nt, 0.0);
+            done.assign(nt, 0.0);
             std::priority_queue<double, std::vector<double>, std::greater<double>> freeat;
             for (int w = 0; w < workers; ++w) freeat.push(0.0);
             double last = 0.0;
             for (int t : ord) {
                 double tc = freeat.top(); freeat.pop();
-                for (int q = dptr[t]; q + 1 < dptr[t + 1]; q += 2) {
+                for (int a = dptr[t] / 2; a < dptr[t + 1] / 2; ++a) {
+                    const int q = walk ? dptr[t] + 2 * (*walk)[a] : 2 * a;
                     double av = done[dep[q]];
                     if (dep[q + 1] >= 0) av = std::max(av, done[dep[q + 1]]);
                     tc = std::max(tc, av + c_hop) + c_prod;
@@ -1284,7 +1302,7 @@
         };
         const double betas[] = {0.0, 0.25, 0.5, 1.0, 2.0, 4.0, 1e6};
         const int ncand = (int)(sizeof(betas) / sizeof(betas[0])) + 1;
-        std::vector<int> best_ord;
+        std::vector<int> best_ord, list_ords[2];
         double tbest = 1e300;
         int best = -1;
         std::vector<double> key(nt), tcs(ncand);
@@ -1295,11 +1313,61 @@
             else for (int t = 0; t < nt; ++t) key[t] = est[t] - c_prod * nprod_of(t);
             std::vector<int> ord = kahn(key);
             tcs[c] = simulate(ord);
+            if (sums == 1 || sums < 0) { if (c == 0) list_ords[0] = ord; else if (c == 3) list_ords[1] = ord; }
             if (forced == c || (forced < 0 && tcs[c] < tbest)) { tbest = tcs[c]; best = c; best_ord.swap(ord); }
         }
         double cp = 0.0;
         for (int t = 0; t < nt; ++t) cp = std::max(cp, fin[t]);
         sim_critical_us.push_back(cp); sim_schedule_us.push_back(tbest);
+        L.t_col = tbest; L.t_list = -1.0; L.cp = cp;
+        L.ord_list = best_ord;
+        L.walk.clear(); L.listed.assign(nt, 0);
+        if (sums != 0) {
+            const int nslots = (int)dep.size() / 2;
+            std::vector<int> wk(nslots);
+            for (int t = 0; t < nt; ++t) for (int a = dptr[t] / 2; a < dptr[t + 1] / 2; ++a) wk[a] = a - dptr[t] / 2;
+            if (sums == 2 || sums == 3) {
+                if (sums == 3) for (int t = 0; t < nt; ++t) std::reverse(wk.begin() + dptr[t] / 2, wk.begin() + dptr[t + 1] / 2);
+                walk = &wk;
+                L.t_list = simulate(best_ord);
+                L.walk = wk;
+                for (int t = 0; t < nt; ++t) L.listed[t] = nprod_of(t) > 0;
+            } else {
+                std::vector<double> avail(nslots);
+                for (int lo = -1; lo < 2; ++lo) {
+                    const std::vector<int> &ord = lo < 0 ? best_ord : list_ords[lo];
+                    if (lo >= 0 && (ord.empty() || forced >= 0 || ord == best_ord)) continue;
+                    walk = nullptr;
+                    double tprev = simulate(ord);
+                    for (int round = 0; round < 3; ++round) {
+                        for (int t = 0; t < nt; ++t)
+                            for (int a = dptr[t] / 2; a < dptr[t + 1] / 2; ++a) {
+                                avail[a] = done[dep[2 * a]];
+                                if (dep[2 * a + 1] >= 0) avail[a] = std::max(avail[a], done[dep[2 * a + 1]]);
+                            }
+                        for (int t = 0; t < nt; ++t) {
+                            const int a0 = dptr[t] / 2;
+                            for (int a = a0; a < dptr[t + 1] / 2; ++a) wk[a] = a - a0;
+                            std::stable_sort(wk.begin() + a0, wk.begin() + dptr[t + 1] / 2, [&](int x, int y) { return avail[a0 + x] < avail[a0 + y]; });
+                        }
+                        walk = &wk;
+                        const double tl = simulate(ord);
+                        if (L.t_list < 0.0 || tl < L.t_list) { L.t_list = tl; L.walk = wk; L.ord_list = ord; }
+                        if (!(tl < tprev)) break;
+                        tprev = tl;
+                    }
+                }
+                for (int t = 0; t < nt; ++t)
+                    for (int a = dptr[t] / 2; a < dptr[t + 1] / 2; ++a) if (L.walk[a] != a - dptr[t] / 2) L.listed[t] = 1;
+            }
+            walk = nullptr;
+            if (stats_on()) {
+                int nl = 0;
+                for (int t = 0; t < nt; ++t) nl += L.listed[t];
+                fprintf(stderr, "[chol %s] product lists (mode %d): %d of %d tasks listed, simulated %.0f us (column order %.0f us)\n", what, sums, nl, nt, L.t_list, L.t_col);
+            }
+        }
+        L.ord = best_ord;
         if (stats_on()) {
             fprintf(stderr, "[chol %s] %d tasks, critical path %.0f us; simulated with %d workgroups, key = earliest start - beta x bottom level:",
                     what, nt, cp, workers);
@@ -1309,6 +1377,21 @@
         std::vector<DfJob> sorted(nt);
         for (int t = 0; t < nt; ++t) sorted[t] = jobs[best_ord[t]];
         jobs.swap(sorted);
+    }
+    static void apply_lists(JobList &L, std::vector<int> &plist) {
+        std::vector<DfJob> byno(L.jobs.size());
+        for (size_t t = 0; t < L.jobs.size(); ++t) byno[L.ord[t]] = L.jobs[t];
+        for (size_t t = 0; t < L.jobs.size(); ++t) L.jobs[t] = byno[L.ord_list[t]];
+        L.ord = L.ord_list;
+        for (size_t t = 0; t < L.jobs.size(); ++t) {
+            const int o = L.ord[t];
+            if (!L.listed[o]) continue;
+            const int a0 = L.dptr[o] / 2, a1 = L.dptr[o + 1] / 2;
+            L.jobs[t].jlo = (int)plist.size();
+            for (int a = a0; a < a1; ++a) plist.push_back(L.pj[a0 + L.walk[a]]);
+            L.jobs[t].jhi = (int)plist.size();
+            L.jobs[t].mode |= DF_LISTED;
+        }
     }
     struct Sched { std::vector<int> colsA, colsB, bitsA, bitsB, par, pos, bkl, bptr, bidx; std::vector<uint64_t> rowbits_top; };
     bool quiet = false;
@@ -1318,6 +1401,8 @@
         if (const char *g = env_get("DBAT_HIP_DF_GRID")) grid = std::min(std::max(atoi(g), 1), 4096);
         nparts = 0; n_products = 0;
         two_phase = !col_owner.empty();
+        h_plist.clear(); cand_taken = 0;
+        for (double &c : cand_us) c = -1.0;
         h_rowbits = rowbits;
         use_chain = permuted && env_int("DBAT_HIP_DF_CHAIN", 1) != 0;
         if (use_chain && !two_phase && !env_get("DBAT_HIP_DF_CHAIN")) {
@@ -1363,21 +1448,39 @@
         std::vector<int> &bkl = H.bkl;
         bkl.clear(); h_tasksB.clear(); ntasksB = 0; nchain = nchainB = 0; chain_wg = chain_wgB = 0;
         if (!two_phase) {
+            const int sums = permuted && use_chain ? env_int("DBAT_HIP_DF_SUMS", -1) : 0;
             build_jobs(0, rowbits, col_owner, rank, L);
-            order_jobs(L, "all");
+            L.np = nparts; L.nprod = n_products;
+            order_jobs(L, "all", sums);
             const int force_merge = env_int("DBAT_HIP_DF_MERGE", -1);
+            JobList M;
+            bool have_cut = false;
             if (use_chain && force_merge != 0) {
-                const int np0 = nparts;
-                const long long prod0 = n_products;
-                JobList M;
                 nparts = 0; n_products = 0;
                 build_jobs(0, rowbits, col_owner, rank, M, 2);
-                order_jobs(M, "all, sums cut at the merge columns");
-                const bool better = nparts <= 4096 && (force_merge == 1 || sim_schedule_us[1] < 0.99 * sim_schedule_us[0]);
-                if (better) std::swap(L, M); else { nparts = np0; n_products = prod0; }
-                sim_critical_us.erase(sim_critical_us.begin() + (better ? 0 : 1)); sim_schedule_us.erase(sim_schedule_us.begin() + (better ? 0 : 1));
-                if (stats_on()) fprintf(stderr, "[chol] sums cut at the merge columns: %s (%d partial sums)\n", better ? "yes" : "no", nparts);
-            }
+                M.np = nparts; M.nprod = n_products;
+                order_jobs(M, "all, sums cut at the merge columns", sums);
+                have_cut = M.np <= 4096;
+            }
+            cand_us[0] = L.t_col; cand_us[1] = have_cut ? M.t_col : -1.0;
+            cand_us[2] = L.t_list; cand_us[3] = have_cut ? M.t_list : -1.0;
+            const bool must_cut = have_cut && force_merge == 1;
+            int taken = must_cut || (have_cut && M.t_col < 0.99 * L.t_col) ? 1 : 0;
+            if (sums == 1) taken = must_cut || (have_cut && M.t_list < 0.99 * L.t_list) ? 3 : 2;
+            else if (sums == 2 || sums == 3) taken += 2;
+            else if (sums < 0) {
+                if (!must_cut && L.t_list >= 0.0 && L.t_list < 0.99 * cand_us[taken]) taken = 2;
+                if (have_cut && M.t_list >= 0.0 && M.t_list < 0.99 * cand_us[taken]) taken = 3;
+            }
+            cand_taken = taken;
+            if (taken & 1) std::swap(L, M);
+            nparts = L.np; n_products = L.nprod;
+            h_plist.clear();
+            if (taken >= 2) apply_lists(L, h_plist);
+            sim_critical_us.assign(1, L.cp); sim_schedule_us.assign(1, cand_us[taken]);
+            if (stats_on())
+                fprintf(stderr, "[chol] schedules: column order %.0f us, sums cut %.0f us, product lists %.0f us, lists and cut sums %.0f us -> %d (%d partial sums, %zu listed products)\n",
+                        cand_us[0], cand_us[1], cand_us[2], cand_us[3], taken, nparts, h_plist.size());
             split_chain(L, h_tasks, colsA); ntasks = (int)h_tasks.size();
             for (int j = nT - 1; j >= 0; --j) bkl.push_back(j);
         } else {
@@ -1432,6 +1535,7 @@
         }
         if (use_chain && (!up(d_chain_cols, H.colsA) || !up(d_chain_bits, H.bitsA) || !up(d_chain_par, H.par) || !up(d_chain_pos, H.pos))) return false;
         if (env_on("DBAT_HIP_DF_TRACE") && !two_phase && hipMalloc(&d_trace, (size_t)(ntasks + 3 * nT) * 16 * sizeof(long long)) != hipSuccess) d_trace = nullptr;
+        if (!up(d_plist, h_plist)) return false;
         if (!up(d_tasks, h_tasks) || !up(d_bk_ptr, H.bptr) || !up(d_bk_idx, H.bidx) || !up(d_rowbits, rowbits) || !up(d_toff, toff) || !up(d_bk_list, H.bkl))
             return false;
         if (hipMalloc(&d_flags, ((size_t)(nT + 1) * nT + (size_t)nparts + 4 * (size_t)nT) * sizeof(int)) != hipSuccess) return false;
@@ -1689,6 +1793,7 @@
         C.nwg = which ? chain_wgB : chain_wg;
         C.ctr_slot = which ? 5 : 3; C.role_slot = which ? 6 : 4;
         C.trace_potf2 = env_int("DBAT_HIP_DF_TRACE_POTF2", 0);
+        C.plist = d_plist;
         return C;
     }
     int chain_grid(int work, int wg) const { return std::max(std::min(grid, work + wg), wg + 1); }
diff --git a/dbat_amd/csrc/debug_host.hpp b/dbat_amd/csrc/debug_host.hpp
--- a/dbat_amd/csrc/debug_host.hpp
+++ b/dbat_amd/csrc/debug_host.hpp
@@ -177,6 +177,41 @@
     API_CATCH
 }
 
+int dbat_hip_debug_df_schedule(const dbat_hip_problem *prob, int64_t *hdr, double *cand_us, int32_t *jobs, int64_t jobs_cap,
+                               int32_t *plist, int64_t plist_cap, uint64_t *rowbits, int64_t rowbits_cap) {
+    API_TRY
+    if (!prob || !hdr || !cand_us) { g_err = "null argument"; return DBAT_HIP_EINVAL; }
+    Plan P;
+    if (!build_plan(*prob, P, false)) { g_err = P.err; return DBAT_HIP_EINVAL; }
+    if (P.shared_eo || P.nd.nparts > 1) { g_err = "df_schedule: the compact layout on one rank only"; return DBAT_HIP_EINVAL; }
+    DataflowChol D;
+    DataflowChol::Symbolic Y;
+    D.symbolic_permuted(P.nc, P.nIOu, P.cam_adj.data(), P.cam_adj_words, P.nd, Y);
+    DataflowChol::Sched H;
+    D.schedule_host(Y.rb, Y.col_owner, 0, H);
+    int64_t nlisted = 0;
+    for (const DfJob &j : D.h_tasks) nlisted += (j.mode & DF_LISTED) != 0;
+    const int64_t h[16] = {D.nT, D.W, D.ntasks, (int64_t)D.h_plist.size(), D.cand_taken, D.nparts, D.n_products, D.use_chain ? 1 : 0,
+                           D.nchain, nlisted, DF_LISTED, (int64_t)Y.rb.size(), 0, 0, 0, 0};
+    std::copy(h, h + 16, hdr);
+    std::copy(D.cand_us, D.cand_us + 4, cand_us);
+    if (jobs) {
+        if (jobs_cap < (int64_t)D.h_tasks.size() * 8) { g_err = "df_schedule: task buffer too small"; return DBAT_HIP_EINVAL; }
+        static_assert(sizeof(DfJob) == 8 * sizeof(int32_t), "DfJob is eight ints");
+        if (!D.h_tasks.empty()) memcpy(jobs, D.h_tasks.data(), D.h_tasks.size() * sizeof(DfJob));
+    }
+    if (plist) {
+        if (plist_cap < (int64_t)D.h_plist.size()) { g_err = "df_schedule: list buffer too small"; return DBAT_HIP_EINVAL; }
+        std::copy(D.h_plist.begin(), D.h_plist.end(), plist);
+    }
+    if (rowbits) {
+        if (rowbits_cap < (int64_t)Y.rb.size()) { g_err = "df_schedule: pattern buffer too small"; return DBAT_HIP_EINVAL; }
+        std::copy(Y.rb.begin(), Y.rb.end(), rowbits);
+    }
+    return DBAT_HIP_OK;
+    API_CATCH
+}
+
 int dbat_hip_debug_model_eval_host(int32_t model, int32_t nK, int32_t nP, const double *EO6, const double *IO,
                                    double px_size, const double *Q3, const double *uv, double *r2,
                                    double *A12, double *B6, double *C ) {
diff --git a/dbat_amd/csrc/env.hpp b/dbat_amd/csrc/env.hpp
--- a/dbat_amd/csrc/env.hpp
+++ b/dbat_amd/csrc/env.hpp
@@ -33,6 +33,7 @@
     {"DBAT_HIP_DF_CHUNK", false, "factorisation: products per helper task (default 32)"},
     {"DBAT_HIP_DF_CHAIN", false, "factorisation: 0 = diagonal tiles as ordinary tasks (no chain role), 1 = chain role whatever the pattern", "0|1"},
     {"DBAT_HIP_DF_MERGE", false, "factorisation: sums of the columns where two parts of the dissection meet cut into early and late pieces: 0 = never, 1 = wherever the chain role is on (default: where the simulated schedule is shorter)", "0|1"},
+    {"DBAT_HIP_DF_SUMS", false, "factorisation, compact tiles on one rank with the chain role on: a sum takes its products in the order the schedule's model expects their tiles to exist (a list fixed at plan time): 0 = never, 1 = always, 2 / 3 = every task a list in ascending / descending column order (control, tests) (default: where the simulated schedule is shorter)", "0|1|2|3"},
     {"DBAT_HIP_DF_CHAIN_WG", false, "factorisation: workgroups of the chain role at most (default 32)"},
     {"DBAT_HIP_DF_L2", false, "factorisation: 1 = finished tiles of the compact layout are read through the L2", "0|1"},
     {"DBAT_HIP_COV_DENSE", false, "posterior covariance: the dense inverse of the reduced system (rocsolver_dpotri) instead of the selected inversion"},
diff --git a/include/dbat_hip.h b/include/dbat_hip.h
--- a/include/dbat_hip.h
+++ b/include/dbat_hip.h
@@ -247,6 +247,9 @@
 int32_t dbat_hip_quality_hull_cap(void);
 int  dbat_hip_debug_coverage_host(const dbat_hip_problem *prob, double *lo, double *hi, double *rad_max, int64_t *rad_ip,
                                   double *hull_area, int64_t *hull_start, int64_t *hull_ip);
+int  dbat_hip_debug_df_schedule(const dbat_hip_problem *prob, int64_t *hdr, double *cand_us, int32_t *jobs,
+                                int64_t jobs_cap, int32_t *plist, int64_t plist_cap, uint64_t *rowbits,
+                                int64_t rowbits_cap);
 
 #define DBAT_HIP_LOSS_HUBER    0
 #define DBAT_HIP_LOSS_CAUCHY   1
```

Measured after the change: 660.1, median of 6. 1.02x the previous value.
